# SnakeOnex/vit-is-all-you-need

Measured on AMD Instinct MI355X. Metric: images/sec ViT-B/16 224px bf16 fwd+bwd, higher is better.
Workload: dtype bf16; 1 GPU; ViT-B/16 224x224 bf16 forward+loss+backward, batch 256 per GPU (BASELINE configs[1]; configs[2] at 8 GPUs), random-init weights, 197 tokens, 79.44 M params; global_batch=256, parallelism=dp1

## Files before the change

### include/vitamd.h

```cpp
#ifndef VITAMD_H
#define VITAMD_H

#ifdef __cplusplus
extern "C" {
#endif

#define VITAMD_OK 0
#define VITAMD_ERR_SHAPE 1
#define VITAMD_ERR_ARG 2
#define VITAMD_ERR_LAUNCH 3
#define VITAMD_ERR_INIT 4

int vitamd_abi_version(void);

int vitamd_init(int device, void* stream);

#define VITAMD_EPI_BIAS_BF16 0
#define VITAMD_EPI_GELU 1
#define VITAMD_EPI_RESID_F32 2
#define VITAMD_EPI_DGELU 3
#define VITAMD_EPI_PATCH_F32 4
#define VITAMD_EPI_F32 5
#define VITAMD_EPI_GELU_DG 6
#define VITAMD_EPI_DMUL 7

int vitamd_gemm_nt_bf16(const void* A, const void* B, void* out, void* out2, const float* bias, const void* aux,
                        float* colsum, int M, int N, int K, int ldo, int epi, int n_patches, int seq, int extra,
                        int tile, void* stream);

#define VITAMD_NT_FORM_SMALL 1
#define VITAMD_NT_FORM_PP 2
#define VITAMD_NT_FORM_PP_PERSISTENT 3
#define VITAMD_NT_FORM_SEAM 4
#define VITAMD_NT_FORM_LOADER 5
#define VITAMD_NT_FORM_TAIL_SPLIT 0x80
int vitamd_gemm_nt_plan(int M, int N, int K, int ldo, int epi, int tile);

int vitamd_linear_dropout_resid_bf16(const void* A, const void* B, float* out, const float* bias, const float* resid,
                                     int M, int N, int K, float dropout_p, unsigned long long seed, int tile, void* stream);

int vitamd_gemm_tn_bf16(const void* L, const void* Rm, float* out, int R, int P, int Q, int ldl, int ldr, int ldo,
                        int splits, void* stream);

#define VITAMD_TN_FORM_SHARED 0
#define VITAMD_TN_FORM_EXCLUSIVE 1
int vitamd_gemm_tn_bf16_ws(const void* L, const void* Rm, float* out, int R, int P, int Q, int ldl, int ldr, int ldo,
                           int splits, float* ws, long ws_bytes, int accumulate, int form, void* stream);
long vitamd_gemm_tn_ws_bytes(int R, int P, int Q, int splits);

int vitamd_layernorm_fwd(const float* x_in, const void* addend_bf16, float* x_out, void* y_bf16, float* mean,
                         float* rstd, int M, int D, float eps, void* stream);
int vitamd_layernorm_bwd(const void* dy_bf16, const float* x, const float* mean, const float* rstd,
                         const float* g_res, float* g_out, void* g_bf16, float* colsum, int M, int D, void* stream);
int vitamd_layernorm_bwd_dropout(const void* dy_bf16, const float* x, const float* mean, const float* rstd,
                                 const float* g_res, float* g_out, void* g_bf16, float* colsum, int M, int D,
                                 float dropout_p, unsigned long long seed, void* stream);
int vitamd_layernorm_bwd_xhat(const void* dy_bf16, const void* y_bf16, const float* rstd, const float* g_res, float* g_out,
                              void* g_bf16, float* colsum, int M, int D, float dropout_p, unsigned long long seed, void* stream);
int vitamd_layernorm_fwd_keep(const float* x_in, const void* addend_bf16, float* x_out, void* y_bf16, float* mean, float* rstd,
                              int B, int seq, int keep, int D, float eps, void* stream);
int vitamd_layernorm_bwd_keep(const void* dy_bf16, const void* x_or_y, const float* mean, const float* rstd, const float* g_res,
                              float* g_out, void* g_bf16, float* colsum, int B, int seq, int keep, int D, int use_xhat,
                              float dropout_p, unsigned long long seed, void* stream);

int vitamd_layernorm_affine_fwd(const float* x, const float* gamma, const float* beta, void* y_bf16, float* mean,
                                float* rstd, int M, int D, float eps, void* stream);
int vitamd_layernorm_affine_bwd(const void* dy_bf16, const float* x, const float* mean, const float* rstd,
                                const float* gamma, const float* g_res, float* g_out, void* g_bf16, float* colsum,
                                float* dgamma, float* dbeta, int M, int D, void* stream);
int vitamd_layernorm_affine_fwd_f32(const float* x, const float* gamma, const float* beta, float* y, float* mean,
                                    float* rstd, int M, int D, float eps, void* stream);
int vitamd_layernorm_affine_bwd_f32(const float* dy, const float* x, const float* mean, const float* rstd,
                                    const float* gamma, float* g_out, float* dgamma, float* dbeta, int M, int D, void* stream);

int vitamd_attention_fwd(const void* qkv, void* o, float* lse2, int B, int N, int H, int head_dim, int causal,
                         float dropout_p, unsigned long long seed, void* stream);
int vitamd_attention_fwd_resid(const void* qkv, void* o, float* lse2, const float* resid_in, float* resid_out, int B, int N, int H,
                               int head_dim, int causal, float dropout_p, unsigned long long seed, void* stream);
int vitamd_attention_bwd(const void* qkv, const void* o, const float* lse2, const void* d_o, void* dqkv,
                         float* delta, float* dbias, int B, int N, int H, int head_dim, int causal, float dropout_p,
                         unsigned long long seed, void* stream);
int vitamd_attention_keep_forms(int N, int nq);
int vitamd_attention_fwd_keep(const void* qkv, void* o, float* lse2, int B, int N, int H, int head_dim, int nq, void* stream);
int vitamd_attention_bwd_keep(const void* qkv, const void* o, const float* lse2, const void* d_o, void* dqkv, float* delta,
                              float* dbias, int B, int N, int H, int head_dim, int nq, void* stream);

int vitamd_kv_append(const void* qkv, void* k_cache, void* v_cache, const int* len, int B, int T, int H, int head_dim, int Lmax,
                     void* stream);
long vitamd_decode_attention_ws_bytes(int B, int H, int Lmax);
int vitamd_decode_attention(const void* qkv, const void* k_cache, const void* v_cache, void* o, const int* len, int B, int H,
                            int head_dim, int Lmax, float* ws, long ws_bytes, void* stream);
long vitamd_gemm_skinny_ws_bytes(int M, int N, int K);
int vitamd_gemm_skinny_bf16(const void* A, const void* W, void* out, void* out2, const float* bias, const float* aux, int M, int N,
                            int K, int epi, float* ws, long ws_bytes, void* stream);

int vitamd_gemm_skinny_qkv_append(const void* A, const void* W, void* qkv, const float* bias, void* k_cache, void* v_cache, const int* len,
                                  int M, int H, int K, int head_dim, int Lmax, float* ws, long ws_bytes, void* stream);
int vitamd_decode_embed(const float* tok_table, const float* pos_table, const long long* token, const int* len, float* x, int B, int D,
                        int tok_rows, int pos_rows, void* stream);

int vitamd_sample_logits(const float* logits, long long* token, float* info, const float* u, const unsigned long long* step, int B, int V,
                         int ld, float temperature, int top_k, float top_p, unsigned long long seed, void* stream);

int vitamd_cross_entropy_fwd(const void* logits, int logits_bf16, const long long* target, float* loss_row, float* lse, float* stats,
                             int M, int V, int ld, long long ignore_index, void* stream);
int vitamd_cross_entropy_grid_rows(int V);
int vitamd_cross_entropy_bwd(const void* logits, int logits_bf16, const long long* target, const float* lse, const float* stats,
                             const float* grad_out, void* dlogits, int dlogits_bf16, int M, int V, int ld, int ldo,
                             long long ignore_index, void* stream);
int vitamd_embed_tokens_fwd(const float* tok_table, const float* pos_table, const long long* ids, float* x, int B, int S, int D,
                            int tok_rows, int pos_rows, void* stream);
int vitamd_embed_tokens_bwd(const float* g, const long long* ids, float* dtok, float* dpos, int B, int S, int D, int tok_rows, void* stream);

int vitamd_cast_f32_bf16(const float* in, void* out_bf16, long n, void* stream);
int vitamd_cast_f32_bf16_dropout(const float* in, void* out_bf16, long n, float dropout_p, unsigned long long seed, void* stream);
int vitamd_dropout_bf16(const void* in, void* out, long n, long group, float dropout_p, unsigned long long seed, void* stream);
int vitamd_dropout_f32(const float* in, float* out, long n, long group, float dropout_p, unsigned long long seed, void* stream);
int vitamd_cast_transpose_weight(const float* w, void* wb, void* wbt, int N, int K, void* stream);
int vitamd_cast_transpose_batched(const void* desc_dev, int n, int total_tiles, void* stream);
int vitamd_im2col_bf16(const float* img, void* out_bf16, int B, int C, int H, int W, int p, void* stream);
int vitamd_colsum_bf16(const void* x_bf16, float* out, int M, int N, int ld, void* stream);
int vitamd_embed_bwd(const float* g, float* dpos, float* dextra, void* dyp_bf16, float* dbias, float* dbias_rows, int B,
                     int seq, int extra, int D, void* stream);

int vitamd_vq_nearest(const float* x, const float* codebook, long long* idx, int M, int K, int d, void* stream);

int vitamd_conv3x3_fwd(const float* x, const float* w, const float* bias, float* y, int B, int Cin, int Cout, int H, int W,
                       void* stream);
int vitamd_conv3x3_bwd(const float* x, const float* w, const float* dy, float* dx, float* dw, float* db, int B, int Cin,
                       int Cout, int H, int W, void* stream);

int vitamd_adamw_step(float* p, const float* g, float* m, float* v, long n, float lr, float beta1, float beta2,
                      float eps, float weight_decay, int step, void* stream);
int vitamd_adamw_step_d(float* p, const float* g, float* m, float* v, long n, float lr, double beta1, double beta2,
                        float eps, float weight_decay, int step, void* stream);

typedef struct vitamd_mt_row {
  float* p;
  const float* g;
  float* m;
  float* v;
  long long n;
  int first_chunk;
  float lr, weight_decay;
  float beta1, one_minus_beta1, beta2, one_minus_beta2;
  float eps;
  float inv_bc1;
  float inv_sqrt_bc2;
} vitamd_mt_row;
long vitamd_mt_row_bytes(void);
int vitamd_mt_chunk_elems(void);
int vitamd_mt_grid_cap(void);
int vitamd_mt_sumsq(const vitamd_mt_row* rows_host, const void* rows_dev, int n_rows, int total_chunks, float* partials, float* norm_coef,
                    float max_norm, void* stream);
int vitamd_mt_adamw(const vitamd_mt_row* rows_host, const void* rows_dev, int n_rows, int total_chunks, const float* coef, void* stream);
int vitamd_mt_scale(const vitamd_mt_row* rows_host, const void* rows_dev, int n_rows, int total_chunks, const float* coef, void* stream);

#ifdef __cplusplus
}
#endif
#endif
```

### vit-is-all-you-need_amd/csrc/capi.hip

```cpp
#include "common.h"
#include "vitamd_internal.h"
#include "../../include/vitamd.h"

extern "C" int vitamd_abi_version(void) { return 9; }

extern "C" int vitamd_init(int device, void* stream) { return vitamd_init_impl(device, (hipStream_t)stream); }

extern "C" int vitamd_gemm_nt_bf16(const void* A, const void* B, void* out, void* out2, const float* bias, const void* aux,
                                   float* colsum, int M, int N, int K, int ldo, int epi, int n_patches, int seq, int extra,
                                   int tile, void* stream) {
  const int dg = (epi == 6 || epi == 7) ? 1 : 0;
  if (epi == 6) epi = EPI_GELU;
  if (epi == 7) epi = EPI_DGELU;
  GemmNtArgs p{A, B, out, out2, bias, aux, colsum, M, N, K, ldo, epi, n_patches, seq, extra, tile, 0u, 1.0f, 0u, 0u, 0, dg};
  if (!is_auto(tile) && tile != NT_TILE_128 && tile != NT_TILE_256 && tile != NT_TILE_320 && tile != NT_TILE_LOADER) return VITAMD_ERR_ARG;
  return vitamd_gemm_nt_impl(p, (hipStream_t)stream);
}

extern "C" int vitamd_gemm_nt_plan(int M, int N, int K, int ldo, int epi, int tile) {
  const int dg = (epi == 6 || epi == 7) ? 1 : 0;
  if (epi == 6) epi = EPI_GELU;
  if (epi == 7) epi = EPI_DGELU;
  static char dummy[16];
  GemmNtArgs p{dummy, dummy, dummy, dummy, nullptr, dummy, (float*)dummy, M, N, K, ldo, epi, 1, 1, 0, tile, 0u, 1.0f, 0u, 0u, 0, dg};
  if (!is_auto(tile) && tile != NT_TILE_128 && tile != NT_TILE_256 && tile != NT_TILE_320 && tile != NT_TILE_LOADER) return -VITAMD_ERR_ARG;
  return vitamd_gemm_nt_plan_impl(p);
}

extern "C" int vitamd_gemm_tn_bf16(const void* L, const void* Rm, float* out, int R, int P, int Q, int ldl, int ldr, int ldo,
                                   int splits, void* stream) {
  GemmTnArgs a{L, Rm, out, R, P, Q, ldl, ldr, ldo, splits, nullptr, 0, 1, 0};
  return vitamd_gemm_tn_impl(a, (hipStream_t)stream);
}

extern "C" int vitamd_gemm_tn_bf16_ws(const void* L, const void* Rm, float* out, int R, int P, int Q, int ldl, int ldr, int ldo,
                                      int splits, float* ws, long ws_bytes, int accumulate, int form, void* stream) {
  if (form != 0 && form != 1) return VITAMD_ERR_ARG;
  GemmTnArgs a{L, Rm, out, R, P, Q, ldl, ldr, ldo, splits, ws, (size_t)(ws_bytes < 0 ? 0 : ws_bytes), accumulate, form};
  return vitamd_gemm_tn_impl(a, (hipStream_t)stream);
}

static bool dropout_params(float p, unsigned& thresh, float& scale) {
  if (!(p >= 0.0f) || p >= 1.0f) return false;
  thresh = p > 0.0f ? (unsigned)((double)p * 4294967296.0) : 0u;
  if (p > 0.0f && thresh == 0u) thresh = 1u;
  scale = 1.0f / (1.0f - p);
  return true;
}

extern "C" int vitamd_linear_dropout_resid_bf16(const void* A, const void* B, float* out, const float* bias, const float* resid,
                                                int M, int N, int K, float dropout_p, unsigned long long seed, int tile, void* stream) {
  if (!is_auto(tile) && tile != NT_TILE_128 && tile != NT_TILE_256 && tile != NT_TILE_320) return VITAMD_ERR_ARG;
  GemmNtArgs p{A, B, out, nullptr, bias, resid, nullptr, M, N, K, N, EPI_RESID_F32, 0, 0, 0, tile, 0u, 1.0f,
               (unsigned)seed, (unsigned)(seed >> 32), 0, 0};
  if (!dropout_params(dropout_p, p.drop_thresh, p.drop_scale)) return VITAMD_ERR_ARG;
  return vitamd_gemm_nt_impl(p, (hipStream_t)stream);
}
```

### vit-is-all-you-need_amd/csrc/gemm_nt.hip

```cpp
#include <type_traits>
#include <mutex>
#include <atomic>
#include <cmath>
#include <cstring>
#include <climits>
#include "gemm_nt_ld.h"

namespace {

template <int BM, int BN, int WM, int WN, int EPI>
__global__ __launch_bounds__(WM * WN * 64) void gemm_nt_kernel(const GemmNtArgs p) {
  constexpr int NW = WM * WN;
  constexpr int WTM = BM / WM, WTN = BN / WN;
  constexpr int MT = WTM / 16, NT = WTN / 16;
  constexpr int PIECES = (BM + BN) / 8;
  constexpr int PPW = PIECES / NW;
  static_assert(PIECES % NW == 0, "pieces must divide over waves");
  constexpr int BUF_BYTES = (BM + BN) * 128;

  extern __shared__ __attribute__((aligned(16))) char smem[];

  const int tid = threadIdx.x;
  const int lane = tid & 63;
  const int wave = __builtin_amdgcn_readfirstlane(tid >> 6);
  const int wm = wave / WN, wn = wave % WN;

  const int tiles_n = (p.N + BN - 1) / BN;
  const int tiles_m = (p.M + BM - 1) / BM;
  const int tile = xcd_remap(blockIdx.x, tiles_m * tiles_n);
  const int m0 = (tile / tiles_n) * BM;
  const int n0 = (tile % tiles_n) * BN;

  const __bf16* __restrict__ A = (const __bf16*)p.A;
  const __bf16* __restrict__ B = (const __bf16*)p.B;
  const int K = p.K;

  const __bf16* src[PPW];
#pragma unroll
  for (int i = 0; i < PPW; ++i) {
    const int piece = wave * PPW + i;
    const int row = piece * 8 + (lane >> 3);
    const int logical = (lane & 7) ^ (row & 7);
    if (piece < BM / 8) {
      const int g = min(m0 + row, p.M - 1);
      src[i] = A + (size_t)g * K + logical * 8;
    } else {
      const int g = min(n0 + row - BM, p.N - 1);
      src[i] = B + (size_t)g * K + logical * 8;
    }
  }

  auto stage = [&](int kt, int buf) {
    char* base = smem + buf * BUF_BYTES + wave * PPW * 1024;
#pragma unroll
    for (int i = 0; i < PPW; ++i) glds16(src[i] + kt * BK, base + i * 1024);
  };

  f32x4 acc[MT][NT];
#pragma unroll
  for (int i = 0; i < MT; ++i)
#pragma unroll
    for (int j = 0; j < NT; ++j) acc[i][j] = (f32x4){0.f, 0.f, 0.f, 0.f};

  const int frag_off = (lane & 15) * 128 + ((((lane >> 4) ^ (lane & 7)) & 7) << 4);
  const int a_off = wm * WTM * 128 + frag_off;
  const int b_off = BM * 128 + wn * WTN * 128 + frag_off;

  const int nkt = K / BK;
  stage(0, 0);
  for (int kt = 0; kt < nkt; ++kt) {
    const int cur = kt & 1;
    asm volatile("s_waitcnt vmcnt(0)" ::: "memory");
    __syncthreads();
    if (kt + 1 < nkt) stage(kt + 1, cur ^ 1);
    const char* buf = smem + cur * BUF_BYTES;
#pragma unroll
    for (int ks = 0; ks < 2; ++ks) {
      bf16x8 af[MT], bfr[NT];
#pragma unroll
      for (int j = 0; j < NT; ++j) bfr[j] = *(const bf16x8*)(buf + ((b_off + j * 16 * 128) ^ (ks * 64)));
#pragma unroll
      for (int i = 0; i < MT; ++i) af[i] = *(const bf16x8*)(buf + ((a_off + i * 16 * 128) ^ (ks * 64)));
#pragma unroll
      for (int i = 0; i < MT; ++i)
#pragma unroll
        for (int j = 0; j < NT; ++j)
          acc[i][j] = __builtin_amdgcn_mfma_f32_16x16x32_bf16(bfr[j], af[i], acc[i][j], 0, 0, 0);
    }
  }
  if constexpr (BM == 256 && BN == 256 && WM == 2 && WN == 4 && EPI != EPI_F32) {
    if (p.N % 8 == 0 && p.ldo % 8 == 0) {
      gemm_epilogue_rows<EPI>(p, acc, m0, n0, wm, wn, lane, tid, wave, smem);
      return;
    }
  }
  gemm_epilogue<BN, WM, WN, WTM, WTN, MT, NT, EPI>(p, acc, m0, n0, wm, wn, lane, tid, smem);
}

template <int EPI, int MT, int LA, int LB, bool PERS = false>
__global__ __launch_bounds__(512) void gemm_nt_pp_kernel(const GemmNtArgs p) {
  using S = NtSchedule<MT, LA>;
  static_assert(LB == S::LB, "the B lead the shared schedule implements");
  constexpr int NP = S::NP;
  constexpr int BM = 32 * MT, BN = 256, WN = 4, NT = 4;
  constexpr int PART = 64 * 128;
  constexpr int BUFB = NP * PART + 256 * 128;

  extern __shared__ __attribute__((aligned(16))) char smem[];
  const int tid = threadIdx.x, lane = tid & 63;
  const int wave = __builtin_amdgcn_readfirstlane(tid >> 6);
  const int wm = wave / WN, wn = wave % WN;
  const int tiles_n = (p.N + BN - 1) / BN, tiles_m = (p.M + BM - 1) / BM;
  const int ntiles = tiles_m * tiles_n;
  const int K = p.K;
  const int nkt = K / 64;
  const srd_t srdA = make_srd(p.A, (size_t)p.M * K * 2);
  const srd_t srdB = make_srd(p.B, (size_t)p.N * K * 2);
  for (int ti = blockIdx.x; ti < ntiles; ti += PERS ? (int)gridDim.x : ntiles) {
  const NtTile t = nt_tile<BM>(ti, tiles_m, tiles_n);
  const int m0 = t.m0, n0 = t.n0;
  unsigned voffA[NP], voffB[4];
  pp_offsets<MT, false>(p, t, wave, lane, voffA, voffB);
  const unsigned lds0 = lds_addr(smem) + wave * 1024;
  constexpr unsigned OOB = 0x80000000u;
  auto request_a = [&](int kt, int j) {
    const bool live = kt >= 0 && kt < nkt;
    asm_glds16(srdA, lds0 + (kt & 1) * BUFB + j * PART, live ? voffA[j] : OOB, live ? (unsigned)kt * 128u : 0u);
  };
  auto request_b = [&](int kt, int q) {
    const bool live = kt >= 0 && kt < nkt;
    asm_glds16(srdB, lds0 + (kt & 1) * BUFB + NP * PART + q * 8192, live ? voffB[q] : OOB, live ? (unsigned)kt * 128u : 0u);
  };

  f32x4 acc[MT][NT];
#pragma unroll
  for (int i = 0; i < MT; ++i)
#pragma unroll
    for (int j = 0; j < NT; ++j) acc[i][j] = (f32x4){0.f, 0.f, 0.f, 0.f};

  const char *rdA[2], *rdB[2];
  frag_bases(smem + wm * 32 * 128, lane, rdA);
  frag_bases(smem + NP * PART + wn * 64 * 128, lane, rdB);

#pragma unroll
  for (int P = -S::lookback; P < 0; ++P) S::requests(S::tile_of(P), S::phase_of(P), request_a, request_b);
  VITAMD_WAIT_VM(S::wait(NP - 1));
  __builtin_amdgcn_s_barrier();
  asm volatile("" ::: "memory");
  if (wm == 1) __builtin_amdgcn_s_barrier();

  auto ktile = [&](int kt, auto bufc) {
    constexpr int BUF = decltype(bufc)::value;
    pp_ktile<MT, PART>(acc, rdA[0] + BUF * BUFB, rdA[1] + BUF * BUFB, rdB[0] + BUF * BUFB, rdB[1] + BUF * BUFB,
                       [&](int ph) { S::requests(kt, ph, request_a, request_b); }, [&](int ph) { VITAMD_WAIT_VM(S::wait(ph)); });
  };
  int kt = 0;
  for (; kt + 1 < nkt; kt += 2) {
    ktile(kt, std::integral_constant<int, 0>{});
    ktile(kt + 1, std::integral_constant<int, 1>{});
  }
  if (kt < nkt) ktile(kt, std::integral_constant<int, 0>{});
  if (wm == 0) __builtin_amdgcn_s_barrier();
  asm volatile("s_waitcnt vmcnt(0)" ::: "memory");
  if constexpr (EPI == EPI_F32) gemm_epilogue<BN, 2, WN, 16 * MT, 64, MT, NT, EPI>(p, acc, m0, n0, wm, wn, lane, tid, smem);
  else if (p.N % 8 == 0 && p.ldo % 8 == 0) gemm_epilogue_rows<EPI, MT>(p, acc, m0, n0, wm, wn, lane, tid, wave, smem);
  else gemm_epilogue<BN, 2, WN, 16 * MT, 64, MT, NT, EPI>(p, acc, m0, n0, wm, wn, lane, tid, smem);
  if constexpr (PERS) __syncthreads();
  }
}

static int device_cus() {
  static int cus[16] = {};
  int dev = 0;
  if (hipGetDevice(&dev) != hipSuccess || dev < 0 || dev >= 16) return 256;
  if (!cus[dev]) {
    int n = 0;
    cus[dev] = (hipDeviceGetAttribute(&n, hipDeviceAttributeMultiprocessorCount, dev) == hipSuccess && n > 0) ? n : 256;
  }
  return cus[dev];
}

template <int EPI, int MT, int LA, int LB, bool PERS = false>
int launch_pp(const GemmNtArgs& p, hipStream_t stream) {
  constexpr int ops_b = 2 * ((MT / 2) * 8192 + 32768), epi_b = 8 * MT * 2048;
  return launch_tiles(gemm_nt_pp_kernel<EPI, MT, LA, LB, PERS>, p, stream, 32 * MT, 512, ops_b > epi_b ? ops_b : epi_b, PERS ? device_cus() : INT_MAX);
}
#undef VITAMD_WAIT_VM

template <int BM, int BN, int WM, int WN, int EPI>
int launch(const GemmNtArgs& p, hipStream_t stream) {
  constexpr int lds = 2 * (BM + BN) * 128;
  auto kern = gemm_nt_kernel<BM, BN, WM, WN, EPI>;
  if (int e = set_lds(kern, lds)) return e;
  const int tiles = ((p.M + BM - 1) / BM) * ((p.N + BN - 1) / BN);
  hipLaunchKernelGGL(kern, dim3(tiles), dim3(WM * WN * 64), lds, stream, p);
  return hipGetLastError() == hipSuccess ? VITAMD_OK : VITAMD_ERR_LAUNCH;
}

static bool prefer_tall(const GemmNtArgs& p) {
  if (p.N % 8 != 0 || p.ldo % 8 != 0 || p.K % 64 != 0) return false;
  if (p.epi != EPI_BIAS_BF16 && p.epi != EPI_RESID_F32 && p.epi != EPI_GELU && p.epi != EPI_DGELU) return false;
  const long tn = (p.N + 255) / 256;
  const long r256 = (((p.M + 255) / 256) * tn + 255) / 256, r320 = (((p.M + 319) / 320) * tn + 255) / 256;
  return r320 * 320 <= r256 * 256;
}

static unsigned short bf16_rne_d(double v) {
  auto val = [](unsigned short b) { const unsigned w = (unsigned)b << 16; float g; memcpy(&g, &w, 4); return (double)g; };
  const float f = (float)v;
  unsigned u;
  memcpy(&u, &f, 4);
  unsigned short best = (unsigned short)((u + 0x7fffu + ((u >> 16) & 1u)) >> 16);
  double bd = fabs(val(best) - v);
  const unsigned short first = best;
  for (int dl = -1; dl <= 1; dl += 2) {
    const unsigned short n = (unsigned short)(first + dl);
    const double dd = fabs(val(n) - v);
    if (dd < bd || (dd == bd && !(n & 1) && (best & 1))) { best = n; bd = dd; }
  }
  return best;
}

static std::atomic<const unsigned*> g_gelu_tab[64];

static const unsigned* gelu_table() {
  int dev = -1;
  if (hipGetDevice(&dev) != hipSuccess || dev < 0 || dev >= 64) { (void)hipGetLastError(); return nullptr; }
  return g_gelu_tab[dev].load(std::memory_order_acquire);
}

}

const unsigned* vitamd_gelu_table() { return gelu_table(); }

int vitamd_init_impl(int device, hipStream_t stream) {
  static std::mutex mu;
  static unsigned host[4096];
  static bool built = false;
  int cur = -1;
  if (hipGetDevice(&cur) != hipSuccess) { (void)hipGetLastError(); return VITAMD_ERR_LAUNCH; }
  if (device < 0) device = cur;
  if (device >= 64) return VITAMD_ERR_ARG;
  std::lock_guard<std::mutex> lock(mu);
  if (g_gelu_tab[device].load(std::memory_order_acquire)) return VITAMD_OK;
  hipStreamCaptureStatus cap = hipStreamCaptureStatusNone;
  if (hipStreamIsCapturing(stream, &cap) != hipSuccess || cap != hipStreamCaptureStatusNone) { (void)hipGetLastError(); return VITAMD_ERR_ARG; }
  if (!built) {
    for (int sg = 0; sg < 2; ++sg)
      for (int i = 0; i < 2048; ++i) {
        const unsigned w = (unsigned)(0x3900 + i) << 16;
        float ax;
        memcpy(&ax, &w, 4);
        const double x = sg ? -(double)ax : (double)ax;
        const double cdf = 0.5 * erfc(-x * 0.70710678118654752440);
        const double pdf = 0.39894228040143267794 * exp(-0.5 * x * x);
        host[sg * 2048 + i] = (unsigned)bf16_rne_d(x * cdf) | ((unsigned)bf16_rne_d(cdf + x * pdf) << 16);
      }
    built = true;
  }
  if (device != cur && hipSetDevice(device) != hipSuccess) { (void)hipGetLastError(); return VITAMD_ERR_ARG; }
  void* d = nullptr;
  bool ok = hipMalloc(&d, sizeof(host)) == hipSuccess;
  ok = ok && hipMemcpy(d, host, sizeof(host), hipMemcpyHostToDevice) == hipSuccess && hipDeviceSynchronize() == hipSuccess;
  if (!ok) {
    (void)hipGetLastError();
    if (d) (void)hipFree(d);
  }
  if (device != cur) (void)hipSetDevice(cur);
  if (!ok) return VITAMD_ERR_LAUNCH;
  g_gelu_tab[device].store((const unsigned*)d, std::memory_order_release);
  return VITAMD_OK;
}

namespace {

enum NtForm { NT_FORM_SMALL = 1, NT_FORM_PP = 2, NT_FORM_PP_PERSISTENT = 3, NT_FORM_SEAM = 4, NT_FORM_LOADER = 5 };
struct NtPlan { int form, rows, err; };

static NtPlan plan_single(const GemmNtArgs& p) {
  int tile = p.tile;
  const int epi = p.epi;
  const bool seam_epi = epi == EPI_BIAS_BF16 || epi == EPI_GELU || epi == EPI_DGELU;
  const bool tall_epi = seam_epi || epi == EPI_RESID_F32;
  if (tile == NT_TILE_LOADER) return (seam_epi && ld_ok(p)) ? NtPlan{NT_FORM_LOADER, 256, VITAMD_OK} : NtPlan{0, 0, VITAMD_ERR_SHAPE};
  const bool no_seam = tile == NT_TILE_AUTO_NO_SEAM;
  if (no_seam) tile = NT_TILE_AUTO;
  const long big_tiles = (long)((p.M + 255) / 256) * ((p.N + 255) / 256);
  const bool pp_ok = (size_t)p.M * p.K * 2 < 0xf0000000ull && (size_t)p.N * p.K * 2 < 0xf0000000ull && p.K % 64 == 0;
  const bool big = p.N >= 256 && big_tiles >= 192 && pp_ok;
  const bool tall = tall_epi && prefer_tall(p);
  if (tile == NT_TILE_AUTO_NO_PERSISTENT) tile = NT_TILE_AUTO;
  else if (tile == NT_TILE_AUTO && big) {
    const int cus = device_cus();
    if (seam_epi && !no_seam && seam_ok(p) && p.K <= 1536) {
      if (epi == EPI_BIAS_BF16 && tall && (long)((p.M + 319) / 320) * ((p.N + 255) / 256) >= 3L * cus) return NtPlan{NT_FORM_SEAM, 320, VITAMD_OK};
      if (big_tiles >= 3L * cus) return NtPlan{ld_ok(p) ? NT_FORM_LOADER : NT_FORM_SEAM, 256, VITAMD_OK};
    }
    return NtPlan{NT_FORM_PP_PERSISTENT, tall ? 320 : 256, VITAMD_OK};
  }
  if (tile == NT_TILE_AUTO) tile = big ? (tall ? NT_TILE_320 : NT_TILE_256) : NT_TILE_128;
  if (tile == NT_TILE_320) return (tall_epi && pp_ok) ? NtPlan{NT_FORM_PP, 320, VITAMD_OK} : NtPlan{0, 0, VITAMD_ERR_SHAPE};
  if (tile == NT_TILE_256) return pp_ok ? NtPlan{NT_FORM_PP, 256, VITAMD_OK} : NtPlan{0, 0, VITAMD_ERR_SHAPE};
  if (tile != NT_TILE_128) return NtPlan{0, 0, VITAMD_ERR_ARG};
  return p.K % BK == 0 ? NtPlan{NT_FORM_SMALL, 128, VITAMD_OK} : NtPlan{0, 0, VITAMD_ERR_SHAPE};
}

template <int EPI>
int dispatch_tile(const GemmNtArgs& p, hipStream_t stream) {
  constexpr bool seam_epi = EPI == EPI_BIAS_BF16 || EPI == EPI_GELU || EPI == EPI_DGELU;
  constexpr bool tall_epi = seam_epi || EPI == EPI_RESID_F32;
  const NtPlan pl = plan_single(p);
  if (pl.err) return pl.err;
  switch (pl.form) {
    case NT_FORM_LOADER:
      if constexpr (seam_epi) return launch_ld<EPI, EPI == EPI_GELU>(p, stream, device_cus());
      break;
    case NT_FORM_SEAM:
      if constexpr (EPI == EPI_BIAS_BF16) { if (pl.rows == 320) return launch_seam<EPI, 10>(p, stream, device_cus()); }
      if constexpr (seam_epi) return launch_seam<EPI, 8, EPI == EPI_GELU>(p, stream, device_cus());
      break;
    case NT_FORM_PP_PERSISTENT:
      if constexpr (tall_epi) { if (pl.rows == 320) return launch_pp<EPI, 10, 4, 6, true>(p, stream); }
      return launch_pp<EPI, 8, 4, 6, true>(p, stream);
    case NT_FORM_PP:
      if constexpr (tall_epi) { if (pl.rows == 320) return launch_pp<EPI, 10, 4, 6>(p, stream); }
      return launch_pp<EPI, 8, 4, 6>(p, stream);
    case NT_FORM_SMALL:
      return launch<128, 128, 2, 2, EPI>(p, stream);
  }
  return VITAMD_ERR_SHAPE;
}

}

static int dispatch_epi(const GemmNtArgs& p, hipStream_t stream) {
  switch (p.epi) {
    case EPI_BIAS_BF16: return dispatch_tile<EPI_BIAS_BF16>(p, stream);
    case EPI_GELU: return dispatch_tile<EPI_GELU>(p, stream);
    case EPI_RESID_F32: return dispatch_tile<EPI_RESID_F32>(p, stream);
    case EPI_DGELU: return dispatch_tile<EPI_DGELU>(p, stream);
    case EPI_PATCH_F32: return dispatch_tile<EPI_PATCH_F32>(p, stream);
    case EPI_F32: return dispatch_tile<EPI_F32>(p, stream);
    default: return VITAMD_ERR_ARG;
  }
}

static int tail_split_rows(const GemmNtArgs& p, bool& tall) {
  const int CUS = device_cus();
  tall = is_auto(p.tile) && prefer_tall(p);
  const int bm = tall ? 320 : 256;
  const int tiles_m = (p.M + bm - 1) / bm, tiles_n = (p.N + 255) / 256;
  const long big_tiles = (long)tiles_m * tiles_n;
  const long rem = big_tiles % CUS;
  const bool split_on = p.epi == EPI_RESID_F32 && !tall;
  if (!(is_auto(p.tile) && split_on && p.epi != EPI_PATCH_F32 && p.N >= 256 && p.K % 64 == 0 && big_tiles > 2 * CUS && rem != 0 && rem * 10 < CUS * 6))
    return 0;
  const int rows_a = (int)((big_tiles - rem) / tiles_n) * bm;
  return rows_a > 0 && rows_a < p.M ? rows_a : 0;
}

static int check_args(const GemmNtArgs& p) {
  if (p.M <= 0 || p.N <= 0 || p.K <= 0 || p.K % 32 != 0 || p.N % 4 != 0 || p.ldo % 4 != 0) return VITAMD_ERR_SHAPE;
  if (!p.A || !p.B || !p.out) return VITAMD_ERR_ARG;
  if (p.epi == EPI_GELU && !p.out2) return VITAMD_ERR_ARG;
  if ((p.epi == EPI_RESID_F32 || p.epi == EPI_DGELU) && !p.aux) return VITAMD_ERR_ARG;
  if (p.epi == EPI_PATCH_F32 && (!p.aux || p.n_patches <= 0)) return VITAMD_ERR_ARG;
  if (p.epi < EPI_BIAS_BF16 || p.epi > EPI_F32) return VITAMD_ERR_ARG;
  return VITAMD_OK;
}

int vitamd_gemm_nt_impl(const GemmNtArgs& p0, hipStream_t stream) {
  if (int e = check_args(p0)) return e;
  GemmNtArgs p = p0;
  if (p.epi == EPI_GELU) {
    p.gelu_tab = gelu_table();
    if (!p.gelu_tab) return VITAMD_ERR_INIT;
  }
  bool tall = false;
  const int rows_a = tail_split_rows(p, tall);
  if (rows_a) {
    GemmNtArgs a = p, b = p;
    a.M = rows_a;
    a.tile = tall ? p.tile : NT_TILE_256;
    const size_t esz_out = (p.epi == EPI_RESID_F32 || p.epi == EPI_F32) ? 4 : 2;
    b.M = p.M - rows_a;
    b.A = (const char*)p.A + (size_t)rows_a * p.K * 2;
    b.out = (char*)p.out + (size_t)rows_a * p.ldo * esz_out;
    if (p.out2) b.out2 = (char*)p.out2 + (size_t)rows_a * p.ldo * 2;
    if (p.aux) b.aux = (const char*)p.aux + (size_t)rows_a * p.ldo * (p.epi == EPI_RESID_F32 ? 4 : 2);
    b.tile = NT_TILE_128;
    b.row0 = p.row0 + rows_a;
    if (int e = dispatch_epi(a, stream)) return e;
    return dispatch_epi(b, stream);
  }
  return dispatch_epi(p, stream);
}

int vitamd_gemm_nt_plan_impl(const GemmNtArgs& p0) {
  if (int e = check_args(p0)) return -e;
  bool tall = false;
  GemmNtArgs p = p0;
  const int rows_a = tail_split_rows(p, tall);
  if (rows_a) {
    p.M = rows_a;
    p.tile = tall ? p.tile : NT_TILE_256;
  }
  const NtPlan pl = plan_single(p);
  if (pl.err) return -pl.err;
  return pl.form | (pl.rows << 8) | (rows_a ? 0x80 : 0);
}
```

### vit-is-all-you-need_amd/csrc/gemm_nt_ld.h

```cpp
#pragma once
#include "gemm_nt_seam.h"

namespace {

template <int EPI, bool TAB = false, int SCHED = 1>
__global__ __launch_bounds__(768) void gemm_nt_ld_kernel(const GemmNtArgs p) {
  static_assert(EPI == EPI_BIAS_BF16 || EPI == EPI_GELU || EPI == EPI_DGELU, "epilogues of the loader form");
  static_assert(SCHED == 1, "request schedule");
  static_assert(!TAB || EPI == EPI_GELU, "table = GELU");
  constexpr int BM = 256, BN = 256, MT = 8, NT = 4;
  constexpr int AREG = 16384, ABUF = 32768, BBUF = 32768, BBASE = 2 * ABUF, OPS = BBASE + 2 * BBUF;
  constexpr int STG = 2048, TABOFF = OPS + 8 * STG;
  constexpr unsigned OOB = 0x80000000u;

  extern __shared__ __attribute__((aligned(16))) char smem[];
  const int tid = threadIdx.x, lane = tid & 63;
  const int wave = __builtin_amdgcn_readfirstlane(tid >> 6);
  const int tiles_n = (p.N + BN - 1) / BN, tiles_m = (p.M + BM - 1) / BM;
  const int ntiles = tiles_m * tiles_n;
  const int K = p.K;
  const int nkt = K / 64;
  auto coords = [&](int ti) { return nt_tile<BM>(ti, tiles_m, tiles_n); };

  if (wave >= 8) {
    const int l = wave - 8;
    const srd_t srdA = make_srd(p.A, (size_t)p.M * K * 2);
    const srd_t srdB = make_srd(p.B, (size_t)p.N * K * 2);
    const srd_t srdBias = make_srd(p.bias ? (const void*)p.bias : p.out, p.bias ? (size_t)p.N * 4 : 0);
    const unsigned ldsA = lds_addr(smem) + l * 4096;
    const unsigned ldsB = lds_addr(smem) + BBASE + l * 8192;
    unsigned voffA[2][4], voffB[8];
    auto offsets = [&](const NtTile& t) {
      const int r8 = lane >> 3;
      const unsigned chunk = (unsigned)(((lane & 7) ^ r8) * 16);
#pragma unroll
      for (int h = 0; h < 2; ++h)
#pragma unroll
        for (int i = 0; i < 4; ++i) {
          const int a = 4 * l + i;
          const int row = min(t.m0 + (a >> 3) * 128 + h * 64 + (a & 7) * 8 + r8, p.M - 1);
          voffA[h][i] = (unsigned)row * (unsigned)(K * 2) + chunk;
        }
#pragma unroll
      for (int i = 0; i < 8; ++i) {
        const int row = min(t.n0 + (8 * l + i) * 8 + r8, p.N - 1);
        voffB[i] = (unsigned)row * (unsigned)(K * 2) + chunk;
      }
    };
    bool live = true;
    unsigned so = 0u, par = 0u;
    auto request_b = [&](int i) {
      asm_glds16(srdB, ldsB + par * BBUF + i * 1024, live ? voffB[i] : OOB, so);
    };
    auto request_a = [&](int h, int i) {
      asm_glds16(srdA, ldsA + par * ABUF + h * AREG + i * 1024, live ? voffA[h][i] : OOB, so);
    };
    auto target = [&](int kt, bool lv) {
      live = lv;
      so = live ? (unsigned)kt * 128u : 0u;
      par = (unsigned)(kt & 1);
    };
    __builtin_amdgcn_s_setprio(3);
    int ti = blockIdx.x;
    NtTile cur = coords(ti);
    offsets(cur);
    int bias_n0 = cur.n0;
    target(0, true);
#pragma unroll
    for (int i = 0; i < 8; ++i) request_b(i);
#pragma unroll
    for (int i = 0; i < 4; ++i) request_a(0, i);
#pragma unroll
    for (int i = 0; i < 4; ++i) request_a(1, i);
    VITAMD_WAIT_VM(4);
    __builtin_amdgcn_s_barrier();
    for (;;) {
      const int ti_next = ti + (int)gridDim.x;
      const bool has_next = ti_next < ntiles;
      for (int kt = 0; kt < nkt; ++kt) {
        const bool last = kt + 1 == nkt;
        if (last && has_next) {
          cur = coords(ti_next);
          offsets(cur);
        }
        target(last ? 0 : kt + 1, !last || has_next);
        request_b(0); request_b(1); request_b(2);
        __builtin_amdgcn_s_barrier();
        request_b(3); request_b(4); request_b(5);
        VITAMD_WAIT_VM(6);
        __builtin_amdgcn_s_barrier();
        if constexpr (EPI != EPI_DGELU) {
          if (kt == 0) {
            asm_glds4(srdBias, lds_addr(smem) + OPS + l * STG, (unsigned)(bias_n0 + l * 64 + lane) * 4u, 0u);
            asm_glds4(srdBias, lds_addr(smem) + OPS + (4 + l) * STG, (unsigned)(bias_n0 + l * 64 + lane) * 4u, 0u);
          }
        }
        request_b(6); request_b(7); request_a(0, 0);
        __builtin_amdgcn_s_barrier();
        request_a(0, 1); request_a(0, 2); request_a(0, 3);
        __builtin_amdgcn_s_barrier();
        request_a(1, 0); request_a(1, 1);
        __builtin_amdgcn_s_barrier();
        request_a(1, 2); request_a(1, 3);
        __builtin_amdgcn_s_barrier();
        __builtin_amdgcn_s_barrier();
        VITAMD_WAIT_VM(4);
        __builtin_amdgcn_s_barrier();
      }
      __builtin_amdgcn_s_barrier();
      if (!has_next) break;
      ti = ti_next;
      bias_n0 = cur.n0;
    }
    asm volatile("s_waitcnt vmcnt(0)" ::: "memory");
    return;
  }

  const int wm = wave >> 2, wn = wave & 3;
  const srd_t rsO = make_srd(p.out, (size_t)p.M * p.ldo * 2);
  const srd_t rsO2 = make_srd(EPI == EPI_GELU ? p.out2 : p.out, (size_t)p.M * p.ldo * 2);
  const srd_t srdAux = make_srd(EPI == EPI_DGELU ? p.aux : p.out, (size_t)p.M * p.ldo * 2);
  if constexpr (TAB) gelu_table_to_lds(p.gelu_tab, smem + TABOFF, tid);
  __builtin_amdgcn_s_barrier();
  asm volatile("" ::: "memory");
  for (int ti = blockIdx.x; ti < ntiles; ti += (int)gridDim.x) {
    const NtTile cur = coords(ti);
    if (wm == 1) __builtin_amdgcn_s_barrier();
    f32x4 acc[MT][NT];
#pragma unroll
    for (int i = 0; i < MT; ++i)
#pragma unroll
      for (int j = 0; j < NT; ++j) acc[i][j] = (f32x4){0.f, 0.f, 0.f, 0.f};
    {
      int l2 = (int)__builtin_amdgcn_mbcnt_hi(~0u, __builtin_amdgcn_mbcnt_lo(~0u, 0u));
      asm volatile("" : "+v"(l2));
      const char *rdA[2], *rdB[2];
      frag_bases(smem + wm * 8192, l2, rdA);
      frag_bases(smem + BBASE + wn * 8192, l2, rdB);
      bf16x8 bq[NT], af[4];
      auto ktile = [&](auto bufc) {
        constexpr int BUF = decltype(bufc)::value;
#pragma unroll
        for (int ph = 0; ph < 4; ++ph) {
          const int ks = ph >> 1, h = ph & 1;
          if (h == 0) {
#pragma unroll
            for (int j = 0; j < NT; ++j) bq[j] = *(const bf16x8*)(rdB[ks] + BUF * BBUF + j * 2048);
          }
#pragma unroll
          for (int ii = 0; ii < 4; ++ii) af[ii] = *(const bf16x8*)(rdA[ks] + BUF * ABUF + h * AREG + ii * 2048);
          __builtin_amdgcn_sched_barrier(0);
          __builtin_amdgcn_s_barrier();
          asm volatile("s_waitcnt lgkmcnt(0)" ::: "memory");
          __builtin_amdgcn_sched_barrier(0);
          __builtin_amdgcn_s_setprio(1);
#pragma unroll
          for (int ii = 0; ii < 4; ++ii)
#pragma unroll
            for (int j = 0; j < NT; ++j)
              acc[4 * h + ii][j] = __builtin_amdgcn_mfma_f32_16x16x32_bf16(bq[j], af[ii], acc[4 * h + ii][j], 0, 0, 0);
          __builtin_amdgcn_s_setprio(0);
          __builtin_amdgcn_sched_barrier(0);
          __builtin_amdgcn_s_barrier();
          asm volatile("" ::: "memory");
        }
      };
      for (int kt = 0; kt < nkt; kt += 2) {
        ktile(std::integral_constant<int, 0>{});
        ktile(std::integral_constant<int, 1>{});
      }
    }
    if (wm == 0) __builtin_amdgcn_s_barrier();

    int ln = (int)__builtin_amdgcn_mbcnt_hi(~0u, __builtin_amdgcn_mbcnt_lo(~0u, 0u));
    asm volatile("" : "+v"(ln));
    const int mloc = ln & 15, g = ln >> 4, rsub = ln >> 3, pc = ln & 7;
    char* const stg = smem + OPS + wave * STG;
    const int m0 = cur.m0, n0 = cur.n0;
    const int ncol = n0 + wn * 64 + 8 * (pc ^ rsub);
    const bool ncol_ok = ncol < p.N;
    const int mrow0 = m0 + wm * 128 + rsub;
    const unsigned obase = ncol_ok ? (unsigned)mrow0 * (unsigned)(p.ldo * 2) + (unsigned)ncol * 2u : OOB;
    const unsigned rstep = (unsigned)(p.ldo * 2) * 8u;
    u32x4 aux[EPI == EPI_DGELU ? 2 * MT : 1];
    u32x2 pk[EPI == EPI_DGELU ? MT : 1][NT];
    f32x4 bias4[NT];
    if constexpr (EPI == EPI_DGELU) {
#pragma unroll
      for (int i = 0; i < MT; ++i)
#pragma unroll
        for (int j = 0; j < NT; ++j) pk[i][j] = (u32x2){pack_bf16x2(acc[i][j][0], acc[i][j][1]), pack_bf16x2(acc[i][j][2], acc[i][j][3])};
#pragma unroll
      for (int it = 0; it < 2 * MT; ++it) aux[it] = asm_bload16(srdAux, mrow0 + 8 * it < p.M ? obase : OOB, rstep * (unsigned)it);
      static_assert(MT == 8, "16 pre-load registers named in one asm statement");
      asm volatile("s_waitcnt vmcnt(0)" : "+v"(aux[0]), "+v"(aux[1]), "+v"(aux[2]), "+v"(aux[3]), "+v"(aux[4]), "+v"(aux[5]), "+v"(aux[6]), "+v"(aux[7]), "+v"(aux[8]), "+v"(aux[9]), "+v"(aux[10]), "+v"(aux[11]), "+v"(aux[12]), "+v"(aux[13]), "+v"(aux[14]), "+v"(aux[15]) :: "memory");
    } else {
#pragma unroll
      for (int j = 0; j < NT; ++j)
#pragma unroll
        for (int r = 0; r < 4; ++r) bias4[j][r] = round_bf16(((const float*)stg)[16 * j + 4 * g + r]);
    }
    float cs[8];
#pragma unroll
    for (int c = 0; c < 8; ++c) cs[c] = 0.f;
#pragma unroll
    for (int i = 0; i < MT; ++i) {
#pragma unroll
      for (int j = 0; j < NT; ++j) {
        u32x2 o;
        if constexpr (EPI == EPI_DGELU) o = pk[i][j];
        else {
          const f32x4 v = acc[i][j] + bias4[j];
          o = (u32x2){pack_bf16x2(v[0], v[1]), pack_bf16x2(v[2], v[3])};
        }
        *(u32x2*)(stg + mloc * 128 + (((2 * j + (g >> 1)) ^ (mloc & 7)) << 4) + (g & 1) * 8) = o;
      }
#pragma unroll
      for (int h = 0; h < 2; ++h) {
        const u32x4 v = *(const u32x4*)(stg + (rsub + 8 * h) * 128 + pc * 16);
        const unsigned voff = mrow0 + 16 * i + 8 * h < p.M ? obase : OOB;
        const unsigned soff = rstep * (unsigned)(2 * i + h);
        if constexpr (EPI == EPI_BIAS_BF16) {
          asm_bstore16_nt(v, rsO, voff, soff);
        } else if constexpr (EPI == EPI_GELU) {
          u32x4 a, d = v;
          if constexpr (TAB) gelu_lookup8(v, smem + TABOFF, p.gelu_dg != 0, a, d);
          else
#pragma unroll
            for (int c = 0; c < 4; ++c) {
              float dlo, dhi;
              a[c] = pack_bf16x2(gelu_fwd_grad(bf16lo(v[c]), dlo), gelu_fwd_grad(bf16hi(v[c]), dhi));
              if (p.gelu_dg) d[c] = pack_bf16x2(dlo, dhi);
            }
          asm_bstore16_nt(d, rsO, voff, soff);
          asm_bstore16_nt(a, rsO2, voff, soff);
        } else {
          const u32x4 pz = aux[2 * i + h];
          u32x4 o;
#pragma unroll
          for (int c = 0; c < 4; ++c) {
            const float lo = round_bf16(bf16lo(v[c]) * bf16lo(pz[c]));
            const float hi = round_bf16(bf16hi(v[c]) * bf16hi(pz[c]));
            if (voff != OOB) { cs[2 * c] += lo; cs[2 * c + 1] += hi; }
            o[c] = pack_bf16x2(lo, hi);
          }
          asm_bstore16_nt(o, rsO, voff, soff);
        }
      }
    }
    if constexpr (EPI == EPI_DGELU) {
#pragma unroll
      for (int bf = 1; bf < 8; bf <<= 1)
#pragma unroll
        for (int c = 0; c < 8; ++c) cs[c] += __shfl_xor(cs[c], 9 * bf, 64);
      float s = cs[0];
#pragma unroll
      for (int c = 1; c < 8; ++c) s = rsub == c ? cs[c] : s;
      atomicAdd(p.colsum + n0 + wn * 64 + 8 * (pc ^ rsub) + rsub, s);
    }
    asm volatile("s_waitcnt lgkmcnt(0)" ::: "memory");
  }
}

template <int EPI, bool TAB = false, int SCHED = 1>
int launch_ld(const GemmNtArgs& p, hipStream_t stream, int cus) {
  if (TAB && !p.gelu_tab) return VITAMD_ERR_ARG;
  return launch_tiles(gemm_nt_ld_kernel<EPI, TAB, SCHED>, p, stream, 256, 768, 160 * 1024, cus);
}

static bool ld_ok(const GemmNtArgs& p) { return seam_ok(p) && p.K % 128 == 0; }

}
```

### vit-is-all-you-need_amd/csrc/gemm_nt_seam.h

```cpp
#pragma once
#include "gemm_nt_pp.h"

namespace {

template <int EPI, int MT, bool TAB = false>
__global__ __launch_bounds__(512) void gemm_nt_seam_kernel(const GemmNtArgs p) {
  static_assert(EPI == EPI_BIAS_BF16 || EPI == EPI_GELU || EPI == EPI_DGELU, "epilogues without (or with up-front) auxiliary loads");
  static_assert(!TAB || (EPI == EPI_GELU && MT == 8), "the GELU table needs the 16 KiB that only the 256-row ring leaves");
  constexpr int LA = 4;
  using S = NtSchedule<MT, LA>;
  constexpr int NP = S::NP;
  constexpr int BM = 32 * MT, BN = 256, WN = 4, NT = 4;
  constexpr int PART = 8192, ASLOT = NP * PART, BSLOT = 32768, BBASE = 2 * ASLOT, OPS = BBASE + 2 * BSLOT;
  constexpr int STG = TAB ? 2048 : (160 * 1024 - OPS) / 8;
  constexpr int TABOFF = OPS + 8 * STG;
  constexpr int SL = STG / 2048;
  static_assert(SL >= 1 && MT % SL == 0, "staging");
  constexpr int E = EPI == EPI_GELU ? 4 * MT : EPI == EPI_DGELU ? 2 * MT + 1 : 2 * MT;
  static_assert(S::wait(NP - 1) + E <= 63 && S::wait(0, E) <= 63, "vmcnt is a 6-bit counter");

  extern __shared__ __attribute__((aligned(16))) char smem[];
  const int tid = threadIdx.x, lane = tid & 63;
  const int wave = __builtin_amdgcn_readfirstlane(tid >> 6);
  const int wm = wave / WN, wn = wave % WN;
  const int tiles_n = (p.N + BN - 1) / BN, tiles_m = (p.M + BM - 1) / BM;
  const int ntiles = tiles_m * tiles_n;
  const int K = p.K;
  const int nkt = K / 64;
  const srd_t srdA = make_srd(p.A, (size_t)p.M * K * 2);
  const srd_t srdB = make_srd(p.B, (size_t)p.N * K * 2);
  const srd_t rsO = make_srd(p.out, (size_t)p.M * p.ldo * 2);
  const srd_t rsO2 = make_srd(EPI == EPI_GELU ? p.out2 : p.out, (size_t)p.M * p.ldo * 2);
  const srd_t srdAux = make_srd(EPI == EPI_DGELU ? p.aux : p.out, (size_t)p.M * p.ldo * 2);
  const srd_t srdBias = make_srd(p.bias ? (const void*)p.bias : p.out, p.bias ? (size_t)p.N * 4 : 0);
  constexpr unsigned OOB = 0x80000000u;
  const unsigned lds0 = lds_addr(smem) + wave * 1024;

  unsigned voffA[NP], voffB[4];
  auto offsets = [&](const NtTile& t) {
    int l2 = (int)__builtin_amdgcn_mbcnt_hi(~0u, __builtin_amdgcn_mbcnt_lo(~0u, 0u));
    asm volatile("" : "+v"(l2));
    pp_offsets<MT, true>(p, t, wave, l2, voffA, voffB);
  };
  bool fill = true;
  auto request_a = [&](int kt, int j) {
    const bool live = fill && kt >= 0 && kt < nkt;
    asm_glds16(srdA, lds0 + ((kt + 8) & 1) * ASLOT + j * PART, live ? voffA[j] : OOB, live ? (unsigned)kt * 128u : 0u);
  };
  auto request_b = [&](int kt, int q) {
    const bool live = fill && kt >= 0 && kt < nkt;
    asm_glds16(srdB, lds0 + BBASE + ((kt + 8) & 1) * BSLOT + q * 8192, live ? voffB[q] : OOB, live ? (unsigned)kt * 128u : 0u);
  };
  auto prologue = [&]() {
#pragma unroll
    for (int P = -S::lookback; P < 0; ++P) S::requests(S::tile_of(P), S::phase_of(P), request_a, request_b);
  };

  const char *rdA[2], *rdB[2];
  frag_bases(smem + wm * 32 * 128, lane, rdA);
  frag_bases(smem + BBASE + wn * 64 * 128, lane, rdB);

  if constexpr (TAB) gelu_table_to_lds(p.gelu_tab, smem + TABOFF, tid);
  int ti = blockIdx.x;
  NtTile cur = nt_tile<BM>(ti, tiles_m, tiles_n);
  offsets(cur);
  prologue();
  VITAMD_WAIT_VM(S::wait(NP - 1));
  __builtin_amdgcn_s_barrier();
  asm volatile("" ::: "memory");
  if (wm == 1) __builtin_amdgcn_s_barrier();
  bool seam = false;

  for (;;) {
    f32x4 acc[MT][NT];
#pragma unroll
    for (int i = 0; i < MT; ++i)
#pragma unroll
      for (int j = 0; j < NT; ++j) acc[i][j] = (f32x4){0.f, 0.f, 0.f, 0.f};

    auto ktile = [&](int kt) {
      const bool lenient = seam && kt == 0;
      const int sa = (kt & 1) * ASLOT, sb = (kt & 1) * BSLOT;
      pp_ktile<MT, PART>(acc, rdA[0] + sa, rdA[1] + sa, rdB[0] + sb, rdB[1] + sb,
                         [&](int ph) { S::requests(kt, ph, request_a, request_b); },
                         [&](int ph) {
                           if (S::wait(ph, E) != S::wait(ph) && lenient) VITAMD_WAIT_VM(S::wait(ph, E));
                           else VITAMD_WAIT_VM(S::wait(ph));
                         });
    };
    for (int kt = 0; kt < nkt; ++kt) ktile(kt);
    if (wm == 0) __builtin_amdgcn_s_barrier();
    asm volatile("s_waitcnt vmcnt(0)" ::: "memory");

    int ln = (int)__builtin_amdgcn_mbcnt_hi(~0u, __builtin_amdgcn_mbcnt_lo(~0u, 0u));
    asm volatile("" : "+v"(ln));
    const int mloc = ln & 15, g = ln >> 4, rsub = ln >> 3, pc = ln & 7;
    char* const stg = smem + OPS + wave * STG;
    const int m0 = cur.m0, n0 = cur.n0;
    const int ncol = n0 + wn * 64 + 8 * (pc ^ rsub);
    const bool ncol_ok = ncol < p.N;
    const int mrow0 = m0 + wm * (16 * MT) + rsub;
    const unsigned obase = ncol_ok ? (unsigned)mrow0 * (unsigned)(p.ldo * 2) + (unsigned)ncol * 2u : OOB;
    const unsigned rstep = (unsigned)(p.ldo * 2) * 8u;
    u32x4 aux[EPI == EPI_DGELU ? 2 * MT : 1];
    u32x2 pk[EPI == EPI_DGELU ? MT : 1][NT];
    if constexpr (EPI == EPI_DGELU) {
#pragma unroll
      for (int i = 0; i < MT; ++i)
#pragma unroll
        for (int j = 0; j < NT; ++j) pk[i][j] = (u32x2){pack_bf16x2(acc[i][j][0], acc[i][j][1]), pack_bf16x2(acc[i][j][2], acc[i][j][3])};
#pragma unroll
      for (int it = 0; it < 2 * MT; ++it) {
        aux[it] = asm_bload16(srdAux, mrow0 + 8 * it < p.M ? obase : OOB, rstep * (unsigned)it);
      }
    } else {
      asm_glds4(srdBias, lds_addr(stg), (unsigned)(n0 + wn * 64 + ln) * 4u, 0u);
    }
    const int ti_next = ti + (int)gridDim.x;
    const bool has_next = ti_next < ntiles;
    if (has_next) {
      cur = nt_tile<BM>(ti_next, tiles_m, tiles_n);
      offsets(cur);
    }
    fill = has_next;
    prologue();
    fill = true;
    constexpr int NREQ = S::prologue_requests();
    if constexpr (EPI == EPI_DGELU) {
      static_assert(MT == 8, "16 pre-load registers named in one asm statement");
      asm volatile("s_waitcnt vmcnt(%16)" : "+v"(aux[0]), "+v"(aux[1]), "+v"(aux[2]), "+v"(aux[3]), "+v"(aux[4]), "+v"(aux[5]), "+v"(aux[6]), "+v"(aux[7]), "+v"(aux[8]), "+v"(aux[9]), "+v"(aux[10]), "+v"(aux[11]), "+v"(aux[12]), "+v"(aux[13]), "+v"(aux[14]), "+v"(aux[15]) : "n"(NREQ) : "memory");
    } else {
      asm volatile("s_waitcnt vmcnt(%0)" :: "n"(NREQ) : "memory");
    }
    f32x4 bias4[NT];
#pragma unroll
    for (int j = 0; j < NT; ++j) {
      bias4[j] = (f32x4){0.f, 0.f, 0.f, 0.f};
      if constexpr (EPI != EPI_DGELU) {
#pragma unroll
        for (int r = 0; r < 4; ++r) bias4[j][r] = round_bf16(((const float*)stg)[16 * j + 4 * g + r]);
      }
    }
    float cs[8];
#pragma unroll
    for (int c = 0; c < 8; ++c) cs[c] = 0.f;
#pragma unroll
    for (int rd = 0; rd < MT / SL; ++rd) {
#pragma unroll
      for (int s = 0; s < SL; ++s) {
        const int i = rd * SL + s;
#pragma unroll
        for (int j = 0; j < NT; ++j) {
          u32x2 o;
          if constexpr (EPI == EPI_DGELU) o = pk[i][j];
          else {
            const f32x4 v = acc[i][j] + bias4[j];
            o = (u32x2){pack_bf16x2(v[0], v[1]), pack_bf16x2(v[2], v[3])};
          }
          *(u32x2*)(stg + s * 2048 + mloc * 128 + (((2 * j + (g >> 1)) ^ (mloc & 7)) << 4) + (g & 1) * 8) = o;
        }
      }
#pragma unroll
      for (int s = 0; s < SL; ++s) {
        const int i = rd * SL + s;
#pragma unroll
        for (int h = 0; h < 2; ++h) {
          const u32x4 v = *(const u32x4*)(stg + s * 2048 + (rsub + 8 * h) * 128 + pc * 16);
          const unsigned voff = mrow0 + 16 * i + 8 * h < p.M ? obase : OOB;
          const unsigned soff = rstep * (unsigned)(2 * i + h);
          if constexpr (EPI == EPI_BIAS_BF16) {
            asm_bstore16_nt(v, rsO, voff, soff);
          } else if constexpr (EPI == EPI_GELU) {
            u32x4 a, d = v;
            if constexpr (TAB) gelu_lookup8(v, smem + TABOFF, p.gelu_dg != 0, a, d);
            else
#pragma unroll
            for (int c = 0; c < 4; ++c) {
              float dlo, dhi;
              a[c] = pack_bf16x2(gelu_fwd_grad(bf16lo(v[c]), dlo), gelu_fwd_grad(bf16hi(v[c]), dhi));
              if (p.gelu_dg) d[c] = pack_bf16x2(dlo, dhi);
            }
            asm_bstore16_nt(d, rsO, voff, soff);
            asm_bstore16_nt(a, rsO2, voff, soff);
          } else {
            const u32x4 pz = aux[2 * i + h];
            u32x4 o;
#pragma unroll
            for (int c = 0; c < 4; ++c) {
              const float lo = round_bf16(bf16lo(v[c]) * bf16lo(pz[c]));
              const float hi = round_bf16(bf16hi(v[c]) * bf16hi(pz[c]));
              if (voff != OOB) { cs[2 * c] += lo; cs[2 * c + 1] += hi; }
              o[c] = pack_bf16x2(lo, hi);
            }
            asm_bstore16_nt(o, rsO, voff, soff);
          }
        }
      }
    }
    if constexpr (EPI == EPI_DGELU) {
#pragma unroll
      for (int bf = 1; bf < 8; bf <<= 1)
#pragma unroll
        for (int c = 0; c < 8; ++c) cs[c] += __shfl_xor(cs[c], 9 * bf, 64);
      float s = cs[0];
#pragma unroll
      for (int c = 1; c < 8; ++c) s = rsub == c ? cs[c] : s;
      atomicAdd(p.colsum + n0 + wn * 64 + 8 * (pc ^ rsub) + rsub, s);
    }
    if (!has_next) break;
    ti = ti_next;
    VITAMD_WAIT_VM(S::wait(NP - 1) + E);
    asm volatile("s_waitcnt lgkmcnt(0)" ::: "memory");
    __builtin_amdgcn_s_barrier();
    asm volatile("" ::: "memory");
    if (wm == 1) __builtin_amdgcn_s_barrier();
    seam = true;
  }
}

template <int EPI, int MT, bool TAB = false>
int launch_seam(const GemmNtArgs& p, hipStream_t stream, int cus) {
  if (TAB && !p.gelu_tab) return VITAMD_ERR_ARG;
  return launch_tiles(gemm_nt_seam_kernel<EPI, MT, TAB>, p, stream, 32 * MT, 512, 160 * 1024, cus);
}

static bool seam_ok(const GemmNtArgs& p) {
  if (p.K % 64 != 0 || p.K < 128 || p.N % 8 != 0 || p.ldo % 8 != 0) return false;
  if ((size_t)p.M * p.K * 2 >= 0xf0000000ull || (size_t)p.N * p.K * 2 >= 0xf0000000ull || (size_t)p.M * p.ldo * 2 >= 0x80000000ull) return false;
  if (p.epi == EPI_DGELU) return p.gelu_dg && p.colsum != nullptr && p.N % 256 == 0 && p.aux != nullptr;
  if (p.epi == EPI_GELU) return p.out2 != nullptr;
  return p.epi == EPI_BIAS_BF16;
}

}
```

### vit-is-all-you-need_amd/csrc/gemm_tn.hip

```cpp
#include "common.h"
#include "vitamd_internal.h"

namespace {

constexpr int BR = 64;
constexpr int BP = 256, BQ = 256;
constexpr int WP = 2, WQ = 4, NW = 8;
constexpr int MT = BP / WP / 32;
constexpr int NT = BQ / WQ / 32;
constexpr int TILE_BYTES = BR * 512;
constexpr int BUF_BYTES = 2 * TILE_BYTES;
constexpr int PPW = (2 * BR / 2) / NW;

typedef LDS_AS bf16x4* lds_bf16x4_ptr;

__device__ __forceinline__ bf16x8 tr_frag(const char* p) {
  bf16x4 lo = __builtin_amdgcn_ds_read_tr16_b64_v4bf16((lds_bf16x4_ptr)(p));
  bf16x4 hi = __builtin_amdgcn_ds_read_tr16_b64_v4bf16((lds_bf16x4_ptr)(p + 4 * 512));
  return __builtin_shufflevector(lo, hi, 0, 1, 2, 3, 4, 5, 6, 7);
}

constexpr int QSLOT = 16 * 512 * 2;

template <bool WS, int NQ, int D>
__global__ __launch_bounds__(NW * 64) void gemm_tn_pp_kernel(const GemmTnArgs a, int tiles_p, int tiles_q, int splits) {
  static_assert(D >= 2 && D <= NQ - 2, "prefetch distance: WAR rule");
  extern __shared__ __attribute__((aligned(16))) char smem[];
  const int tid = threadIdx.x, lane = tid & 63;
  const int wave = __builtin_amdgcn_readfirstlane(tid >> 6);
  const int wp = wave / WQ, wq = wave % WQ;

  const int ntile = tiles_p * tiles_q;
  const int id = xcd_remap(blockIdx.x, ntile * splits);
  const int split = id / ntile, tile = id % ntile;
  const int p0 = (tile / tiles_q) * BP, q0 = (tile % tiles_q) * BQ;
  const int nsteps = (a.R + BR - 1) / BR;
  const int s_lo = (int)((long)nsteps * split / splits), s_hi = (int)((long)nsteps * (split + 1) / splits);
  if (s_lo >= s_hi) return;
  const int g_lo = 4 * s_lo, g_hi = 4 * s_hi;

  const bool isL = wave < NW / 2;
  const int ld = isL ? a.ldl : a.ldr;
  const int c0 = isL ? p0 : q0;
  const int ncols = isL ? a.P : a.Q;
  const srd_t srd = isL ? make_srd(a.L, (size_t)a.R * a.ldl * 2) : make_srd(a.Rm, (size_t)a.R * a.ldr * 2);
  unsigned voff[2];
#pragma unroll
  for (int i = 0; i < 2; ++i) {
    const int row = ((wave & 3) * 2 + i) * 2 + (lane >> 5);
    const int logical = (lane & 31) ^ ((row & 3) << 2);
    const int col = c0 + logical * 8;
    voff[i] = (col < ncols) ? (unsigned)(((size_t)row * ld + col) * 2) : 0x80000000u;
  }
  const unsigned qbytes = (unsigned)16 * ld * 2;
  const unsigned dst0 = lds_addr(smem) + (isL ? 0 : 8192) + (wave & 3) * 2048;

  f32x16 acc[MT][NT];
#pragma unroll
  for (int i = 0; i < MT; ++i)
#pragma unroll
    for (int j = 0; j < NT; ++j)
#pragma unroll
      for (int r = 0; r < 16; ++r) acc[i][j][r] = 0.f;

  const int h = lane >> 5, colhalf = (lane >> 4) & 1, qq = (lane >> 2) & 3, pp = lane & 3;
  const int rowpart = (8 * h + qq) * 512 + (pp & 1) * 8;
  int offA[MT], offB[NT];
#pragma unroll
  for (int i = 0; i < MT; ++i) {
    const int chunk = (wp * (BP / WP) + i * 32) / 8 + 2 * colhalf + (pp >> 1);
    offA[i] = rowpart + ((chunk ^ (qq << 2)) << 4);
  }
#pragma unroll
  for (int j = 0; j < NT; ++j) {
    const int chunk = (wq * (BQ / WQ) + j * 32) / 8 + 2 * colhalf + (pp >> 1);
    offB[j] = 8192 + rowpart + ((chunk ^ (qq << 2)) << 4);
  }

  int slot_w = 0;
  unsigned soff = (unsigned)g_lo * qbytes;
#pragma unroll
  for (int d = 0; d < D; ++d) {
    const unsigned dst = dst0 + slot_w * QSLOT;
    asm_glds16(srd, dst, voff[0], soff);
    asm_glds16(srd, dst + 1024, voff[1], soff);
    soff += qbytes;
    slot_w = slot_w + 1 == NQ ? 0 : slot_w + 1;
  }
  static_assert(D <= 8, "add a vmcnt literal");
#define VITAMD_WAIT_VM(n) asm volatile("s_waitcnt vmcnt(%0)" ::"n"(n) : "memory")
  VITAMD_WAIT_VM(2 * (D - 1));
  __builtin_amdgcn_s_barrier();
  asm volatile("" ::: "memory");
  if (wp == 1) __builtin_amdgcn_s_barrier();
  int slot_r = 0;
  for (int g = g_lo; g < g_hi; ++g) {
    const char* q = smem + slot_r * QSLOT;
    bf16x8 af[MT], bfr[NT];
#pragma unroll
    for (int j = 0; j < NT; ++j) bfr[j] = tr_frag(q + offB[j]);
#pragma unroll
    for (int i = 0; i < MT; ++i) af[i] = tr_frag(q + offA[i]);
    {
      const unsigned dst = dst0 + slot_w * QSLOT;
      asm_glds16(srd, dst, voff[0], soff);
      asm_glds16(srd, dst + 1024, voff[1], soff);
      soff += qbytes;
      slot_w = slot_w + 1 == NQ ? 0 : slot_w + 1;
    }
    VITAMD_WAIT_VM(2 * (D - 1));
    __builtin_amdgcn_sched_barrier(0);
    __builtin_amdgcn_s_barrier();
    asm volatile("s_waitcnt lgkmcnt(0)" ::: "memory");
    __builtin_amdgcn_sched_barrier(0);
    __builtin_amdgcn_s_setprio(1);
#pragma unroll
    for (int i = 0; i < MT; ++i)
#pragma unroll
      for (int j = 0; j < NT; ++j) acc[i][j] = __builtin_amdgcn_mfma_f32_32x32x16_bf16(af[i], bfr[j], acc[i][j], 0, 0, 0);
    __builtin_amdgcn_s_setprio(0);
    __builtin_amdgcn_sched_barrier(0);
    __builtin_amdgcn_s_barrier();
    asm volatile("" ::: "memory");
    slot_r = slot_r + 1 == NQ ? 0 : slot_r + 1;
  }
  if (wp == 0) __builtin_amdgcn_s_barrier();
  asm volatile("s_waitcnt vmcnt(0)" ::: "memory");
#undef VITAMD_WAIT_VM

  if constexpr (WS) {
    float* wt = a.ws + ((size_t)split * ntile + tile) * (BP * BQ);
#pragma unroll
    for (int j = 0; j < NT; ++j) {
      const int ql = wq * (BQ / WQ) + j * 32 + (lane & 31);
#pragma unroll
      for (int i = 0; i < MT; ++i) {
        const int pl = wp * (BP / WP) + i * 32 + 4 * (lane >> 5);
#pragma unroll
        for (int r = 0; r < 16; ++r) wt[(pl + (r & 3) + 8 * (r >> 2)) * BQ + ql] = acc[i][j][r];
      }
    }
  } else {
#pragma unroll
    for (int j = 0; j < NT; ++j) {
      const int q = q0 + wq * (BQ / WQ) + j * 32 + (lane & 31);
#pragma unroll
      for (int i = 0; i < MT; ++i) {
        const int pbase = p0 + wp * (BP / WP) + i * 32 + 4 * (lane >> 5);
#pragma unroll
        for (int r = 0; r < 16; ++r) {
          const int p = pbase + (r & 3) + 8 * (r >> 2);
          if (p < a.P && q < a.Q) atomicAdd(a.out + (size_t)p * a.ldo + q, acc[i][j][r]);
        }
      }
    }
  }
}

template <int NQ, int D>
__global__ __launch_bounds__(768) void gemm_tn_ld_kernel(const GemmTnArgs a, int tiles_p, int tiles_q, int splits) {
  static_assert(D >= 2 && D <= NQ - 2, "prefetch distance: WAR rule");
  extern __shared__ __attribute__((aligned(16))) char smem[];
  const int tid = threadIdx.x, lane = tid & 63;
  const int wave = __builtin_amdgcn_readfirstlane(tid >> 6);
  const bool loader = wave >= NW;
  const int ntile = tiles_p * tiles_q;
  const int id = xcd_remap(blockIdx.x, ntile * splits);
  const int split = id / ntile, tile = id % ntile;
  const int p0 = (tile / tiles_q) * BP, q0 = (tile % tiles_q) * BQ;
  const int nsteps = (a.R + BR - 1) / BR;
  const int s_lo = (int)((long)nsteps * split / splits), s_hi = (int)((long)nsteps * (split + 1) / splits);
  if (s_lo >= s_hi) return;
  const int g_lo = 4 * s_lo, g_hi = 4 * s_hi;
#define VITAMD_WAIT_VM(n) asm volatile("s_waitcnt vmcnt(%0)" ::"n"(n) : "memory")
  if (loader) {
    const int l = wave - NW;
    const srd_t srdL = make_srd(a.L, (size_t)a.R * a.ldl * 2), srdR = make_srd(a.Rm, (size_t)a.R * a.ldr * 2);
    unsigned voffL[2], voffR[2];
#pragma unroll
    for (int i = 0; i < 2; ++i) {
      const int row = (l * 2 + i) * 2 + (lane >> 5);
      const int logical = (lane & 31) ^ ((row & 3) << 2);
      voffL[i] = (p0 + logical * 8 < a.P) ? (unsigned)(((size_t)row * a.ldl + p0 + logical * 8) * 2) : 0x80000000u;
      voffR[i] = (q0 + logical * 8 < a.Q) ? (unsigned)(((size_t)row * a.ldr + q0 + logical * 8) * 2) : 0x80000000u;
    }
    const unsigned qbL = (unsigned)16 * a.ldl * 2, qbR = (unsigned)16 * a.ldr * 2;
    const unsigned dstL = lds_addr(smem) + l * 2048, dstR = dstL + 8192;
    unsigned soL = (unsigned)g_lo * qbL, soR = (unsigned)g_lo * qbR;
    int slot_w = 0;
    auto issue_l = [&]() {
      const unsigned o = slot_w * QSLOT;
      asm_glds16(srdL, dstL + o, voffL[0], soL);
      asm_glds16(srdL, dstL + o + 1024, voffL[1], soL);
    };
    auto issue_r = [&]() {
      const unsigned o = slot_w * QSLOT;
      asm_glds16(srdR, dstR + o, voffR[0], soR);
      asm_glds16(srdR, dstR + o + 1024, voffR[1], soR);
      soL += qbL; soR += qbR;
      slot_w = slot_w + 1 == NQ ? 0 : slot_w + 1;
    };
    auto issue = [&]() { issue_l(); issue_r(); };
    __builtin_amdgcn_s_setprio(3);
#pragma unroll
    for (int d = 0; d < D; ++d) issue();
    VITAMD_WAIT_VM(4 * (D - 1));
    __builtin_amdgcn_s_barrier();
    for (int g = g_lo; g < g_hi; ++g) {
      issue_l();
      __builtin_amdgcn_s_barrier();
      issue_r();
      VITAMD_WAIT_VM(4 * (D - 1));
      __builtin_amdgcn_s_barrier();
    }
    __builtin_amdgcn_s_barrier();
    asm volatile("s_waitcnt vmcnt(0)" ::: "memory");
    return;
  }
  const int wp = wave / WQ, wq = wave % WQ;
  f32x16 acc[MT][NT];
#pragma unroll
  for (int i = 0; i < MT; ++i)
#pragma unroll
    for (int j = 0; j < NT; ++j)
#pragma unroll
      for (int r = 0; r < 16; ++r) acc[i][j][r] = 0.f;
  const int h = lane >> 5, colhalf = (lane >> 4) & 1, qq = (lane >> 2) & 3, pp = lane & 3;
  const int rowpart = (8 * h + qq) * 512 + (pp & 1) * 8;
  int offA[MT], offB[NT];
#pragma unroll
  for (int i = 0; i < MT; ++i) {
    const int chunk = (wp * (BP / WP) + i * 32) / 8 + 2 * colhalf + (pp >> 1);
    offA[i] = rowpart + ((chunk ^ (qq << 2)) << 4);
  }
#pragma unroll
  for (int j = 0; j < NT; ++j) {
    const int chunk = (wq * (BQ / WQ) + j * 32) / 8 + 2 * colhalf + (pp >> 1);
    offB[j] = 8192 + rowpart + ((chunk ^ (qq << 2)) << 4);
  }
  __builtin_amdgcn_s_barrier();
  asm volatile("" ::: "memory");
  if (wp == 1) __builtin_amdgcn_s_barrier();
  int slot_r = 0;
  for (int g = g_lo; g < g_hi; ++g) {
    const char* q = smem + slot_r * QSLOT;
    bf16x8 af[MT], bfr[NT];
#pragma unroll
    for (int j = 0; j < NT; ++j) bfr[j] = tr_frag(q + offB[j]);
#pragma unroll
    for (int i = 0; i < MT; ++i) af[i] = tr_frag(q + offA[i]);
    __builtin_amdgcn_sched_barrier(0);
    __builtin_amdgcn_s_barrier();
    asm volatile("s_waitcnt lgkmcnt(0)" ::: "memory");
    __builtin_amdgcn_sched_barrier(0);
    __builtin_amdgcn_s_setprio(1);
#pragma unroll
    for (int i = 0; i < MT; ++i)
#pragma unroll
      for (int j = 0; j < NT; ++j) acc[i][j] = __builtin_amdgcn_mfma_f32_32x32x16_bf16(af[i], bfr[j], acc[i][j], 0, 0, 0);
    __builtin_amdgcn_s_setprio(0);
    __builtin_amdgcn_sched_barrier(0);
    __builtin_amdgcn_s_barrier();
    asm volatile("" ::: "memory");
    slot_r = slot_r + 1 == NQ ? 0 : slot_r + 1;
  }
  if (wp == 0) __builtin_amdgcn_s_barrier();
#undef VITAMD_WAIT_VM
  float* wt = a.ws + ((size_t)split * ntile + tile) * (BP * BQ);
#pragma unroll
  for (int j = 0; j < NT; ++j) {
    const int ql = wq * (BQ / WQ) + j * 32 + (lane & 31);
#pragma unroll
    for (int i = 0; i < MT; ++i) {
      const int pl = wp * (BP / WP) + i * 32 + 4 * (lane >> 5);
#pragma unroll
      for (int r = 0; r < 16; ++r) wt[(pl + (r & 3) + 8 * (r >> 2)) * BQ + ql] = acc[i][j][r];
    }
  }
}

constexpr int RPT = 1;
__global__ __launch_bounds__(256) void splitk_reduce_kernel(const float* __restrict__ ws, float* __restrict__ out, int P, int Q, int ldo,
                                                            int tiles_q, int ntile, int splits, int accumulate) {
  const int tile = blockIdx.y;
  const int p0 = (tile / tiles_q) * BP, q0 = (tile % tiles_q) * BQ;
  f32x4 sum[RPT];
  const float* src[RPT];
  bool ok[RPT];
#pragma unroll
  for (int k = 0; k < RPT; ++k) {
    const int idx = (blockIdx.x * RPT + k) * 256 + threadIdx.x;
    const int pl = idx >> 6, ql = (idx & 63) * 4;
    ok[k] = p0 + pl < P && q0 + ql < Q;
    src[k] = ws + (size_t)tile * (BP * BQ) + pl * BQ + ql;
    sum[k] = ok[k] ? *(const f32x4*)src[k] : (f32x4){0.f, 0.f, 0.f, 0.f};
  }
  for (int s2 = 1; s2 < splits; ++s2) {
#pragma unroll
    for (int k = 0; k < RPT; ++k)
      if (ok[k]) sum[k] += *(const f32x4*)(src[k] + (size_t)s2 * ntile * (BP * BQ));
  }
#pragma unroll
  for (int k = 0; k < RPT; ++k) {
    if (!ok[k]) continue;
    const int idx = (blockIdx.x * RPT + k) * 256 + threadIdx.x;
    const int p = p0 + (idx >> 6), q = q0 + (idx & 63) * 4;
    float* dst = out + (size_t)p * ldo + q;
    if (q + 3 < Q && (ldo & 3) == 0) {
      if (accumulate) sum[k] += *(const f32x4*)dst;
      *(f32x4*)dst = sum[k];
    } else {
      for (int c = 0; c < 4 && q + c < Q; ++c) dst[c] = accumulate ? dst[c] + sum[k][c] : sum[k][c];
    }
  }
}

}

static int auto_splits(int R, int P, int Q, int requested) {
  const int ntile = ((P + BP - 1) / BP) * ((Q + BQ - 1) / BQ);
  const int nsteps = (R + BR - 1) / BR;
  int splits = requested;
  if (splits <= 0) splits = ntile >= 256 ? 1 : 256 / ntile;
  if (splits > nsteps) splits = nsteps;
  return splits;
}

extern "C" long vitamd_gemm_tn_ws_bytes(int R, int P, int Q, int splits) {
  if (R <= 0 || P <= 0 || Q <= 0) return 0;
  const long ntile = (long)((P + BP - 1) / BP) * ((Q + BQ - 1) / BQ);
  return (long)auto_splits(R, P, Q, splits) * ntile * BP * BQ * (long)sizeof(float);
}

int vitamd_gemm_tn_impl(const GemmTnArgs& a, hipStream_t stream) {
  if (a.R <= 0 || a.P <= 0 || a.Q <= 0 || a.ldl % 8 || a.ldr % 8 || a.ldl < a.P || a.ldr < a.Q || a.ldo < a.Q) return VITAMD_ERR_SHAPE;
  if ((size_t)(a.R + BR) * a.ldl * 2 >= 0x80000000ull || (size_t)(a.R + BR) * a.ldr * 2 >= 0x80000000ull) return VITAMD_ERR_SHAPE;
  if (!a.L || !a.Rm || !a.out) return VITAMD_ERR_ARG;
  const int tiles_p = (a.P + BP - 1) / BP, tiles_q = (a.Q + BQ - 1) / BQ;
  const int ntile = tiles_p * tiles_q;
  const int splits = auto_splits(a.R, a.P, a.Q, a.splits);
  constexpr int lds = 8 * QSLOT;
  const bool use_ws = a.ws != nullptr && a.ws_bytes >= (size_t)splits * ntile * BP * BQ * sizeof(float);
  if (!use_ws && !a.accumulate) return VITAMD_ERR_ARG;
  const dim3 grid(ntile * splits), block(NW * 64);
  if (use_ws) {
    if (a.form == 1) {
      if (int e = set_lds(gemm_tn_ld_kernel<8, 4>, lds)) return e;
      hipLaunchKernelGGL((gemm_tn_ld_kernel<8, 4>), grid, dim3(768), lds, stream, a, tiles_p, tiles_q, splits);
    } else {
      if (int e = set_lds(gemm_tn_pp_kernel<true, 8, 4>, lds)) return e;
      hipLaunchKernelGGL((gemm_tn_pp_kernel<true, 8, 4>), grid, block, lds, stream, a, tiles_p, tiles_q, splits);
    }
    hipLaunchKernelGGL(splitk_reduce_kernel, dim3(BP * BQ / 4 / 256 / RPT, ntile), dim3(256), 0, stream, a.ws, a.out, a.P, a.Q, a.ldo, tiles_q, ntile, splits,
                       a.accumulate);
  } else {
    if (int e = set_lds(gemm_tn_pp_kernel<false, 8, 4>, lds)) return e;
    hipLaunchKernelGGL((gemm_tn_pp_kernel<false, 8, 4>), grid, block, lds, stream, a, tiles_p, tiles_q, splits);
  }
  return hipGetLastError() == hipSuccess ? VITAMD_OK : VITAMD_ERR_LAUNCH;
}
```

### vit-is-all-you-need_amd/csrc/vitamd_internal.h

```cpp
#pragma once
#include <hip/hip_runtime.h>

enum GemmEpilogue {
  EPI_BIAS_BF16 = 0,
  EPI_GELU = 1,
  EPI_RESID_F32 = 2,
  EPI_DGELU = 3,
  EPI_PATCH_F32 = 4,
  EPI_F32 = 5,
};

enum NtTileCode {
  NT_TILE_AUTO = 0,
  NT_TILE_128 = 128,
  NT_TILE_256 = 256,
  NT_TILE_320 = 320,
  NT_TILE_AUTO_NO_PERSISTENT = 512,
  NT_TILE_AUTO_NO_SEAM = 1024,
  NT_TILE_LOADER = 2048,
};
inline bool is_auto(int tile) { return tile == NT_TILE_AUTO || tile == NT_TILE_AUTO_NO_PERSISTENT || tile == NT_TILE_AUTO_NO_SEAM; }

struct GemmNtArgs {
  const void* A;
  const void* B;
  void* out;
  void* out2;
  const float* bias;
  const void* aux;
  float* colsum;
  int M, N, K, ldo;
  int epi;
  int n_patches, seq, extra;
  int tile;
  unsigned drop_thresh;
  float drop_scale;
  unsigned drop_seed_lo, drop_seed_hi;
  int row0;
  int gelu_dg;
  const unsigned* gelu_tab;
};

struct GemmTnArgs {
  const void* L;
  const void* Rm;
  float* out;
  int R, P, Q, ldl, ldr, ldo;
  int splits;
  float* ws;
  size_t ws_bytes;
  int accumulate;
  int form;
};

int vitamd_gemm_nt_impl(const GemmNtArgs& p, hipStream_t stream);
int vitamd_gemm_nt_plan_impl(const GemmNtArgs& p);
int vitamd_init_impl(int device, hipStream_t stream);
const unsigned* vitamd_gelu_table();
int vitamd_gemm_tn_impl(const GemmTnArgs& p, hipStream_t stream);
```

### vit-is-all-you-need_amd/vitamd/functions.py

```python
from __future__ import annotations

import weakref

import torch

from . import ops

BF16, F32 = torch.bfloat16, torch.float32

_amp_fwd = torch.amp.custom_fwd(device_type="cuda", cast_inputs=torch.float32)
_amp_bwd = torch.amp.custom_bwd(device_type="cuda")


class WeightCache:

    def __init__(self):
        self._c = {}
        self._groups = {}
        self.epoch = 0

    def clear(self):
        self.epoch += 1

    def _fresh(self, ent, w, want_t):
        return (ent is not None and ent["ref"]() is w and ent["ver"] == w._version and ent["ptr"] == w.data_ptr()
                and ent["epoch"] == self.epoch and (ent["wbt"] is not None or not want_t))

    @staticmethod
    def _as2d(w):
        w2 = w.detach()
        return w2 if w2.dim() == 2 else w2.reshape(w2.shape[0], -1)

    def _entry(self, w, want_t):
        ent = self._c.get(id(w))
        w2 = self._as2d(w)
        if ent is None or ent["ref"]() is not w or ent["ptr"] != w.data_ptr() or tuple(ent["wb"].shape) != tuple(w2.shape):
            if len(self._c) > 4096:
                self._c = {k: v for k, v in self._c.items() if v["ref"]() is not None}
                self._groups.clear()
            ent = self._c[id(w)] = {"ref": weakref.ref(w), "ver": -1, "ptr": w.data_ptr(), "epoch": -1,
                                    "wb": torch.empty(w2.shape, dtype=BF16, device=w.device), "wbt": None}
        if want_t and ent["wbt"] is None:
            ent["wbt"] = torch.empty((w2.shape[1], w2.shape[0]), dtype=BF16, device=w.device)
            ent["ver"] = -1
        return ent

    def get(self, w: torch.Tensor, want_t: bool):
        if not w.is_cuda:
            raise ops._lib.VitamdError("weight: expected a ROCm device tensor (the HIP kernels are the only implementation)")
        ent = self._c.get(id(w))
        if self._fresh(ent, w, want_t):
            return ent["wb"], ent["wbt"]
        ent = self._entry(w, want_t)
        w2 = self._as2d(w).contiguous()
        N, K = w2.shape
        ops._lib.check(ops._L().vitamd_cast_transpose_weight(w2.data_ptr(), ent["wb"].data_ptr(),
                                                             ent["wbt"].data_ptr() if ent["wbt"] is not None else None, N, K,
                                                             ops._stream()), "cast_transpose_weight")
        ent["ver"], ent["epoch"] = w._version, self.epoch
        return ent["wb"], ent["wbt"]

    def prepare(self, weights, want_t: bool):
        for w in weights:
            ops._need(w.detach(), F32, "weight")
        if all(self._fresh(self._c.get(id(w)), w, want_t) for w in weights):
            return
        import numpy as np
        ents = [self._entry(w, want_t) for w in weights]
        key = (tuple(id(w) for w in weights), want_t)
        grp = self._groups.get(key)
        sig = tuple((e["ptr"], e["wb"].data_ptr(), e["wbt"].data_ptr() if e["wbt"] is not None else 0) for e in ents)
        if grp is None or grp["sig"] != sig or any(not w.is_contiguous() for w in weights):
            if any(not w.is_contiguous() for w in weights):
                for w in weights:
                    self.get(w, want_t)
                return
            dt = np.dtype([("w", "<u8"), ("wb", "<u8"), ("wbt", "<u8"), ("N", "<i4"), ("K", "<i4"), ("first", "<i4"), ("tk", "<i4")])
            tab = np.zeros(len(weights), dtype=dt)
            first = 0
            for i, (w, e) in enumerate(zip(weights, ents)):
                N, K = e["wb"].shape
                tab[i] = (e["ptr"], sig[i][1], sig[i][2], N, K, first, (K + 63) // 64)
                first += ((N + 63) // 64) * ((K + 63) // 64)
            dev_tab = torch.from_numpy(tab.view(np.uint8).copy()).to(weights[0].device)
            grp = self._groups[key] = {"sig": sig, "table": dev_tab, "tiles": first}
        ops._lib.check(ops._L().vitamd_cast_transpose_batched(grp["table"].data_ptr(), len(weights), grp["tiles"], ops._stream()),
                       "cast_transpose_batched")
        for w, e in zip(weights, ents):
            e["ver"], e["epoch"] = w._version, self.epoch


WEIGHTS = WeightCache()


TN_TARGET_WGS = None


TN_FORM_POLICY = "auto"


def _tn_form(which):
    if TN_FORM_POLICY == "shared":
        return ops.TN_FORM_SHARED
    if TN_FORM_POLICY == "exclusive" or not SIDE.enabled:
        return ops.TN_FORM_EXCLUSIVE
    return ops.TN_FORM_EXCLUSIVE if which == "fc2" else ops.TN_FORM_SHARED


def _tn_splits(dW, R=None):
    target = tn_target_wgs()
    if not target or not SIDE.enabled:
        return 0
    ntile = ((dW.shape[0] + 255) // 256) * ((dW.shape[1] + 255) // 256)
    splits = max(1, round(target / ntile))
    if R is not None:
        splits = min(splits, max(1, (R + 63) // 64))
    return splits


def tn_target_wgs():
    if TN_TARGET_WGS is not None:
        return TN_TARGET_WGS
    return 252 if ops.NT_PERSISTENT else 128


DEFER_RESID = True

KEEP_ROWS = True


def keep_rows(keep, N, causal, p_attn, p_mlp):
    if keep is None or not KEEP_ROWS or keep >= N or causal or p_attn > 0 or p_mlp > 0:
        return None
    return int(keep)


def streams_overlap(device, side=None):
    device = torch.device(device)
    side = side if side is not None else SIDE.stream(device)
    R, P = 16384, 512
    l = torch.ones(R, P, device=device, dtype=torch.bfloat16)
    o1, o2 = torch.empty(P, P, device=device), torch.empty(P, P, device=device)
    cur = torch.cuda.current_stream(device)

    def run(both):
        cur.synchronize(); side.synchronize()
        a, b = torch.cuda.Event(enable_timing=True), torch.cuda.Event(enable_timing=True)
        a.record(cur)
        if both:
            side.wait_stream(cur)
            with torch.cuda.stream(side):
                for _ in range(3):
                    ops.gemm_tn(l, l, o2, accumulate=False, splits=1)
        for _ in range(3):
            ops.gemm_tn(l, l, o1, accumulate=False, splits=1)
        if both:
            cur.wait_stream(side)
        b.record(cur)
        b.synchronize()
        return a.elapsed_time(b)

    run(True)
    one = min(run(False) for _ in range(2))
    two = min(run(True) for _ in range(2))
    return two / max(one, 1e-6)


def ensure_side_overlap(device, attempts=6):
    device = _indexed(device)
    ratio = streams_overlap(device)
    kept = []
    while ratio > 1.5 and attempts > 0:
        kept.append(SIDE._streams[device])
        SIDE._streams[device] = torch.cuda.Stream(device=device)
        ratio = streams_overlap(device)
        attempts -= 1
    return ratio


def _f32c(t):
    return t.detach().to(F32).contiguous()


def new_seed():
    return int(torch.randint(0, 2 ** 62, (1,)).item())


def _keep_native(N, keep):
    return ops.attention_keep_forms(N, keep) == (ops.KEEP_FWD | ops.KEEP_BWD)


def layer_forward(x0, wqkv, bqkv, w1, b1, w2, b2, B, N, H, causal, need_grad, p_attn=0.0, p_mlp=0.0, pending=None, defer=False, keep=None):
    drop = (p_attn, new_seed() if p_attn > 0 else 0, p_mlp, new_seed() if p_mlp > 0 else 0)
    wqkv_b, _ = WEIGHTS.get(wqkv, need_grad)
    w1_b, _ = WEIGHTS.get(w1, need_grad)
    w2_b, _ = WEIGHTS.get(w2, need_grad)
    x0, a, mean1, rstd1 = ops.layernorm_fwd(x0, addend=pending)
    qkv = ops.gemm_nt(a, wqkv_b, ops.EPI_BIAS_BF16, bias=bqkv)
    if keep is not None:
        if causal or p_attn > 0 or p_mlp > 0 or defer or not 0 < keep < N:
            raise ops._lib.VitamdError("layer_forward: keep needs a non-causal layer without dropout, defer=False and 0 < keep < N")
        if _keep_native(N, keep):
            o, lse = ops.attention_fwd_keep(qkv, B, N, H, keep)
            o_k = o
        else:
            o, lse = ops.attention_fwd(qkv, B, N, H)
            o_k = o.view(B, N, -1)[:, :keep].reshape(B * keep, -1).contiguous()
        x1, bln, mean2, rstd2 = ops.layernorm_fwd_keep(x0, o_k, B, N, keep)
        pre, h = ops.gemm_nt(bln, w1_b, ops.EPI_GELU_DG, bias=b1)
        x2 = ops.gemm_nt(h, w2_b, ops.EPI_RESID_F32, bias=b2, aux=x1)
        saved = (x0, mean1, rstd1, a, qkv, o, lse, x1, mean2, rstd2, bln, pre, h) if need_grad else None
        return x2, saved, drop
    o, lse = ops.attention_fwd(qkv, B, N, H, causal, dropout=drop[:2])
    x1, bln, mean2, rstd2 = ops.layernorm_fwd(x0, addend=o)
    pre, h = ops.gemm_nt(bln, w1_b, ops.EPI_GELU_DG, bias=b1)
    y = None
    if p_mlp > 0:
        x2 = ops.linear_dropout_resid(h, w2_b, b2, x1, drop[2:])
    elif defer:
        x2, y = x1, ops.gemm_nt(h, w2_b, ops.EPI_BIAS_BF16, bias=b2)
    else:
        x2 = ops.gemm_nt(h, w2_b, ops.EPI_RESID_F32, bias=b2, aux=x1)
    saved = (x0, mean1, rstd1, a, qkv, o, lse, x1, mean2, rstd2, bln, pre, h) if need_grad else None
    return (x2, y) if defer else x2, saved, drop


def _indexed(device):
    device = torch.device(device)
    if device.type == "cuda" and device.index is None:
        device = torch.device("cuda", torch.cuda.current_device())
    return device


class _Side:

    def __init__(self):
        self._streams = {}
        self.enabled = True

    def stream(self, device):
        device = _indexed(device)
        s = self._streams.get(device)
        if s is None:
            s = self._streams[device] = torch.cuda.Stream(device=device)
        return s


SIDE = _Side()


def claim_streams(device):
    device = _indexed(device)
    with torch.cuda.stream(SIDE.stream(device)):
        torch.zeros(16, device=device).add_(1)
    torch.cuda.current_stream(device).synchronize()


class GradSink:
    _sinks = []

    @classmethod
    def register(cls, sink):
        cls._sinks = [r for r in cls._sinks if r() is not None and r() is not sink]
        cls._sinks.append(weakref.ref(sink))

    @classmethod
    def find(cls, params):
        if params is None:
            return None
        for r in cls._sinks:
            s = r()
            if s is not None and s.owns(params):
                return s
        return None


def layer_sizes(D):
    return (3 * D * D, 3 * D, 4 * D * D, 4 * D, 4 * D * D, D), ((3 * D, D), (3 * D,), (4 * D, D), (4 * D,), (D, 4 * D), (D,))


def grad_arena(D, n_layers, device, params=None):
    sizes, shapes = layer_sizes(D)
    sink = GradSink.find(params)
    if sink is not None:
        got = sink.arena_for(params, n_layers)
        if got is not None:
            return got, sink
    per_w, per_b = sum(sizes[0::2]), sum(sizes[1::2])
    flat_w = torch.empty(per_w * n_layers, dtype=F32, device=device)
    flat_b = torch.zeros(per_b * n_layers, dtype=F32, device=device)
    out = []
    for i in range(n_layers):
        ow, ob, views = i * per_w, i * per_b, []
        for j, (n, sh) in enumerate(zip(sizes, shapes)):
            if j % 2 == 0:
                views.append(flat_w[ow: ow + n].view(sh))
                ow += n
            else:
                views.append(flat_b[ob: ob + n].view(sh))
                ob += n
        out.append(tuple(views))
    return out, None


KEEP_WGRAD_SIDE = True


def layer_backward(g2, saved, wqkv, w1, w2, B, N, H, causal, grads, dy2=None, have_db2=False, emit_bf16=False,
                   emit_colsum=None, drop=(0.0, 0, 0.0, 0), emit_dropout=(0.0, 0), keep=None):
    x0, mean1, rstd1, a, qkv, o, lse, x1, mean2, rstd2, bln, pre, h = saved
    dWqkv, dbqkv, dW1, db1, dW2, db2 = grads
    main = torch.cuda.current_stream()
    side = SIDE.stream(g2.device) if SIDE.enabled else main

    def on_side(fn, *tensors):
        if side is main:
            fn()
            return
        ev = torch.cuda.Event()
        ev.record(main)
        side.wait_event(ev)
        with torch.cuda.stream(side):
            fn()
        _SIDE_KEEP.extend(tensors)

    R_mlp = g2.shape[0] if keep is not None else None
    on_side_mlp = on_side if keep is None or KEEP_WGRAD_SIDE else (lambda fn, *tensors: fn())
    _, wqkv_t = WEIGHTS.get(wqkv, True)
    _, w1_t = WEIGHTS.get(w1, True)
    _, w2_t = WEIGHTS.get(w2, True)
    if dy2 is None:
        dy2 = ops.cast_bf16_dropout(g2, drop[2:]) if drop[2] > 0 else ops.cast_bf16(g2)
    def wgrad_fc2():
        ops.gemm_tn(dy2, h, dW2, accumulate=False, splits=_tn_splits(dW2, R_mlp), form=_tn_form("fc2"))
        if not have_db2:
            ops.colsum(dy2, db2)
    on_side_mlp(wgrad_fc2, dy2, h, dW2, db2)
    dpre = ops.gemm_nt(dy2, w2_t, ops.EPI_DMUL, aux=pre, colsum=db1)
    on_side_mlp(lambda: ops.gemm_tn(dpre, bln, dW1, accumulate=False, splits=_tn_splits(dW1, R_mlp), form=_tn_form("fc1")), dpre, bln, dW1)
    dbln = ops.gemm_nt(dpre, w1_t, ops.EPI_BIAS_BF16)
    g1, d_o = ops.layernorm_bwd(dbln, x1, mean2, rstd2, g_res=g2, want_bf16=True, xhat=bln)
    if keep is None:
        dqkv = ops.attention_bwd(qkv, o, lse, d_o, B, N, H, causal, dbias=dbqkv, dropout=drop[:2])
    elif _keep_native(N, keep):
        dqkv = ops.attention_bwd_keep(qkv, o, lse, d_o, B, N, H, keep, dbias=dbqkv)
    else:
        d_o_full = torch.zeros((B, N, d_o.shape[1]), dtype=BF16, device=d_o.device)
        d_o_full[:, :keep] = d_o.view(B, keep, -1)
        dqkv = ops.attention_bwd(qkv, o, lse, d_o_full.view(B * N, -1), B, N, H, causal, dbias=dbqkv)
    on_side(lambda: ops.gemm_tn(dqkv, a, dWqkv, accumulate=False, splits=_tn_splits(dWqkv), form=_tn_form("qkv")), dqkv, a, dWqkv)
    da = ops.gemm_nt(dqkv, wqkv_t, ops.EPI_BIAS_BF16)
    g0, g0b = ops.layernorm_bwd(da, x0, mean1, rstd1, g_res=g1, want_bf16=emit_bf16, colsum=emit_colsum, dropout=emit_dropout,
                                xhat=a, keep=None if keep is None else (N, keep))
    return g0, g0b


_SIDE_KEEP = []
_SIDE_DONE = []


def side_checkpoint(device):
    if not SIDE.enabled:
        _SIDE_KEEP.clear()
        return
    ev = torch.cuda.Event()
    ev.record(SIDE.stream(device))
    _SIDE_DONE.append((ev, list(_SIDE_KEEP)))
    _SIDE_KEEP.clear()
    while len(_SIDE_DONE) > 1:
        old_ev, _ = _SIDE_DONE.pop(0)
        torch.cuda.current_stream().wait_event(old_ev)


def join_side(device):
    if SIDE.enabled:
        ev = torch.cuda.Event()
        ev.record(SIDE.stream(device))
        torch.cuda.current_stream().wait_event(ev)
    _SIDE_KEEP.clear()
    _SIDE_DONE.clear()


class TransformerLayerFn(torch.autograd.Function):
    @staticmethod
    @_amp_fwd
    def forward(ctx, x, wqkv, bqkv, w1, b1, w2, b2, n_heads, causal, p_attn=0.0, p_mlp=0.0):
        B, N, D = x.shape
        need_grad = any(ctx.needs_input_grad)
        x2, saved, drop = layer_forward(_f32c(x).view(B * N, D), wqkv, _f32c(bqkv), w1, _f32c(b1), w2, _f32c(b2), B, N, n_heads,
                                        causal, need_grad, p_attn, p_mlp)
        if need_grad:
            ctx.save_for_backward(*saved)
            ctx.weights = (wqkv, w1, w2)
        ctx.drop = drop
        ctx.meta = (B, N, D, n_heads, causal, x.dtype)
        return x2.view(B, N, D).to(x.dtype)

    @staticmethod
    @_amp_bwd
    def backward(ctx, g):
        B, N, D, H, causal, xdtype = ctx.meta
        wqkv, w1, w2 = ctx.weights
        (grads,), _ = grad_arena(D, 1, g.device)
        g0, _ = layer_backward(_f32c(g).view(B * N, D), ctx.saved_tensors, wqkv, w1, w2, B, N, H, causal, grads, drop=ctx.drop)
        join_side(g.device)
        return (g0.view(B, N, D).to(xdtype), *grads, None, None, None, None)


class TransformerStackFn(torch.autograd.Function):

    @staticmethod
    @_amp_fwd
    def forward(ctx, x, n_heads, causal, p_attn, p_mlp, keep, *params):
        B, N, D = x.shape
        L = len(params) // 6
        if keep is not None and keep <= 0:
            raise ValueError(f"keep must be a positive number of tokens, got {keep}")
        k_last = keep_rows(keep, N, causal, p_attn, p_mlp)
        need_grad = any(ctx.needs_input_grad)
        cur = _f32c(x).view(B * N, D)
        saved_all, drops = [], []
        WEIGHTS.prepare([params[6 * i + j] for i in range(L) for j in (0, 2, 4)], need_grad)
        pending = None
        for i in range(L):
            wqkv, bqkv, w1, b1, w2, b2 = params[6 * i: 6 * i + 6]
            defer = DEFER_RESID and i + 1 < L and p_mlp == 0
            out, saved, drop = layer_forward(cur, wqkv, _f32c(bqkv), w1, _f32c(b1), w2, _f32c(b2), B, N, n_heads, causal, need_grad,
                                             p_attn, p_mlp, pending=pending, defer=defer, keep=k_last if i + 1 == L else None)
            cur, pending = out if defer else (out, None)
            drops.append(drop)
            if need_grad:
                saved_all.extend(saved)
        if need_grad:
            ctx.save_for_backward(*saved_all)
            ctx.params = params
        ctx.drops = drops
        n_out = N if k_last is None else k_last
        slice_to = keep if k_last is None and keep is not None and keep < N else None
        ctx.meta = (B, N, D, n_heads, causal, L, x.dtype, k_last, slice_to)
        out = cur.view(B, n_out, D)
        if slice_to is not None:
            out = out[:, :slice_to].contiguous()
        return out.to(x.dtype)

    @staticmethod
    @_amp_bwd
    def backward(ctx, g):
        B, N, D, H, causal, L, xdtype, k_last, slice_to = ctx.meta
        saved_all = ctx.saved_tensors
        params = ctx.params
        n_saved = len(saved_all) // L
        if slice_to is not None:
            full = torch.zeros((B, N, D), dtype=F32, device=g.device)
            full[:, :slice_to] = g
            g = full
        cur = _f32c(g).view(B * (N if k_last is None else k_last), D)
        arena, sink = grad_arena(D, L, cur.device, params)
        dy2 = None
        try:
            for i in reversed(range(L)):
                wqkv, _, w1, _, w2, _ = params[6 * i: 6 * i + 6]
                nxt_db2 = arena[i - 1][5] if i > 0 else None
                cur, dy2 = layer_backward(cur, saved_all[n_saved * i: n_saved * (i + 1)], wqkv, w1, w2, B, N, H, causal, arena[i],
                                          dy2=dy2, have_db2=dy2 is not None, emit_bf16=i > 0, emit_colsum=nxt_db2,
                                          drop=ctx.drops[i], emit_dropout=ctx.drops[i - 1][2:] if i > 0 else (0.0, 0),
                                          keep=k_last if i + 1 == L else None)
                if sink is not None:
                    sink.layer_ready(params, i)
                side_checkpoint(cur.device)
        finally:
            join_side(cur.device)
        grads = [t for layer in arena for t in layer]
        return (cur.view(B, N, D).to(xdtype), None, None, None, None, None, *grads)


class AttentionFn(torch.autograd.Function):
    @staticmethod
    @_amp_fwd
    def forward(ctx, x, wqkv, bqkv, n_heads, causal, p_attn=0.0):
        B, N, D = x.shape
        need_grad = any(ctx.needs_input_grad)
        wb, _ = WEIGHTS.get(wqkv, need_grad)
        xb = ops.cast_bf16(_f32c(x).view(B * N, D))
        qkv = ops.gemm_nt(xb, wb, ops.EPI_BIAS_BF16, bias=_f32c(bqkv))
        ctx.drop = (p_attn, new_seed() if p_attn > 0 else 0)
        o, lse = ops.attention_fwd(qkv, B, N, n_heads, causal, dropout=ctx.drop)
        if need_grad:
            ctx.save_for_backward(xb, qkv, o, lse)
            ctx.wqkv = wqkv
        ctx.meta = (B, N, D, n_heads, causal, x.dtype)
        return o.view(B, N, D).to(x.dtype)

    @staticmethod
    @_amp_bwd
    def backward(ctx, g):
        B, N, D, H, causal, xdtype = ctx.meta
        xb, qkv, o, lse = ctx.saved_tensors
        _, wt = WEIGHTS.get(ctx.wqkv, True)
        d_o = ops.cast_bf16(_f32c(g).view(B * N, D))
        db = torch.zeros((3 * D,), dtype=F32, device=g.device)
        dqkv = ops.attention_bwd(qkv, o, lse, d_o, B, N, H, causal, dbias=db, dropout=ctx.drop)
        dW = torch.empty((3 * D, D), dtype=F32, device=g.device)
        ops.gemm_tn(dqkv, xb, dW, accumulate=False)
        dx = ops.gemm_nt(dqkv, wt, ops.EPI_BIAS_BF16)
        return dx.view(B, N, D).to(xdtype), dW, db, None, None, None


class PatchEmbedFn(torch.autograd.Function):
    @staticmethod
    @_amp_fwd
    def forward(ctx, images, conv_w, conv_b, pos_w, extra_w, patch, n_patches):
        B = images.shape[0]
        D = conv_w.shape[0]
        extra = extra_w.shape[0]
        seq = n_patches + extra
        need_grad = any(ctx.needs_input_grad)
        patches = ops.im2col(_f32c(images), patch)
        if patches.shape[0] != B * n_patches:
            raise ops._lib.VitamdError(f"patch grid gives {patches.shape[0] // B} patches, config says {n_patches}")
        wb, _ = WEIGHTS.get(conv_w, ctx.needs_input_grad[0])
        x = torch.empty((B * seq, D), dtype=F32, device=images.device)
        ops.gemm_nt(patches, wb, ops.EPI_PATCH_F32, bias=_f32c(conv_b), aux=_f32c(pos_w)[:n_patches].contiguous(), out=x,
                    n_patches=n_patches, seq=seq, extra=extra)
        x = x.view(B, seq, D)
        if extra > 0:
            x[:, :extra] = extra_w.detach().to(F32)
        if need_grad:
            ctx.save_for_backward(patches)
            ctx.conv_w = conv_w
        ctx.meta = (B, D, extra, seq, n_patches, tuple(conv_w.shape), pos_w.shape[0], tuple(images.shape), patch)
        return x

    @staticmethod
    @_amp_bwd
    def backward(ctx, g):
        B, D, extra, seq, n_patches, wshape, pos_rows, ishape, patch = ctx.meta
        (patches,) = ctx.saved_tensors
        dpos, dextra, dyp, dbias = ops.embed_bwd(_f32c(g).view(B * seq, D), B, seq, extra, D)
        dW = torch.empty((D, patches.shape[1]), dtype=F32, device=g.device)
        ops.gemm_tn(dyp, patches, dW, accumulate=False)
        dimg = None
        if ctx.needs_input_grad[0]:
            _, wt = WEIGHTS.get(ctx.conv_w, True)
            dpatch = ops.gemm_nt(dyp, wt, ops.EPI_BIAS_BF16)
            _, C, Hh, Ww = ishape
            gh, gw = Hh // patch, Ww // patch
            dimg = dpatch.view(B, gh, gw, C, patch, patch).permute(0, 3, 1, 4, 2, 5).reshape(B, C, gh * patch, gw * patch).to(F32)
            if (gh * patch, gw * patch) != (Hh, Ww):
                full = torch.zeros(ishape, dtype=F32, device=g.device)
                full[:, :, : gh * patch, : gw * patch] = dimg
                dimg = full
        if pos_rows != n_patches:
            full = torch.zeros((pos_rows, D), dtype=F32, device=g.device)
            full[:n_patches] = dpos
            dpos = full
        return dimg, dW.view(wshape), dbias, dpos, dextra, None, None


def _pad64(n):
    return (n + 63) // 64 * 64


_PADDED = {}


def _padded_weight(w, b, Np, Kp):
    base = w._base if w._base is not None else w
    ent = _PADDED.get(id(base))
    bver = -1 if b is None else b._version
    if (ent is None or ent["ref"]() is not base or ent["ver"] != w._version or ent["ptr"] != w.data_ptr() or ent["epoch"] != WEIGHTS.epoch
            or ent["bver"] != bver or ent["shape"] != (Np, Kp)):
        if len(_PADDED) > 1024:
            for k in [k for k, v in _PADDED.items() if v["ref"]() is None]:
                del _PADDED[k]
        Nout, K = w.shape
        wp = torch.zeros((Np, Kp), dtype=F32, device=w.device)
        wp[:Nout, :K] = w.detach()
        bp = torch.zeros((Np,), dtype=F32, device=w.device)
        if b is not None:
            bp[:Nout] = b.detach()
        wb, wbt = ops.cast_weight(wp, True, True)
        ent = _PADDED[id(base)] = {"ref": weakref.ref(base), "ver": w._version, "ptr": w.data_ptr(), "epoch": WEIGHTS.epoch, "bver": bver,
                                "shape": (Np, Kp), "wb": wb, "wbt": wbt, "bp": bp}
    return ent["wb"], ent["wbt"], ent["bp"]


class LinearFn(torch.autograd.Function):

    @staticmethod
    @_amp_fwd
    def forward(ctx, x, w, b):
        M, K = x.shape
        Nout = w.shape[0]
        Np, Kp = _pad64(Nout), _pad64(K)
        dev = x.device
        wb, wbt, bp = _padded_weight(w, b, Np, Kp)
        xf = _f32c(x)
        if Kp != K:
            xpad = torch.zeros((M, Kp), dtype=F32, device=dev)
            xpad[:, :K] = xf
            xf = xpad
        xb = ops.cast_bf16(xf)
        y = ops.gemm_nt(xb, wb, ops.EPI_BIAS_BF16, bias=bp)
        ctx.save_for_backward(xb, wbt)
        ctx.meta = (M, K, Kp, Nout, Np, x.dtype, b is not None)
        return y[:, :Nout].to(F32)

    @staticmethod
    @_amp_bwd
    def backward(ctx, g):
        M, K, Kp, Nout, Np, xdtype, has_b = ctx.meta
        xb, wbt = ctx.saved_tensors
        gp = torch.zeros((M, Np), dtype=F32, device=g.device)
        gp[:, :Nout] = g
        gb = ops.cast_bf16(gp)
        dx = ops.gemm_nt(gb, wbt, ops.EPI_BIAS_BF16) if ctx.needs_input_grad[0] else None
        dWp = torch.empty((Np, Kp), dtype=F32, device=g.device)
        ops.gemm_tn(gb, xb, dWp, accumulate=False)
        db = ops.colsum(gb)[:Nout].clone() if has_b else None
        return (dx[:, :K].to(xdtype) if dx is not None else None), dWp[:Nout, :K].clone(), db


def linear(x, weight, bias):
    lead = x.shape[:-1]
    y = LinearFn.apply(x.reshape(-1, x.shape[-1]), weight.reshape(weight.shape[0], -1), bias)
    return y.view(*lead, weight.shape[0])
```

### vit-is-all-you-need_amd/vitamd/lib.py

```python
from __future__ import annotations

import ctypes
import os
import subprocess

_HERE = os.path.dirname(os.path.abspath(__file__))
LIB_PATH = os.path.join(_HERE, "libvitamd.so")
CSRC = os.path.join(os.path.dirname(_HERE), "csrc")
ABI_VERSION = 9

_c = ctypes
_P, _I, _F, _L, _U64, _D, _LL = _c.c_void_p, _c.c_int, _c.c_float, _c.c_long, _c.c_ulonglong, _c.c_double, _c.c_longlong

SIGNATURES = {
    "vitamd_abi_version": [],
    "vitamd_init": [_I, _P],
    "vitamd_gemm_nt_plan": [_I, _I, _I, _I, _I, _I],
    "vitamd_gemm_nt_bf16": [_P, _P, _P, _P, _P, _P, _P, _I, _I, _I, _I, _I, _I, _I, _I, _I, _P],
    "vitamd_gemm_tn_bf16": [_P, _P, _P, _I, _I, _I, _I, _I, _I, _I, _P],
    "vitamd_gemm_tn_bf16_ws": [_P, _P, _P, _I, _I, _I, _I, _I, _I, _I, _P, _L, _I, _I, _P],
    "vitamd_gemm_tn_ws_bytes": [_I, _I, _I, _I],
    "vitamd_layernorm_fwd": [_P, _P, _P, _P, _P, _P, _I, _I, _F, _P],
    "vitamd_layernorm_bwd": [_P, _P, _P, _P, _P, _P, _P, _P, _I, _I, _P],
    "vitamd_layernorm_affine_fwd": [_P, _P, _P, _P, _P, _P, _I, _I, _F, _P],
    "vitamd_layernorm_affine_bwd": [_P, _P, _P, _P, _P, _P, _P, _P, _P, _P, _P, _I, _I, _P],
    "vitamd_layernorm_affine_fwd_f32": [_P, _P, _P, _P, _P, _P, _I, _I, _F, _P],
    "vitamd_layernorm_affine_bwd_f32": [_P, _P, _P, _P, _P, _P, _P, _P, _I, _I, _P],
    "vitamd_attention_fwd": [_P, _P, _P, _I, _I, _I, _I, _I, _F, _U64, _P],
    "vitamd_attention_fwd_resid": [_P, _P, _P, _P, _P, _I, _I, _I, _I, _I, _F, _U64, _P],
    "vitamd_attention_bwd": [_P, _P, _P, _P, _P, _P, _P, _I, _I, _I, _I, _I, _F, _U64, _P],
    "vitamd_layernorm_bwd_dropout": [_P, _P, _P, _P, _P, _P, _P, _P, _I, _I, _F, _U64, _P],
    "vitamd_layernorm_bwd_xhat": [_P, _P, _P, _P, _P, _P, _P, _I, _I, _F, _U64, _P],
    "vitamd_linear_dropout_resid_bf16": [_P, _P, _P, _P, _P, _I, _I, _I, _F, _U64, _I, _P],
    "vitamd_cast_f32_bf16_dropout": [_P, _P, _L, _F, _U64, _P],
    "vitamd_cast_f32_bf16": [_P, _P, _L, _P],
    "vitamd_dropout_bf16": [_P, _P, _L, _L, _F, _U64, _P],
    "vitamd_dropout_f32": [_P, _P, _L, _L, _F, _U64, _P],
    "vitamd_cast_transpose_weight": [_P, _P, _P, _I, _I, _P],
    "vitamd_cast_transpose_batched": [_P, _I, _I, _P],
    "vitamd_im2col_bf16": [_P, _P, _I, _I, _I, _I, _I, _P],
    "vitamd_colsum_bf16": [_P, _P, _I, _I, _I, _P],
    "vitamd_embed_bwd": [_P, _P, _P, _P, _P, _P, _I, _I, _I, _I, _P],
    "vitamd_vq_nearest": [_P, _P, _P, _I, _I, _I, _P],
    "vitamd_conv3x3_fwd": [_P, _P, _P, _P, _I, _I, _I, _I, _I, _P],
    "vitamd_conv3x3_bwd": [_P, _P, _P, _P, _P, _P, _I, _I, _I, _I, _I, _P],
    "vitamd_adamw_step": [_P, _P, _P, _P, _L, _F, _F, _F, _F, _F, _I, _P],
    "vitamd_adamw_step_d": [_P, _P, _P, _P, _L, _F, _D, _D, _F, _F, _I, _P],
    "vitamd_mt_row_bytes": [],
    "vitamd_mt_chunk_elems": [],
    "vitamd_mt_grid_cap": [],
    "vitamd_mt_sumsq": [_P, _P, _I, _I, _P, _P, _F, _P],
    "vitamd_mt_adamw": [_P, _P, _I, _I, _P, _P],
    "vitamd_mt_scale": [_P, _P, _I, _I, _P, _P],
    "vitamd_kv_append": [_P, _P, _P, _P, _I, _I, _I, _I, _I, _P],
    "vitamd_decode_attention_ws_bytes": [_I, _I, _I],
    "vitamd_decode_attention": [_P, _P, _P, _P, _P, _I, _I, _I, _I, _P, _L, _P],
    "vitamd_gemm_skinny_ws_bytes": [_I, _I, _I],
    "vitamd_gemm_skinny_bf16": [_P, _P, _P, _P, _P, _P, _I, _I, _I, _I, _P, _L, _P],
    "vitamd_gemm_skinny_qkv_append": [_P, _P, _P, _P, _P, _P, _P, _I, _I, _I, _I, _I, _P, _L, _P],
    "vitamd_decode_embed": [_P, _P, _P, _P, _P, _I, _I, _I, _I, _P],
    "vitamd_sample_logits": [_P, _P, _P, _P, _P, _I, _I, _I, _F, _I, _F, _U64, _P],
    "vitamd_layernorm_fwd_keep": [_P, _P, _P, _P, _P, _P, _I, _I, _I, _I, _F, _P],
    "vitamd_layernorm_bwd_keep": [_P, _P, _P, _P, _P, _P, _P, _P, _I, _I, _I, _I, _I, _F, _U64, _P],
    "vitamd_attention_keep_forms": [_I, _I],
    "vitamd_attention_fwd_keep": [_P, _P, _P, _I, _I, _I, _I, _I, _P],
    "vitamd_attention_bwd_keep": [_P, _P, _P, _P, _P, _P, _P, _I, _I, _I, _I, _I, _P],
    "vitamd_cross_entropy_grid_rows": [_I],
    "vitamd_cross_entropy_fwd": [_P, _I, _P, _P, _P, _P, _I, _I, _I, _LL, _P],
    "vitamd_cross_entropy_bwd": [_P, _I, _P, _P, _P, _P, _P, _I, _I, _I, _I, _I, _LL, _P],
    "vitamd_embed_tokens_fwd": [_P, _P, _P, _P, _I, _I, _I, _I, _I, _P],
    "vitamd_embed_tokens_bwd": [_P, _P, _P, _P, _I, _I, _I, _I, _P],
}

ERRORS = {1: "unsupported shape", 2: "bad argument", 3: "HIP launch failure", 4: "vitamd_init has not run for this device"}

_lib = None


class VitamdError(RuntimeError):
    pass


def build(verbose: bool = False) -> str:
    r = subprocess.run(["make", "-C", CSRC, "-j8"], capture_output=True, text=True)
    if verbose or r.returncode != 0:
        print(r.stdout[-4000:], r.stderr[-4000:])
    if r.returncode != 0:
        raise VitamdError("building libvitamd.so failed")
    return LIB_PATH


def hip_runtimes(maps_path="/proc/self/maps"):
    found = set()
    with open(maps_path) as fh:
        for line in fh:
            parts = line.split(None, 5)
            if len(parts) == 6 and "libamdhip64" in os.path.basename(parts[5].strip()):
                found.add(os.path.realpath(parts[5].strip()))
    return sorted(found)


def check_single_hip_runtime(maps_path="/proc/self/maps"):
    found = hip_runtimes(maps_path)
    if len(found) > 1 and os.environ.get("VITAMD_ALLOW_TWO_HIP_RUNTIMES") != "1":
        raise VitamdError("two HIP runtimes are mapped into this process: " + " and ".join(found) + " - libvitamd.so must resolve libamdhip64 to "
                          "the runtime that owns the caller's streams and pointers (import torch / load the framework BEFORE dlopen-ing libvitamd.so)")
    return found


def load():
    global _lib
    if _lib is not None:
        return _lib
    if not os.path.exists(LIB_PATH):
        raise VitamdError(f"{LIB_PATH} is missing: run `python -c 'import __graft_entry__ as g; g.build()'` "
                          "(the HIP kernels are the only implementation of this path; there is no fallback)")
    import torch
    lib = ctypes.CDLL(LIB_PATH)
    check_single_hip_runtime()
    for name, argtypes in SIGNATURES.items():
        fn = getattr(lib, name)
        fn.argtypes = argtypes
        fn.restype = ctypes.c_long if name.endswith("_bytes") else ctypes.c_int
    if lib.vitamd_abi_version() != ABI_VERSION:
        raise VitamdError("libvitamd.so ABI version mismatch; rebuild")
    _lib = lib
    return lib


def check(code: int, what: str):
    if code != 0:
        raise VitamdError(f"{what}: {ERRORS.get(code, code)}")
```

### vit-is-all-you-need_amd/vitamd/ops.py

```python
from __future__ import annotations

import torch

from . import lib as _lib

EPI_BIAS_BF16, EPI_GELU, EPI_RESID_F32, EPI_DGELU, EPI_PATCH_F32, EPI_F32, EPI_GELU_DG, EPI_DMUL = range(8)
import os as _os
NT_PERSISTENT = _os.environ.get("VITAMD_NT_PERSISTENT", "1") != "0"
_seam_env = _os.environ.get("VITAMD_NT_SEAM", "auto")
NT_SEAM = {"1": True, "0": False}.get(_seam_env)
SEAM_PROBE = {}
NT_FORM_SEAM, NT_FORM_LOADER = 4, 5
_RAW_AUTO = -1
LN_EPS = 1e-5
BF16, F32 = torch.bfloat16, torch.float32


def _L():
    return _lib.load()


_INITIALISED = set()


def init(device=None):
    device = torch.device("cuda", torch.cuda.current_device()) if device is None else torch.device(device)
    idx = device.index if device.index is not None else torch.cuda.current_device()
    if idx in _INITIALISED:
        return
    if torch.cuda.is_current_stream_capturing():
        raise _lib.VitamdError("vitamd.ops.init: first use of a device inside a stream capture; run one eager step (or ops.init(device)) before capturing")
    _lib.check(_L().vitamd_init(idx, torch.cuda.current_stream(device).cuda_stream), f"vitamd_init[device {idx}]")
    _INITIALISED.add(idx)


def _stream():
    return torch.cuda.current_stream().cuda_stream


def _p(t):
    return None if t is None else t.data_ptr()


def _need(t, dtype, name, ndim=None):
    if not isinstance(t, torch.Tensor) or not t.is_cuda:
        raise _lib.VitamdError(f"{name}: expected a ROCm device tensor (the HIP kernels are the only implementation)")
    if t.dtype != dtype:
        raise _lib.VitamdError(f"{name}: expected {dtype}, got {t.dtype}")
    if not t.is_contiguous():
        raise _lib.VitamdError(f"{name}: must be contiguous")
    if ndim is not None and t.dim() != ndim:
        raise _lib.VitamdError(f"{name}: expected {ndim}-d, got {t.dim()}-d")
    return t


def gemm_nt(a, b, epi, *, bias=None, aux=None, out=None, out2=None, colsum=None, n_patches=0, seq=0, extra=0,
            out_rows=None, tile=0):
    _need(a, BF16, "a", 2); _need(b, BF16, "b", 2)
    M, K = a.shape
    N, K2 = b.shape
    if K != K2:
        raise _lib.VitamdError(f"gemm_nt: K mismatch {K} vs {K2}")
    out_dtype = F32 if epi in (EPI_RESID_F32, EPI_PATCH_F32, EPI_F32) else BF16
    if out is None:
        out = torch.empty((out_rows if out_rows is not None else M, N), dtype=out_dtype, device=a.device)
    _need(out, out_dtype, "out")
    if epi in (EPI_GELU, EPI_GELU_DG) and out2 is None:
        out2 = torch.empty((M, N), dtype=BF16, device=a.device)
    if bias is not None:
        _need(bias, F32, "bias", 1)
    if epi in (EPI_GELU, EPI_GELU_DG):
        init(a.device)
    if tile == 0:
        tile = auto_tile(a.device, M, N, K, epi)
    elif tile == _RAW_AUTO:
        tile = 0
    code = _L().vitamd_gemm_nt_bf16(_p(a), _p(b), _p(out), _p(out2), _p(bias), _p(aux), _p(colsum), M, N, K, N, epi,
                                    n_patches, seq, extra, tile, _stream())
    _lib.check(code, f"gemm_nt[M={M},N={N},K={K},epi={epi}]")
    return (out, out2) if epi in (EPI_GELU, EPI_GELU_DG) else out


def seam_enabled(device):
    if NT_SEAM is not None:
        return NT_SEAM
    idx = device.index if device.index is not None else torch.cuda.current_device()
    rec = SEAM_PROBE.get(idx)
    return None if rec is None else rec["enabled"]


def auto_tile(device, M, N, K, epi):
    if not NT_PERSISTENT:
        return 512
    on = seam_enabled(device)
    if on is None:
        if _L().vitamd_gemm_nt_plan(M, N, K, N, epi, 0) & 0x7f not in (NT_FORM_SEAM, NT_FORM_LOADER) or torch.cuda.is_current_stream_capturing():
            return 0
        on = seam_probe(device)
    return 0 if on else 1024


def seam_probe(device, rows=49152, reps=3):
    device = torch.device(device)
    if device.index is None:
        device = torch.device("cuda", torch.cuda.current_device())
    x = torch.randn(rows, 768, device=device).to(BF16)
    w = torch.randn(2304, 768, device=device).mul_(0.03).to(BF16)
    out = torch.empty((rows, 2304), dtype=BF16, device=device)
    times = {}
    for name, tile in (("seam_us", _RAW_AUTO), ("plain_us", 1024)):
        launch = lambda: gemm_nt(x, w, EPI_BIAS_BF16, out=out, tile=tile)
        launch()
        s, e = torch.cuda.Event(enable_timing=True), torch.cuda.Event(enable_timing=True)
        s.record()
        for _ in range(reps):
            launch()
        e.record()
        e.synchronize()
        times[name] = s.elapsed_time(e) / reps * 1e3
    on = times["seam_us"] <= 1.25 * times["plain_us"]
    SEAM_PROBE[device.index] = {"seam_us": round(times["seam_us"], 1), "plain_us": round(times["plain_us"], 1), "enabled": on}
    if not on:
        import warnings
        warnings.warn(f"vitamd: the seam form of the NT GEMM is slower than the plain persistent form on {device} "
                      f"({times['seam_us']:.0f} vs {times['plain_us']:.0f} us): switched off for this device")
    return on


_WORKSPACES = {}


def _workspace(device, nbytes):
    key = (device, torch.cuda.current_stream().cuda_stream)
    ws = _WORKSPACES.get(key)
    if ws is None or ws.numel() * 4 < nbytes:
        ws = _WORKSPACES[key] = torch.empty((nbytes + 3) // 4, dtype=F32, device=device)
    return ws


TN_FORM_SHARED, TN_FORM_EXCLUSIVE = 0, 1


def gemm_tn(l, r, out, splits=0, accumulate=True, atomic=False, form=TN_FORM_SHARED):
    _need(l, BF16, "l", 2); _need(r, BF16, "r", 2); _need(out, F32, "out", 2)
    R, P = l.shape
    R2, Q = r.shape
    if R != R2 or tuple(out.shape) != (P, Q):
        raise _lib.VitamdError("gemm_tn: shape mismatch")
    if atomic:
        if not accumulate:
            raise _lib.VitamdError("gemm_tn: the atomic form can only accumulate")
        code = _L().vitamd_gemm_tn_bf16(_p(l), _p(r), _p(out), R, P, Q, P, Q, Q, splits, _stream())
    else:
        nbytes = _L().vitamd_gemm_tn_ws_bytes(R, P, Q, splits)
        ws = _workspace(l.device, nbytes)
        code = _L().vitamd_gemm_tn_bf16_ws(_p(l), _p(r), _p(out), R, P, Q, P, Q, Q, splits, _p(ws), ws.numel() * 4, int(accumulate),
                                           int(form), _stream())
    _lib.check(code, f"gemm_tn[R={R},P={P},Q={Q}]")
    return out


def layernorm_fwd(x, addend=None):
    _need(x, F32, "x", 2)
    M, D = x.shape
    y = torch.empty((M, D), dtype=BF16, device=x.device)
    mean = torch.empty((M,), dtype=F32, device=x.device)
    rstd = torch.empty((M,), dtype=F32, device=x.device)
    x_out = None
    if addend is not None:
        _need(addend, BF16, "addend", 2)
        x_out = torch.empty_like(x)
    code = _L().vitamd_layernorm_fwd(_p(x), _p(addend), _p(x_out), _p(y), _p(mean), _p(rstd), M, D, LN_EPS, _stream())
    _lib.check(code, f"layernorm_fwd[M={M},D={D}]")
    return (x_out if addend is not None else x), y, mean, rstd


def layernorm_fwd_keep(x, addend, B, seq, keep):
    _need(x, F32, "x", 2); _need(addend, BF16, "addend", 2)
    D = x.shape[1]
    if x.shape[0] != B * seq or tuple(addend.shape) != (B * keep, D) or not 0 < keep <= seq:
        raise _lib.VitamdError(f"layernorm_fwd_keep: x must be [B*seq, D], addend [B*keep, D], 0 < keep <= seq (B={B}, seq={seq}, keep={keep})")
    Mk = B * keep
    x_out = torch.empty((Mk, D), dtype=F32, device=x.device)
    y = torch.empty((Mk, D), dtype=BF16, device=x.device)
    mean = torch.empty((Mk,), dtype=F32, device=x.device)
    rstd = torch.empty((Mk,), dtype=F32, device=x.device)
    _lib.check(_L().vitamd_layernorm_fwd_keep(_p(x), _p(addend), _p(x_out), _p(y), _p(mean), _p(rstd), B, seq, keep, D, LN_EPS, _stream()),
               f"layernorm_fwd_keep[B={B},seq={seq},keep={keep},D={D}]")
    return x_out, y, mean, rstd


def layernorm_bwd(dy, x, mean, rstd, g_res=None, want_bf16=False, colsum=None, dropout=(0.0, 0), xhat=None, keep=None):
    _need(dy, BF16, "dy", 2); _need(x, F32, "x", 2)
    M, D = x.shape
    g = torch.empty_like(x)
    gb = torch.empty((M, D), dtype=BF16, device=x.device) if want_bf16 else None
    if g_res is not None:
        _need(g_res, F32, "g_res", 2)
    if keep is not None:
        seq, k = keep
        if g_res is None or M % seq or not 0 < k <= seq or tuple(g_res.shape) != (M // seq * k, D):
            raise _lib.VitamdError(f"layernorm_bwd: keep=({seq}, {k}) needs M % seq == 0 and g_res fp32 [M/seq*k, D]")
        use_xhat = xhat is not None and D in (256, 512, 768, 1024)
        if use_xhat:
            _need(xhat, BF16, "xhat", 2)
        code = _L().vitamd_layernorm_bwd_keep(_p(dy), _p(xhat if use_xhat else x), _p(mean), _p(rstd), _p(g_res), _p(g), _p(gb), _p(colsum),
                                              M // seq, seq, k, D, int(use_xhat), float(dropout[0]), int(dropout[1]), _stream())
        _lib.check(code, f"layernorm_bwd_keep[M={M},D={D},seq={seq},keep={k}]")
        return g, gb
    if xhat is not None and D in (256, 512, 768, 1024):
        _need(xhat, BF16, "xhat", 2)
        code = _L().vitamd_layernorm_bwd_xhat(_p(dy), _p(xhat), _p(rstd), _p(g_res), _p(g), _p(gb), _p(colsum), M, D,
                                              float(dropout[0]), int(dropout[1]), _stream())
        _lib.check(code, f"layernorm_bwd_xhat[M={M},D={D}]")
        return g, gb
    code = _L().vitamd_layernorm_bwd_dropout(_p(dy), _p(x), _p(mean), _p(rstd), _p(g_res), _p(g), _p(gb), _p(colsum), M, D,
                                             float(dropout[0]), int(dropout[1]), _stream())
    _lib.check(code, f"layernorm_bwd[M={M},D={D}]")
    return g, gb


def layernorm_affine_fwd(x, gamma, beta, eps=LN_EPS):
    _need(x, F32, "x", 2); _need(gamma, F32, "gamma", 1); _need(beta, F32, "beta", 1)
    M, D = x.shape
    y = torch.empty((M, D), dtype=BF16, device=x.device)
    mean = torch.empty((M,), dtype=F32, device=x.device)
    rstd = torch.empty((M,), dtype=F32, device=x.device)
    _lib.check(_L().vitamd_layernorm_affine_fwd(_p(x), _p(gamma), _p(beta), _p(y), _p(mean), _p(rstd), M, D, float(eps), _stream()),
               "layernorm_affine_fwd")
    return y, mean, rstd


def layernorm_affine_bwd(dy, x, mean, rstd, gamma, dgamma, dbeta, g_res=None, want_bf16=False, colsum=None):
    _need(dy, BF16, "dy", 2); _need(x, F32, "x", 2); _need(gamma, F32, "gamma", 1)
    _need(dgamma, F32, "dgamma", 1); _need(dbeta, F32, "dbeta", 1)
    M, D = x.shape
    g = torch.empty_like(x)
    gb = torch.empty((M, D), dtype=BF16, device=x.device) if want_bf16 else None
    _lib.check(_L().vitamd_layernorm_affine_bwd(_p(dy), _p(x), _p(mean), _p(rstd), _p(gamma), _p(g_res), _p(g), _p(gb), _p(colsum),
                                                _p(dgamma), _p(dbeta), M, D, _stream()), "layernorm_affine_bwd")
    return g, gb


def layernorm_affine_fwd_f32(x, gamma, beta, eps=LN_EPS):
    _need(x, F32, "x", 2); _need(gamma, F32, "gamma", 1); _need(beta, F32, "beta", 1)
    M, D = x.shape
    y = torch.empty_like(x)
    mean = torch.empty((M,), dtype=F32, device=x.device)
    rstd = torch.empty((M,), dtype=F32, device=x.device)
    _lib.check(_L().vitamd_layernorm_affine_fwd_f32(_p(x), _p(gamma), _p(beta), _p(y), _p(mean), _p(rstd), M, D, float(eps), _stream()),
               "layernorm_affine_fwd_f32")
    return y, mean, rstd


def layernorm_affine_bwd_f32(dy, x, mean, rstd, gamma, dgamma, dbeta):
    _need(dy, F32, "dy", 2); _need(x, F32, "x", 2); _need(gamma, F32, "gamma", 1)
    _need(dgamma, F32, "dgamma", 1); _need(dbeta, F32, "dbeta", 1)
    M, D = x.shape
    g = torch.empty_like(x)
    _lib.check(_L().vitamd_layernorm_affine_bwd_f32(_p(dy), _p(x), _p(mean), _p(rstd), _p(gamma), _p(g), _p(dgamma), _p(dbeta), M, D,
                                                    _stream()), "layernorm_affine_bwd_f32")
    return g


ATTN_RESID_MAX_N = 256


def attention_fwd(qkv, B, N, H, causal=False, dropout=(0.0, 0), resid=None):
    _need(qkv, BF16, "qkv", 2)
    D = H * 64
    if tuple(qkv.shape) != (B * N, 3 * D):
        raise _lib.VitamdError("attention_fwd: qkv must be [B*N, 3*H*64] (head_dim 64 only)")
    o = torch.empty((B * N, D), dtype=BF16, device=qkv.device)
    lse = torch.empty((B, H, N), dtype=F32, device=qkv.device)
    if resid is not None:
        _need(resid, F32, "resid", 2)
        if tuple(resid.shape) != (B * N, D):
            raise _lib.VitamdError("attention_fwd: resid must be [B*N, H*64]")
        x1 = torch.empty_like(resid)
        code = _L().vitamd_attention_fwd_resid(_p(qkv), _p(o), _p(lse), _p(resid), _p(x1), B, N, H, 64, int(causal), float(dropout[0]),
                                               int(dropout[1]), _stream())
        _lib.check(code, f"attention_fwd_resid[B={B},N={N},H={H}]")
        return o, lse, x1
    code = _L().vitamd_attention_fwd(_p(qkv), _p(o), _p(lse), B, N, H, 64, int(causal), float(dropout[0]), int(dropout[1]), _stream())
    _lib.check(code, f"attention_fwd[B={B},N={N},H={H}]")
    return o, lse


def attention_bwd(qkv, o, lse, d_o, B, N, H, causal=False, dbias=None, dropout=(0.0, 0)):
    _need(qkv, BF16, "qkv", 2); _need(o, BF16, "o", 2); _need(d_o, BF16, "d_o", 2); _need(lse, F32, "lse")
    if dbias is not None:
        _need(dbias, F32, "dbias", 1)
    dqkv = torch.empty_like(qkv)
    delta = torch.empty_like(lse)
    code = _L().vitamd_attention_bwd(_p(qkv), _p(o), _p(lse), _p(d_o), _p(dqkv), _p(delta), _p(dbias), B, N, H, 64, int(causal),
                                     float(dropout[0]), int(dropout[1]), _stream())
    _lib.check(code, f"attention_bwd[B={B},N={N},H={H}]")
    return dqkv


KEEP_FWD, KEEP_BWD = 1, 2


def attention_keep_forms(N, nq):
    return int(_L().vitamd_attention_keep_forms(int(N), int(nq)))


def attention_fwd_keep(qkv, B, N, H, nq):
    _need(qkv, BF16, "qkv", 2)
    D = H * 64
    if tuple(qkv.shape) != (B * N, 3 * D) or not 0 < nq <= N:
        raise _lib.VitamdError("attention_fwd_keep: qkv must be [B*N, 3*H*64] (head_dim 64 only) and 0 < nq <= N")
    o = torch.empty((B * nq, D), dtype=BF16, device=qkv.device)
    lse = torch.empty((B, H, N), dtype=F32, device=qkv.device)
    _lib.check(_L().vitamd_attention_fwd_keep(_p(qkv), _p(o), _p(lse), B, N, H, 64, nq, _stream()), f"attention_fwd_keep[B={B},N={N},H={H},nq={nq}]")
    return o, lse


def attention_bwd_keep(qkv, o, lse, d_o, B, N, H, nq, dbias=None):
    _need(qkv, BF16, "qkv", 2); _need(o, BF16, "o", 2); _need(d_o, BF16, "d_o", 2); _need(lse, F32, "lse")
    D = H * 64
    if tuple(qkv.shape) != (B * N, 3 * D) or tuple(o.shape) != (B * nq, D) or tuple(d_o.shape) != (B * nq, D) or lse.numel() != B * H * N:
        raise _lib.VitamdError("attention_bwd_keep: qkv [B*N, 3*H*64], o and d_o compact [B*nq, H*64], lse [B, H, N]")
    if dbias is not None:
        _need(dbias, F32, "dbias", 1)
    dqkv = torch.empty_like(qkv)
    delta = torch.empty_like(lse)
    _lib.check(_L().vitamd_attention_bwd_keep(_p(qkv), _p(o), _p(lse), _p(d_o), _p(dqkv), _p(delta), _p(dbias), B, N, H, 64, nq, _stream()),
               f"attention_bwd_keep[B={B},N={N},H={H},nq={nq}]")
    return dqkv


def linear_dropout_resid(a, b, bias, resid, dropout):
    _need(a, BF16, "a", 2); _need(b, BF16, "b", 2); _need(resid, F32, "resid", 2); _need(bias, F32, "bias", 1)
    M, K = a.shape
    N = b.shape[0]
    out = torch.empty((M, N), dtype=F32, device=a.device)
    code = _L().vitamd_linear_dropout_resid_bf16(_p(a), _p(b), _p(out), _p(bias), _p(resid), M, N, K, float(dropout[0]), int(dropout[1]),
                                                 0 if NT_PERSISTENT else 512, _stream())
    _lib.check(code, f"linear_dropout_resid[M={M},N={N},K={K}]")
    return out


def cast_bf16_dropout(x, dropout):
    _need(x, F32, "x")
    out = torch.empty(x.shape, dtype=BF16, device=x.device)
    _lib.check(_L().vitamd_cast_f32_bf16_dropout(_p(x), _p(out), x.numel(), float(dropout[0]), int(dropout[1]), _stream()), "cast_dropout")
    return out


def dropout(x, p, seed, group=1, inplace=False):
    if x.dtype not in (BF16, F32):
        raise _lib.VitamdError(f"dropout: expected bf16 or fp32, got {x.dtype}")
    _need(x, x.dtype, "x")
    out = x if inplace else torch.empty_like(x)
    fn = _L().vitamd_dropout_bf16 if x.dtype == BF16 else _L().vitamd_dropout_f32
    _lib.check(fn(_p(x), _p(out), x.numel(), int(group), float(p), int(seed), _stream()), "dropout")
    return out


def cast_bf16(x):
    _need(x, F32, "x")
    out = torch.empty(x.shape, dtype=BF16, device=x.device)
    _lib.check(_L().vitamd_cast_f32_bf16(_p(x), _p(out), x.numel(), _stream()), "cast_f32_bf16")
    return out


def cast_weight(w, want_plain=True, want_transposed=False):
    _need(w, F32, "w", 2)
    N, K = w.shape
    wb = torch.empty((N, K), dtype=BF16, device=w.device) if want_plain else None
    wbt = torch.empty((K, N), dtype=BF16, device=w.device) if want_transposed else None
    _lib.check(_L().vitamd_cast_transpose_weight(_p(w), _p(wb), _p(wbt), N, K, _stream()), "cast_transpose_weight")
    return wb, wbt


def im2col(img, p):
    _need(img, F32, "img", 4)
    B, C, H, W = img.shape
    out = torch.empty((B * (H // p) * (W // p), C * p * p), dtype=BF16, device=img.device)
    _lib.check(_L().vitamd_im2col_bf16(_p(img), _p(out), B, C, H, W, p, _stream()), "im2col")
    return out


def colsum(x, out=None):
    _need(x, BF16, "x", 2)
    M, N = x.shape
    if out is None:
        out = torch.zeros((N,), dtype=F32, device=x.device)
    _lib.check(_L().vitamd_colsum_bf16(_p(x), _p(out), M, N, N, _stream()), "colsum")
    return out


def embed_bwd(g, B, seq, extra, D):
    _need(g, F32, "g", 2)
    n_p = seq - extra
    dev = g.device
    dpos = torch.zeros((n_p, D), dtype=F32, device=dev)
    dextra = torch.zeros((extra, D), dtype=F32, device=dev)
    dyp = torch.empty((B * n_p, D), dtype=BF16, device=dev)
    dbias = torch.zeros((D,), dtype=F32, device=dev)
    rows = torch.zeros((max(n_p, 1), D), dtype=F32, device=dev)
    _lib.check(_L().vitamd_embed_bwd(_p(g), _p(dpos), _p(dextra) if extra > 0 else None, _p(dyp), _p(dbias), _p(rows), B, seq, extra, D,
                                     _stream()), "embed_bwd")
    return dpos, dextra, dyp, dbias


def vq_nearest(x, codebook):
    _need(x, F32, "x", 2); _need(codebook, F32, "codebook", 2)
    M, d = x.shape
    K, d2 = codebook.shape
    if d != d2:
        raise _lib.VitamdError("vq_nearest: dim mismatch")
    idx = torch.empty((M,), dtype=torch.int64, device=x.device)
    _lib.check(_L().vitamd_vq_nearest(_p(x), _p(codebook), _p(idx), M, K, d, _stream()), "vq_nearest")
    return idx


def conv3x3_fwd(x, w, bias):
    _need(x, F32, "x", 4); _need(w, F32, "w", 4)
    B, C, H, W = x.shape
    Co = w.shape[0]
    if tuple(w.shape) != (Co, C, 3, 3):
        raise _lib.VitamdError("conv3x3: weight must be [Cout, Cin, 3, 3]")
    y = torch.empty((B, Co, H, W), dtype=F32, device=x.device)
    _lib.check(_L().vitamd_conv3x3_fwd(_p(x), _p(w), _p(bias), _p(y), B, C, Co, H, W, _stream()), f"conv3x3_fwd[Cin={C},Cout={Co}]")
    return y


def conv3x3_bwd(x, w, dy, need_dx=True, need_dw=True, has_bias=True):
    _need(x, F32, "x", 4); _need(w, F32, "w", 4); _need(dy, F32, "dy", 4)
    B, C, H, W = x.shape
    Co = w.shape[0]
    if tuple(dy.shape) != (B, Co, H, W):
        raise _lib.VitamdError("conv3x3_bwd: dy shape mismatch")
    dx = torch.empty_like(x) if need_dx else None
    dw = torch.zeros_like(w) if need_dw else None
    db = torch.zeros((Co,), dtype=F32, device=x.device) if (need_dw and has_bias) else None
    _lib.check(_L().vitamd_conv3x3_bwd(_p(x), _p(w), _p(dy), _p(dx), _p(dw), _p(db), B, C, Co, H, W, _stream()), "conv3x3_bwd")
    return dx, dw, db


SKINNY_MAX_M = 64
SKINNY_EPIS = (EPI_BIAS_BF16, EPI_GELU, EPI_RESID_F32, EPI_F32)
DECODE_MAX_LEN = 16384


def _need_len(length):
    _need(length, torch.int32, "len")
    if length.numel() != 1:
        raise _lib.VitamdError("len: expected a one-element device int32")
    return length


def _need_cache(k_cache, v_cache, B, H):
    _need(k_cache, BF16, "k_cache", 4); _need(v_cache, BF16, "v_cache", 4)
    if k_cache.shape != v_cache.shape or k_cache.shape[0] != B or k_cache.shape[1] != H or k_cache.shape[3] != 64:
        raise _lib.VitamdError(f"cache: expected k and v bf16 [B={B}, H={H}, Lmax, 64], got {tuple(k_cache.shape)} / {tuple(v_cache.shape)}")
    Lmax = k_cache.shape[2]
    if not 1 <= Lmax <= DECODE_MAX_LEN:
        raise _lib.VitamdError(f"cache: Lmax must be in [1, {DECODE_MAX_LEN}], got {Lmax}")
    return Lmax


def kv_append(qkv, k_cache, v_cache, length, B, T, H, host_len=None):
    _need(qkv, BF16, "qkv", 2); _need_len(length)
    Lmax = _need_cache(k_cache, v_cache, B, H)
    if tuple(qkv.shape) != (B * T, 3 * H * 64):
        raise _lib.VitamdError(f"kv_append: qkv must be [B*T, 3*H*64] = [{B * T}, {3 * H * 64}], got {tuple(qkv.shape)}")
    if T > Lmax or (host_len is not None and host_len + T > Lmax):
        raise _lib.VitamdError(f"kv_append: len {host_len} + T {T} exceeds the cache length {Lmax}")
    _lib.check(_L().vitamd_kv_append(_p(qkv), _p(k_cache), _p(v_cache), _p(length), B, T, H, 64, Lmax, _stream()),
               f"kv_append[B={B},T={T},H={H},Lmax={Lmax}]")


def decode_attention(qkv, k_cache, v_cache, length, B, H, host_len=None):
    _need(qkv, BF16, "qkv", 2); _need_len(length)
    Lmax = _need_cache(k_cache, v_cache, B, H)
    if tuple(qkv.shape) != (B, 3 * H * 64):
        raise _lib.VitamdError(f"decode_attention: qkv must be [B, 3*H*64] = [{B}, {3 * H * 64}], got {tuple(qkv.shape)}")
    if host_len is not None and host_len + 1 > Lmax:
        raise _lib.VitamdError(f"decode_attention: len {host_len} + 1 exceeds the cache length {Lmax}")
    nbytes = _L().vitamd_decode_attention_ws_bytes(B, H, Lmax)
    if nbytes < 0:
        raise _lib.VitamdError(f"decode_attention[B={B},H={H},Lmax={Lmax}]: {_lib.ERRORS.get(-nbytes, nbytes)}")
    ws = _workspace(qkv.device, nbytes) if nbytes > 0 else None
    o = torch.empty((B, H * 64), dtype=BF16, device=qkv.device)
    _lib.check(_L().vitamd_decode_attention(_p(qkv), _p(k_cache), _p(v_cache), _p(o), _p(length), B, H, 64, Lmax, _p(ws),
                                            0 if ws is None else ws.numel() * 4, _stream()), f"decode_attention[B={B},H={H},Lmax={Lmax}]")
    return o


def gemm_skinny(a, w, epi, *, bias=None, aux=None, out=None):
    _need(a, BF16, "a", 2); _need(w, BF16, "w", 2)
    M, K = a.shape
    N, K2 = w.shape
    if K != K2:
        raise _lib.VitamdError(f"gemm_skinny: K mismatch {K} vs {K2}")
    if epi not in SKINNY_EPIS:
        raise _lib.VitamdError(f"gemm_skinny: unsupported epilogue {epi}")
    if not 1 <= M <= SKINNY_MAX_M or N % 4 != 0 or K % 64 != 0:
        raise _lib.VitamdError(f"gemm_skinny[M={M},N={N},K={K}]: needs 1 <= M <= {SKINNY_MAX_M}, N % 4 == 0, K % 64 == 0")
    out_dtype = F32 if epi in (EPI_RESID_F32, EPI_F32) else BF16
    if out is None:
        out = torch.empty((M, N), dtype=out_dtype, device=a.device)
    _need(out, out_dtype, "out", 2)
    out2 = torch.empty((M, N), dtype=BF16, device=a.device) if epi == EPI_GELU else None
    if bias is not None:
        _need(bias, F32, "bias", 1)
        if bias.numel() != N:
            raise _lib.VitamdError(f"gemm_skinny: bias must have {N} elements")
    if epi == EPI_RESID_F32:
        _need(aux, F32, "aux", 2)
        if tuple(aux.shape) != (M, N):
            raise _lib.VitamdError(f"gemm_skinny: aux must be [{M}, {N}]")
    if tuple(out.shape) != (M, N):
        raise _lib.VitamdError(f"gemm_skinny: out must be [{M}, {N}]")
    if epi == EPI_GELU:
        init(a.device)
    nbytes = _L().vitamd_gemm_skinny_ws_bytes(M, N, K)
    ws = _workspace(a.device, nbytes) if nbytes > 0 else None
    code = _L().vitamd_gemm_skinny_bf16(_p(a), _p(w), _p(out), _p(out2), _p(bias), _p(aux) if epi == EPI_RESID_F32 else None, M, N, K, epi,
                                        _p(ws), 0 if ws is None else ws.numel() * 4, _stream())
    _lib.check(code, f"gemm_skinny[M={M},N={N},K={K},epi={epi}]")
    return (out, out2) if epi == EPI_GELU else out


def gemm_skinny_qkv_append(a, w, bias, k_cache, v_cache, length, H, host_len=None):
    _need(a, BF16, "a", 2); _need(w, BF16, "w", 2); _need_len(length)
    M, K = a.shape
    N, K2 = w.shape
    Lmax = _need_cache(k_cache, v_cache, M, H)
    if K != K2:
        raise _lib.VitamdError(f"gemm_skinny_qkv_append: K mismatch {K} vs {K2}")
    if N != 3 * H * 64:
        raise _lib.VitamdError(f"gemm_skinny_qkv_append: w must be [3*H*64, K] = [{3 * H * 64}, {K}], got {tuple(w.shape)}")
    if not 1 <= M <= SKINNY_MAX_M or K % 64 != 0:
        raise _lib.VitamdError(f"gemm_skinny_qkv_append[M={M},N={N},K={K}]: needs 1 <= M <= {SKINNY_MAX_M}, K % 64 == 0")
    if bias is not None:
        _need(bias, F32, "bias", 1)
        if bias.numel() != N:
            raise _lib.VitamdError(f"gemm_skinny_qkv_append: bias must have {N} elements")
    if host_len is not None and host_len + 1 > Lmax:
        raise _lib.VitamdError(f"gemm_skinny_qkv_append: len {host_len} + 1 exceeds the cache length {Lmax}")
    qkv = torch.empty((M, N), dtype=BF16, device=a.device)
    nbytes = _L().vitamd_gemm_skinny_ws_bytes(M, N, K)
    ws = _workspace(a.device, nbytes) if nbytes > 0 else None
    code = _L().vitamd_gemm_skinny_qkv_append(_p(a), _p(w), _p(qkv), _p(bias), _p(k_cache), _p(v_cache), _p(length), M, H, K, 64, Lmax,
                                              _p(ws), 0 if ws is None else ws.numel() * 4, _stream())
    _lib.check(code, f"gemm_skinny_qkv_append[M={M},H={H},K={K},Lmax={Lmax}]")
    return qkv


def decode_embed(tok_table, pos_table, tokens, length, out=None):
    _need(tok_table, F32, "tok_table", 2); _need(pos_table, F32, "pos_table", 2); _need(tokens, torch.int64, "tokens", 1); _need_len(length)
    B, D = tokens.shape[0], tok_table.shape[1]
    if pos_table.shape[1] != D or D % 4 != 0 or D < 4:
        raise _lib.VitamdError(f"decode_embed: tables must share D with D % 4 == 0, got {tuple(tok_table.shape)} / {tuple(pos_table.shape)}")
    if B < 1:
        raise _lib.VitamdError("decode_embed: expected at least one token")
    if out is None:
        out = torch.empty((B, D), dtype=F32, device=tokens.device)
    _need(out, F32, "out", 2)
    if tuple(out.shape) != (B, D):
        raise _lib.VitamdError(f"decode_embed: out must be [{B}, {D}], got {tuple(out.shape)}")
    _lib.check(_L().vitamd_decode_embed(_p(tok_table), _p(pos_table), _p(tokens), _p(length), _p(out), B, D, tok_table.shape[0],
                                        pos_table.shape[0], _stream()), f"decode_embed[B={B},D={D}]")
    return out


SAMPLE_MAX_V = 65536


def check_sampling(temperature, top_k, top_p, V=None):
    if not (isinstance(temperature, (int, float)) and 0 < temperature < float("inf")):
        raise ValueError(f"sampling: temperature must be a finite number > 0, got {temperature!r}")
    if not (isinstance(top_k, int) and not isinstance(top_k, bool) and top_k >= 0):
        raise ValueError(f"sampling: top_k must be an integer >= 0 (0 = off), got {top_k!r}")
    if not (isinstance(top_p, (int, float)) and 0 < top_p <= 1):
        raise ValueError(f"sampling: top_p must be in (0, 1] (1 = off), got {top_p!r}")
    if V is not None and not 2 <= V <= SAMPLE_MAX_V:
        raise ValueError(f"sampling: the vocabulary must hold 2 .. {SAMPLE_MAX_V} entries, got {V}")


def sample_logits(logits, temperature=1.0, top_k=0, top_p=1.0, *, u=None, seed=0, step=None, return_info=False):
    V = logits.shape[-1] if isinstance(logits, torch.Tensor) and logits.dim() == 2 else None
    check_sampling(temperature, top_k, top_p, V)
    if not isinstance(seed, int) or not 0 <= seed < 1 << 64:
        raise ValueError(f"sampling: seed must be an integer in [0, 2^64), got {seed!r}")
    if not isinstance(logits, torch.Tensor) or not logits.is_cuda:
        raise _lib.VitamdError("logits: expected a ROCm device tensor (the HIP kernels are the only implementation)")
    if logits.dtype != F32 or logits.dim() != 2 or logits.stride(1) != 1 or logits.stride(0) < logits.shape[1]:
        raise _lib.VitamdError(f"logits: expected fp32 [B, V] with unit inner stride, got {logits.dtype} {tuple(logits.shape)} strides {logits.stride()}")
    B, V = logits.shape
    if B < 1:
        raise _lib.VitamdError("logits: expected at least one row")
    if u is not None:
        _need(u, F32, "u", 1)
        if u.numel() != B:
            raise _lib.VitamdError(f"u: expected {B} elements, got {u.numel()}")
    if step is not None:
        _need(step, torch.uint64, "step")
        if step.numel() != 1:
            raise _lib.VitamdError("step: expected a one-element device uint64")
    token = torch.empty((B,), dtype=torch.int64, device=logits.device)
    info = torch.empty((B, 4), dtype=F32, device=logits.device) if return_info else None
    _lib.check(_L().vitamd_sample_logits(_p(logits), _p(token), _p(info), _p(u), _p(step), B, V, logits.stride(0), float(temperature), int(top_k),
                                         float(top_p), seed, _stream()), f"sample_logits[B={B},V={V},T={temperature},top_k={top_k},top_p={top_p}]")
    return (token, info) if return_info else token


CE_MAX_V = 65536


def cross_entropy_grid_rows(V):
    n = int(_L().vitamd_cross_entropy_grid_rows(int(V)))
    if n < 0:
        raise ValueError(f"cross_entropy: the vocabulary must hold 2 .. {CE_MAX_V} entries, got {V}")
    return n


def _need_logits(logits, name="logits"):
    V = logits.shape[-1] if isinstance(logits, torch.Tensor) and logits.dim() == 2 else None
    if V is not None and not 2 <= V <= CE_MAX_V:
        raise ValueError(f"cross_entropy: the vocabulary must hold 2 .. {CE_MAX_V} entries, got {V}")
    if not isinstance(logits, torch.Tensor) or not logits.is_cuda:
        raise _lib.VitamdError(f"{name}: expected a ROCm device tensor (the HIP kernels are the only implementation)")
    if logits.dtype not in (F32, BF16) or logits.dim() != 2 or logits.stride(1) != 1 or logits.stride(0) < logits.shape[1]:
        raise _lib.VitamdError(f"{name}: expected fp32 or bf16 [M, V] with unit inner stride, got {logits.dtype} {tuple(logits.shape)} "
                               f"strides {logits.stride()}")
    if logits.shape[0] < 1:
        raise _lib.VitamdError(f"{name}: expected at least one row")
    return logits.shape[0], logits.shape[1], logits.stride(0), int(logits.dtype == BF16)


def cross_entropy_fwd(logits, target, ignore_index=-100):
    M, V, ld, is_bf16 = _need_logits(logits)
    _need(target, torch.int64, "target", 1)
    if target.numel() != M:
        raise _lib.VitamdError(f"target: expected {M} elements, got {target.numel()}")
    loss_row = torch.empty((M,), dtype=F32, device=logits.device)
    lse = torch.empty((M,), dtype=F32, device=logits.device)
    stats = torch.empty((2,), dtype=F32, device=logits.device)
    _lib.check(_L().vitamd_cross_entropy_fwd(_p(logits), is_bf16, _p(target), _p(loss_row), _p(lse), _p(stats), M, V, ld, int(ignore_index),
                                             _stream()), f"cross_entropy_fwd[M={M},V={V},ld={ld}]")
    return loss_row, lse, stats


def cross_entropy_bwd(logits, target, lse, stats, grad_out=None, ignore_index=-100, out=None, out_dtype=None):
    M, V, ld, is_bf16 = _need_logits(logits)
    _need(target, torch.int64, "target", 1); _need(lse, F32, "lse", 1); _need(stats, F32, "stats", 1)
    if target.numel() != M or lse.numel() != M or stats.numel() != 2:
        raise _lib.VitamdError(f"cross_entropy_bwd: expected target [{M}], lse [{M}] and stats [2]")
    if grad_out is not None:
        _need(grad_out, F32, "grad_out")
        if grad_out.numel() != 1:
            raise _lib.VitamdError("grad_out: expected a one-element device fp32")
    if out is None:
        out = torch.empty((M, V), dtype=out_dtype or logits.dtype, device=logits.device)
    Mo, Vo, ldo, out_bf16 = _need_logits(out, "out")
    if (Mo, Vo) != (M, V):
        raise _lib.VitamdError(f"out: expected [{M}, {V}], got {tuple(out.shape)}")
    if out.data_ptr() == logits.data_ptr() and (out_bf16 != is_bf16 or ldo != ld):
        raise _lib.VitamdError("cross_entropy_bwd: in place needs the logits' own dtype and stride")
    _lib.check(_L().vitamd_cross_entropy_bwd(_p(logits), is_bf16, _p(target), _p(lse), _p(stats), _p(grad_out), _p(out), out_bf16, M, V, ld,
                                             ldo, int(ignore_index), _stream()), f"cross_entropy_bwd[M={M},V={V},ld={ld},ldo={ldo}]")
    return out


def _need_embed(ids, tok_table, pos_table, what):
    _need(tok_table, F32, "tok_table", 2); _need(pos_table, F32, "pos_table", 2); _need(ids, torch.int64, "ids", 2)
    B, S = ids.shape
    D = tok_table.shape[1]
    if pos_table.shape[1] != D or D % 4 != 0 or D < 4:
        raise _lib.VitamdError(f"{what}: tables must share D with D % 4 == 0, got {tuple(tok_table.shape)} / {tuple(pos_table.shape)}")
    if B < 1 or not 1 <= S <= pos_table.shape[0]:
        raise _lib.VitamdError(f"{what}: ids [B, S] need B >= 1 and 1 <= S <= {pos_table.shape[0]} positions, got {tuple(ids.shape)}")
    return B, S, D


def embed_tokens_fwd(ids, tok_table, pos_table, out=None):
    B, S, D = _need_embed(ids, tok_table, pos_table, "embed_tokens_fwd")
    if out is None:
        out = torch.empty((B * S, D), dtype=F32, device=ids.device)
    _need(out, F32, "out", 2)
    if tuple(out.shape) != (B * S, D):
        raise _lib.VitamdError(f"embed_tokens_fwd: out must be [{B * S}, {D}], got {tuple(out.shape)}")
    _lib.check(_L().vitamd_embed_tokens_fwd(_p(tok_table), _p(pos_table), _p(ids), _p(out), B, S, D, tok_table.shape[0], pos_table.shape[0],
                                            _stream()), f"embed_tokens_fwd[B={B},S={S},D={D}]")
    return out


def embed_tokens_bwd(g, ids, dtok, dpos):
    B, S, D = _need_embed(ids, dtok, dpos, "embed_tokens_bwd")
    _need(g, F32, "g", 2)
    if tuple(g.shape) != (B * S, D):
        raise _lib.VitamdError(f"embed_tokens_bwd: g must be [{B * S}, {D}], got {tuple(g.shape)}")
    _lib.check(_L().vitamd_embed_tokens_bwd(_p(g), _p(ids), _p(dtok), _p(dpos), B, S, D, dtok.shape[0], _stream()),
               f"embed_tokens_bwd[B={B},S={S},D={D}]")
    return dtok, dpos
```

Before: 9092 images/sec.

## Compute bias gradients inside weight-gradient GEMMs instead of epilogue/attention colsums

Bias gradients for fc2, fc1 and qkv are now accumulated from the A-fragments inside the split-K TN weight-gradient kernel using bf16 dot2 with ones. Partial sums are written to the workspace and reduced in the existing split-K reduce pass. This removes the separate colsum kernel for db2, the colsum epilogue in the dGELU NT GEMM (a new no-colsum variant), and the dbias path in attention backward. The cost is extra dot instructions and rotated fragment indexing in the TN inner loop, plus extra reduce blocks, and the precision of bias sums may change.

Result: faster. 9195 images/sec (median of 6 runs) (+1.1%).

```diff
diff --git a/include/vitamd.h b/include/vitamd.h
--- a/include/vitamd.h
+++ b/include/vitamd.h
@@ -47,6 +47,9 @@
 int vitamd_gemm_tn_bf16_ws(const void* L, const void* Rm, float* out, int R, int P, int Q, int ldl, int ldr, int ldo,
                            int splits, float* ws, long ws_bytes, int accumulate, int form, void* stream);
 long vitamd_gemm_tn_ws_bytes(int R, int P, int Q, int splits);
+
+int vitamd_gemm_tn_bf16_ws_colsum(const void* L, const void* Rm, float* out, float* colsum, int R, int P, int Q, int ldl, int ldr,
+                                  int ldo, int splits, float* ws, long ws_bytes, int accumulate, int form, void* stream);
 
 int vitamd_layernorm_fwd(const float* x_in, const void* addend_bf16, float* x_out, void* y_bf16, float* mean,
                          float* rstd, int M, int D, float eps, void* stream);
diff --git a/vit-is-all-you-need_amd/csrc/capi.hip b/vit-is-all-you-need_amd/csrc/capi.hip
--- a/vit-is-all-you-need_amd/csrc/capi.hip
+++ b/vit-is-all-you-need_amd/csrc/capi.hip
@@ -13,7 +13,7 @@
   if (epi == 6) epi = EPI_GELU;
   if (epi == 7) epi = EPI_DGELU;
   GemmNtArgs p{A, B, out, out2, bias, aux, colsum, M, N, K, ldo, epi, n_patches, seq, extra, tile, 0u, 1.0f, 0u, 0u, 0, dg};
-  if (!is_auto(tile) && tile != NT_TILE_128 && tile != NT_TILE_256 && tile != NT_TILE_320 && tile != NT_TILE_LOADER) return VITAMD_ERR_ARG;
+  if (!is_auto(tile) && tile != NT_TILE_128 && tile != NT_TILE_256 && tile != NT_TILE_320 && tile != NT_TILE_LOADER && tile != NT_TILE_SEAM) return VITAMD_ERR_ARG;
   return vitamd_gemm_nt_impl(p, (hipStream_t)stream);
 }
 
@@ -23,7 +23,7 @@
   if (epi == 7) epi = EPI_DGELU;
   static char dummy[16];
   GemmNtArgs p{dummy, dummy, dummy, dummy, nullptr, dummy, (float*)dummy, M, N, K, ldo, epi, 1, 1, 0, tile, 0u, 1.0f, 0u, 0u, 0, dg};
-  if (!is_auto(tile) && tile != NT_TILE_128 && tile != NT_TILE_256 && tile != NT_TILE_320 && tile != NT_TILE_LOADER) return -VITAMD_ERR_ARG;
+  if (!is_auto(tile) && tile != NT_TILE_128 && tile != NT_TILE_256 && tile != NT_TILE_320 && tile != NT_TILE_LOADER && tile != NT_TILE_SEAM) return -VITAMD_ERR_ARG;
   return vitamd_gemm_nt_plan_impl(p);
 }
 
@@ -37,6 +37,14 @@
                                       int splits, float* ws, long ws_bytes, int accumulate, int form, void* stream) {
   if (form != 0 && form != 1) return VITAMD_ERR_ARG;
   GemmTnArgs a{L, Rm, out, R, P, Q, ldl, ldr, ldo, splits, ws, (size_t)(ws_bytes < 0 ? 0 : ws_bytes), accumulate, form};
+  return vitamd_gemm_tn_impl(a, (hipStream_t)stream);
+}
+
+extern "C" int vitamd_gemm_tn_bf16_ws_colsum(const void* L, const void* Rm, float* out, float* colsum, int R, int P, int Q, int ldl, int ldr,
+                                             int ldo, int splits, float* ws, long ws_bytes, int accumulate, int form, void* stream) {
+  if (form != 0 && form != 1) return VITAMD_ERR_ARG;
+  GemmTnArgs a{L, Rm, out, R, P, Q, ldl, ldr, ldo, splits, ws, (size_t)(ws_bytes < 0 ? 0 : ws_bytes), accumulate, form, colsum};
+  if (colsum && !ws) return VITAMD_ERR_ARG;
   return vitamd_gemm_tn_impl(a, (hipStream_t)stream);
 }
 
diff --git a/vit-is-all-you-need_amd/csrc/gemm_nt.hip b/vit-is-all-you-need_amd/csrc/gemm_nt.hip
--- a/vit-is-all-you-need_amd/csrc/gemm_nt.hip
+++ b/vit-is-all-you-need_amd/csrc/gemm_nt.hip
@@ -283,6 +283,7 @@
   const bool seam_epi = epi == EPI_BIAS_BF16 || epi == EPI_GELU || epi == EPI_DGELU;
   const bool tall_epi = seam_epi || epi == EPI_RESID_F32;
   if (tile == NT_TILE_LOADER) return (seam_epi && ld_ok(p)) ? NtPlan{NT_FORM_LOADER, 256, VITAMD_OK} : NtPlan{0, 0, VITAMD_ERR_SHAPE};
+  if (tile == NT_TILE_SEAM) return (seam_epi && seam_ok(p)) ? NtPlan{NT_FORM_SEAM, 256, VITAMD_OK} : NtPlan{0, 0, VITAMD_ERR_SHAPE};
   const bool no_seam = tile == NT_TILE_AUTO_NO_SEAM;
   if (no_seam) tile = NT_TILE_AUTO;
   const long big_tiles = (long)((p.M + 255) / 256) * ((p.N + 255) / 256);
@@ -313,9 +314,11 @@
   if (pl.err) return pl.err;
   switch (pl.form) {
     case NT_FORM_LOADER:
+      if constexpr (EPI == EPI_DGELU) { if (!p.colsum) return launch_ld<EPI_DGELU_NOCS>(p, stream, device_cus()); }
       if constexpr (seam_epi) return launch_ld<EPI, EPI == EPI_GELU>(p, stream, device_cus());
       break;
     case NT_FORM_SEAM:
+      if constexpr (EPI == EPI_DGELU) { if (!p.colsum) return launch_seam<EPI_DGELU_NOCS, 8>(p, stream, device_cus()); }
       if constexpr (EPI == EPI_BIAS_BF16) { if (pl.rows == 320) return launch_seam<EPI, 10>(p, stream, device_cus()); }
       if constexpr (seam_epi) return launch_seam<EPI, 8, EPI == EPI_GELU>(p, stream, device_cus());
       break;
diff --git a/vit-is-all-you-need_amd/csrc/gemm_nt_ld.h b/vit-is-all-you-need_amd/csrc/gemm_nt_ld.h
--- a/vit-is-all-you-need_amd/csrc/gemm_nt_ld.h
+++ b/vit-is-all-you-need_amd/csrc/gemm_nt_ld.h
@@ -5,9 +5,11 @@
 
 template <int EPI, bool TAB = false, int SCHED = 1>
 __global__ __launch_bounds__(768) void gemm_nt_ld_kernel(const GemmNtArgs p) {
-  static_assert(EPI == EPI_BIAS_BF16 || EPI == EPI_GELU || EPI == EPI_DGELU, "epilogues of the loader form");
+  static_assert(EPI == EPI_BIAS_BF16 || EPI == EPI_GELU || EPI == EPI_DGELU || EPI == EPI_DGELU_NOCS, "epilogues of the loader form");
   static_assert(SCHED == 1, "request schedule");
   static_assert(!TAB || EPI == EPI_GELU, "table = GELU");
+  constexpr bool DG = EPI == EPI_DGELU || EPI == EPI_DGELU_NOCS;
+  constexpr bool CS = EPI == EPI_DGELU;
   constexpr int BM = 256, BN = 256, MT = 8, NT = 4;
   constexpr int AREG = 16384, ABUF = 32768, BBUF = 32768, BBASE = 2 * ABUF, OPS = BBASE + 2 * BBUF;
   constexpr int STG = 2048, TABOFF = OPS + 8 * STG;
@@ -89,7 +91,7 @@
         request_b(3); request_b(4); request_b(5);
         VITAMD_WAIT_VM(6);
         __builtin_amdgcn_s_barrier();
-        if constexpr (EPI != EPI_DGELU) {
+        if constexpr (!DG) {
           if (kt == 0) {
             asm_glds4(srdBias, lds_addr(smem) + OPS + l * STG, (unsigned)(bias_n0 + l * 64 + lane) * 4u, 0u);
             asm_glds4(srdBias, lds_addr(smem) + OPS + (4 + l) * STG, (unsigned)(bias_n0 + l * 64 + lane) * 4u, 0u);
@@ -119,7 +121,7 @@
   const int wm = wave >> 2, wn = wave & 3;
   const srd_t rsO = make_srd(p.out, (size_t)p.M * p.ldo * 2);
   const srd_t rsO2 = make_srd(EPI == EPI_GELU ? p.out2 : p.out, (size_t)p.M * p.ldo * 2);
-  const srd_t srdAux = make_srd(EPI == EPI_DGELU ? p.aux : p.out, (size_t)p.M * p.ldo * 2);
+  const srd_t srdAux = make_srd(DG ? p.aux : p.out, (size_t)p.M * p.ldo * 2);
   if constexpr (TAB) gelu_table_to_lds(p.gelu_tab, smem + TABOFF, tid);
   __builtin_amdgcn_s_barrier();
   asm volatile("" ::: "memory");
@@ -182,10 +184,10 @@
     const int mrow0 = m0 + wm * 128 + rsub;
     const unsigned obase = ncol_ok ? (unsigned)mrow0 * (unsigned)(p.ldo * 2) + (unsigned)ncol * 2u : OOB;
     const unsigned rstep = (unsigned)(p.ldo * 2) * 8u;
-    u32x4 aux[EPI == EPI_DGELU ? 2 * MT : 1];
-    u32x2 pk[EPI == EPI_DGELU ? MT : 1][NT];
+    u32x4 aux[DG ? 2 * MT : 1];
+    u32x2 pk[DG ? MT : 1][NT];
     f32x4 bias4[NT];
-    if constexpr (EPI == EPI_DGELU) {
+    if constexpr (DG) {
 #pragma unroll
       for (int i = 0; i < MT; ++i)
 #pragma unroll
@@ -208,7 +210,7 @@
 #pragma unroll
       for (int j = 0; j < NT; ++j) {
         u32x2 o;
-        if constexpr (EPI == EPI_DGELU) o = pk[i][j];
+        if constexpr (DG) o = pk[i][j];
         else {
           const f32x4 v = acc[i][j] + bias4[j];
           o = (u32x2){pack_bf16x2(v[0], v[1]), pack_bf16x2(v[2], v[3])};
@@ -241,14 +243,14 @@
           for (int c = 0; c < 4; ++c) {
             const float lo = round_bf16(bf16lo(v[c]) * bf16lo(pz[c]));
             const float hi = round_bf16(bf16hi(v[c]) * bf16hi(pz[c]));
-            if (voff != OOB) { cs[2 * c] += lo; cs[2 * c + 1] += hi; }
+            if constexpr (CS) { if (voff != OOB) { cs[2 * c] += lo; cs[2 * c + 1] += hi; } }
             o[c] = pack_bf16x2(lo, hi);
           }
           asm_bstore16_nt(o, rsO, voff, soff);
         }
       }
     }
-    if constexpr (EPI == EPI_DGELU) {
+    if constexpr (CS) {
 #pragma unroll
       for (int bf = 1; bf < 8; bf <<= 1)
 #pragma unroll
diff --git a/vit-is-all-you-need_amd/csrc/gemm_nt_seam.h b/vit-is-all-you-need_amd/csrc/gemm_nt_seam.h
--- a/vit-is-all-you-need_amd/csrc/gemm_nt_seam.h
+++ b/vit-is-all-you-need_amd/csrc/gemm_nt_seam.h
@@ -5,8 +5,10 @@
 
 template <int EPI, int MT, bool TAB = false>
 __global__ __launch_bounds__(512) void gemm_nt_seam_kernel(const GemmNtArgs p) {
-  static_assert(EPI == EPI_BIAS_BF16 || EPI == EPI_GELU || EPI == EPI_DGELU, "epilogues without (or with up-front) auxiliary loads");
+  static_assert(EPI == EPI_BIAS_BF16 || EPI == EPI_GELU || EPI == EPI_DGELU || EPI == EPI_DGELU_NOCS, "epilogues without (or with up-front) auxiliary loads");
   static_assert(!TAB || (EPI == EPI_GELU && MT == 8), "the GELU table needs the 16 KiB that only the 256-row ring leaves");
+  constexpr bool DG = EPI == EPI_DGELU || EPI == EPI_DGELU_NOCS;
+  constexpr bool CS = EPI == EPI_DGELU;
   constexpr int LA = 4;
   using S = NtSchedule<MT, LA>;
   constexpr int NP = S::NP;
@@ -16,7 +18,7 @@
   constexpr int TABOFF = OPS + 8 * STG;
   constexpr int SL = STG / 2048;
   static_assert(SL >= 1 && MT % SL == 0, "staging");
-  constexpr int E = EPI == EPI_GELU ? 4 * MT : EPI == EPI_DGELU ? 2 * MT + 1 : 2 * MT;
+  constexpr int E = EPI == EPI_GELU ? 4 * MT : CS ? 2 * MT + 1 : 2 * MT;
   static_assert(S::wait(NP - 1) + E <= 63 && S::wait(0, E) <= 63, "vmcnt is a 6-bit counter");
 
   extern __shared__ __attribute__((aligned(16))) char smem[];
@@ -31,7 +33,7 @@
   const srd_t srdB = make_srd(p.B, (size_t)p.N * K * 2);
   const srd_t rsO = make_srd(p.out, (size_t)p.M * p.ldo * 2);
   const srd_t rsO2 = make_srd(EPI == EPI_GELU ? p.out2 : p.out, (size_t)p.M * p.ldo * 2);
-  const srd_t srdAux = make_srd(EPI == EPI_DGELU ? p.aux : p.out, (size_t)p.M * p.ldo * 2);
+  const srd_t srdAux = make_srd(DG ? p.aux : p.out, (size_t)p.M * p.ldo * 2);
   const srd_t srdBias = make_srd(p.bias ? (const void*)p.bias : p.out, p.bias ? (size_t)p.N * 4 : 0);
   constexpr unsigned OOB = 0x80000000u;
   const unsigned lds0 = lds_addr(smem) + wave * 1024;
@@ -102,9 +104,9 @@
     const int mrow0 = m0 + wm * (16 * MT) + rsub;
     const unsigned obase = ncol_ok ? (unsigned)mrow0 * (unsigned)(p.ldo * 2) + (unsigned)ncol * 2u : OOB;
     const unsigned rstep = (unsigned)(p.ldo * 2) * 8u;
-    u32x4 aux[EPI == EPI_DGELU ? 2 * MT : 1];
-    u32x2 pk[EPI == EPI_DGELU ? MT : 1][NT];
-    if constexpr (EPI == EPI_DGELU) {
+    u32x4 aux[DG ? 2 * MT : 1];
+    u32x2 pk[DG ? MT : 1][NT];
+    if constexpr (DG) {
 #pragma unroll
       for (int i = 0; i < MT; ++i)
 #pragma unroll
@@ -126,7 +128,7 @@
     prologue();
     fill = true;
     constexpr int NREQ = S::prologue_requests();
-    if constexpr (EPI == EPI_DGELU) {
+    if constexpr (DG) {
       static_assert(MT == 8, "16 pre-load registers named in one asm statement");
       asm volatile("s_waitcnt vmcnt(%16)" : "+v"(aux[0]), "+v"(aux[1]), "+v"(aux[2]), "+v"(aux[3]), "+v"(aux[4]), "+v"(aux[5]), "+v"(aux[6]), "+v"(aux[7]), "+v"(aux[8]), "+v"(aux[9]), "+v"(aux[10]), "+v"(aux[11]), "+v"(aux[12]), "+v"(aux[13]), "+v"(aux[14]), "+v"(aux[15]) : "n"(NREQ) : "memory");
     } else {
@@ -136,7 +138,7 @@
 #pragma unroll
     for (int j = 0; j < NT; ++j) {
       bias4[j] = (f32x4){0.f, 0.f, 0.f, 0.f};
-      if constexpr (EPI != EPI_DGELU) {
+      if constexpr (!DG) {
 #pragma unroll
         for (int r = 0; r < 4; ++r) bias4[j][r] = round_bf16(((const float*)stg)[16 * j + 4 * g + r]);
       }
@@ -152,7 +154,7 @@
 #pragma unroll
         for (int j = 0; j < NT; ++j) {
           u32x2 o;
-          if constexpr (EPI == EPI_DGELU) o = pk[i][j];
+          if constexpr (DG) o = pk[i][j];
           else {
             const f32x4 v = acc[i][j] + bias4[j];
             o = (u32x2){pack_bf16x2(v[0], v[1]), pack_bf16x2(v[2], v[3])};
@@ -189,7 +191,7 @@
             for (int c = 0; c < 4; ++c) {
               const float lo = round_bf16(bf16lo(v[c]) * bf16lo(pz[c]));
               const float hi = round_bf16(bf16hi(v[c]) * bf16hi(pz[c]));
-              if (voff != OOB) { cs[2 * c] += lo; cs[2 * c + 1] += hi; }
+              if constexpr (CS) { if (voff != OOB) { cs[2 * c] += lo; cs[2 * c + 1] += hi; } }
               o[c] = pack_bf16x2(lo, hi);
             }
             asm_bstore16_nt(o, rsO, voff, soff);
@@ -197,7 +199,7 @@
         }
       }
     }
-    if constexpr (EPI == EPI_DGELU) {
+    if constexpr (CS) {
 #pragma unroll
       for (int bf = 1; bf < 8; bf <<= 1)
 #pragma unroll
@@ -227,7 +229,7 @@
 static bool seam_ok(const GemmNtArgs& p) {
   if (p.K % 64 != 0 || p.K < 128 || p.N % 8 != 0 || p.ldo % 8 != 0) return false;
   if ((size_t)p.M * p.K * 2 >= 0xf0000000ull || (size_t)p.N * p.K * 2 >= 0xf0000000ull || (size_t)p.M * p.ldo * 2 >= 0x80000000ull) return false;
-  if (p.epi == EPI_DGELU) return p.gelu_dg && p.colsum != nullptr && p.N % 256 == 0 && p.aux != nullptr;
+  if (p.epi == EPI_DGELU) return p.gelu_dg && p.N % 256 == 0 && p.aux != nullptr;
   if (p.epi == EPI_GELU) return p.out2 != nullptr;
   return p.epi == EPI_BIAS_BF16;
 }
diff --git a/vit-is-all-you-need_amd/csrc/gemm_tn.hip b/vit-is-all-you-need_amd/csrc/gemm_tn.hip
--- a/vit-is-all-you-need_amd/csrc/gemm_tn.hip
+++ b/vit-is-all-you-need_amd/csrc/gemm_tn.hip
@@ -20,11 +20,18 @@
   return __builtin_shufflevector(lo, hi, 0, 1, 2, 3, 4, 5, 6, 7);
 }
 
+typedef __attribute__((ext_vector_type(2))) __bf16 bf16x2;
+__device__ __forceinline__ float frag_pairsum(bf16x8 f, int c, float s) {
+  const bf16x2 ones = {(__bf16)1.0f, (__bf16)1.0f};
+  return __builtin_amdgcn_fdot2_f32_bf16((bf16x2){f[2 * c], f[2 * c + 1]}, ones, s, false);
+}
+
 constexpr int QSLOT = 16 * 512 * 2;
 
-template <bool WS, int NQ, int D>
+template <bool WS, int NQ, int D, bool CS = false>
 __global__ __launch_bounds__(NW * 64) void gemm_tn_pp_kernel(const GemmTnArgs a, int tiles_p, int tiles_q, int splits) {
   static_assert(D >= 2 && D <= NQ - 2, "prefetch distance: WAR rule");
+  static_assert(!CS || WS, "column sums go through the workspace");
   extern __shared__ __attribute__((aligned(16))) char smem[];
   const int tid = threadIdx.x, lane = tid & 63;
   const int wave = __builtin_amdgcn_readfirstlane(tid >> 6);
@@ -68,7 +75,8 @@
   int offA[MT], offB[NT];
 #pragma unroll
   for (int i = 0; i < MT; ++i) {
-    const int chunk = (wp * (BP / WP) + i * 32) / 8 + 2 * colhalf + (pp >> 1);
+    const int ip = CS ? (i + wq) & (MT - 1) : i;
+    const int chunk = (wp * (BP / WP) + ip * 32) / 8 + 2 * colhalf + (pp >> 1);
     offA[i] = rowpart + ((chunk ^ (qq << 2)) << 4);
   }
 #pragma unroll
@@ -94,6 +102,7 @@
   asm volatile("" ::: "memory");
   if (wp == 1) __builtin_amdgcn_s_barrier();
   int slot_r = 0;
+  float csum = 0.f;
   for (int g = g_lo; g < g_hi; ++g) {
     const char* q = smem + slot_r * QSLOT;
     bf16x8 af[MT], bfr[NT];
@@ -117,7 +126,10 @@
 #pragma unroll
     for (int i = 0; i < MT; ++i)
 #pragma unroll
-      for (int j = 0; j < NT; ++j) acc[i][j] = __builtin_amdgcn_mfma_f32_32x32x16_bf16(af[i], bfr[j], acc[i][j], 0, 0, 0);
+      for (int j = 0; j < NT; ++j) {
+        acc[i][j] = __builtin_amdgcn_mfma_f32_32x32x16_bf16(af[i], bfr[j], acc[i][j], 0, 0, 0);
+        if constexpr (CS) { if (i * NT + j < 4) csum = frag_pairsum(af[0], i * NT + j, csum); }
+      }
     __builtin_amdgcn_s_setprio(0);
     __builtin_amdgcn_sched_barrier(0);
     __builtin_amdgcn_s_barrier();
@@ -127,6 +139,15 @@
   if (wp == 0) __builtin_amdgcn_s_barrier();
   asm volatile("s_waitcnt vmcnt(0)" ::: "memory");
 #undef VITAMD_WAIT_VM
+  int rot = wq;
+  if constexpr (CS) asm volatile("" : "+s"(rot));
+  if constexpr (CS) {
+    if (tile % tiles_q == 0) {
+      csum += __shfl_xor(csum, 32, 64);
+      float* wc = a.ws + (size_t)splits * ntile * (BP * BQ) + ((size_t)split * tiles_p + tile / tiles_q) * BP;
+      if (lane < 32) wc[wp * (BP / WP) + rot * 32 + lane] = csum;
+    }
+  }
 
   if constexpr (WS) {
     float* wt = a.ws + ((size_t)split * ntile + tile) * (BP * BQ);
@@ -135,6 +156,13 @@
       const int ql = wq * (BQ / WQ) + j * 32 + (lane & 31);
 #pragma unroll
       for (int i = 0; i < MT; ++i) {
+        if constexpr (CS) {
+          float* const wti = wt + ((i + rot) & (MT - 1)) * (32 * BQ);
+          const int pl = wp * (BP / WP) + 4 * (lane >> 5);
+#pragma unroll
+          for (int r = 0; r < 16; ++r) wti[(pl + (r & 3) + 8 * (r >> 2)) * BQ + ql] = acc[i][j][r];
+          continue;
+        }
         const int pl = wp * (BP / WP) + i * 32 + 4 * (lane >> 5);
 #pragma unroll
         for (int r = 0; r < 16; ++r) wt[(pl + (r & 3) + 8 * (r >> 2)) * BQ + ql] = acc[i][j][r];
@@ -157,7 +185,7 @@
   }
 }
 
-template <int NQ, int D>
+template <int NQ, int D, bool CS = false>
 __global__ __launch_bounds__(768) void gemm_tn_ld_kernel(const GemmTnArgs a, int tiles_p, int tiles_q, int splits) {
   static_assert(D >= 2 && D <= NQ - 2, "prefetch distance: WAR rule");
   extern __shared__ __attribute__((aligned(16))) char smem[];
@@ -230,7 +258,8 @@
   int offA[MT], offB[NT];
 #pragma unroll
   for (int i = 0; i < MT; ++i) {
-    const int chunk = (wp * (BP / WP) + i * 32) / 8 + 2 * colhalf + (pp >> 1);
+    const int ip = CS ? (i + wq) & (MT - 1) : i;
+    const int chunk = (wp * (BP / WP) + ip * 32) / 8 + 2 * colhalf + (pp >> 1);
     offA[i] = rowpart + ((chunk ^ (qq << 2)) << 4);
   }
 #pragma unroll
@@ -242,6 +271,7 @@
   asm volatile("" ::: "memory");
   if (wp == 1) __builtin_amdgcn_s_barrier();
   int slot_r = 0;
+  float csum = 0.f;
   for (int g = g_lo; g < g_hi; ++g) {
     const char* q = smem + slot_r * QSLOT;
     bf16x8 af[MT], bfr[NT];
@@ -257,7 +287,10 @@
 #pragma unroll
     for (int i = 0; i < MT; ++i)
 #pragma unroll
-      for (int j = 0; j < NT; ++j) acc[i][j] = __builtin_amdgcn_mfma_f32_32x32x16_bf16(af[i], bfr[j], acc[i][j], 0, 0, 0);
+      for (int j = 0; j < NT; ++j) {
+        acc[i][j] = __builtin_amdgcn_mfma_f32_32x32x16_bf16(af[i], bfr[j], acc[i][j], 0, 0, 0);
+        if constexpr (CS) { if (i * NT + j < 4) csum = frag_pairsum(af[0], i * NT + j, csum); }
+      }
     __builtin_amdgcn_s_setprio(0);
     __builtin_amdgcn_sched_barrier(0);
     __builtin_amdgcn_s_barrier();
@@ -266,12 +299,28 @@
   }
   if (wp == 0) __builtin_amdgcn_s_barrier();
 #undef VITAMD_WAIT_VM
+  int rot = wq;
+  if constexpr (CS) asm volatile("" : "+s"(rot));
+  if constexpr (CS) {
+    if (tile % tiles_q == 0) {
+      csum += __shfl_xor(csum, 32, 64);
+      float* wc = a.ws + (size_t)splits * ntile * (BP * BQ) + ((size_t)split * tiles_p + tile / tiles_q) * BP;
+      if (lane < 32) wc[wp * (BP / WP) + rot * 32 + lane] = csum;
+    }
+  }
   float* wt = a.ws + ((size_t)split * ntile + tile) * (BP * BQ);
 #pragma unroll
   for (int j = 0; j < NT; ++j) {
     const int ql = wq * (BQ / WQ) + j * 32 + (lane & 31);
 #pragma unroll
     for (int i = 0; i < MT; ++i) {
+      if constexpr (CS) {
+        float* const wti = wt + ((i + rot) & (MT - 1)) * (32 * BQ);
+        const int pl = wp * (BP / WP) + 4 * (lane >> 5);
+#pragma unroll
+        for (int r = 0; r < 16; ++r) wti[(pl + (r & 3) + 8 * (r >> 2)) * BQ + ql] = acc[i][j][r];
+        continue;
+      }
       const int pl = wp * (BP / WP) + i * 32 + 4 * (lane >> 5);
 #pragma unroll
       for (int r = 0; r < 16; ++r) wt[(pl + (r & 3) + 8 * (r >> 2)) * BQ + ql] = acc[i][j][r];
@@ -281,7 +330,17 @@
 
 constexpr int RPT = 1;
 __global__ __launch_bounds__(256) void splitk_reduce_kernel(const float* __restrict__ ws, float* __restrict__ out, int P, int Q, int ldo,
-                                                            int tiles_q, int ntile, int splits, int accumulate) {
+                                                            int tiles_q, int ntile, int splits, int accumulate, float* __restrict__ colsum) {
+  if ((int)blockIdx.y >= ntile) {
+    static_assert(BP == 256, "one thread per column of a row tile");
+    const int tiles_p = ntile / tiles_q, tp = (int)blockIdx.y - ntile, p = tp * BP + (int)threadIdx.x;
+    if (blockIdx.x != 0 || p >= P) return;
+    const float* part = ws + (size_t)splits * ntile * (BP * BQ) + tp * BP + threadIdx.x;
+    float s = part[0];
+    for (int s2 = 1; s2 < splits; ++s2) s += part[(size_t)s2 * tiles_p * BP];
+    colsum[p] += s;
+    return;
+  }
   const int tile = blockIdx.y;
   const int p0 = (tile / tiles_q) * BP, q0 = (tile % tiles_q) * BQ;
   f32x4 sum[RPT];
@@ -329,7 +388,8 @@
 extern "C" long vitamd_gemm_tn_ws_bytes(int R, int P, int Q, int splits) {
   if (R <= 0 || P <= 0 || Q <= 0) return 0;
   const long ntile = (long)((P + BP - 1) / BP) * ((Q + BQ - 1) / BQ);
-  return (long)auto_splits(R, P, Q, splits) * ntile * BP * BQ * (long)sizeof(float);
+  const long tiles_p = (P + BP - 1) / BP;
+  return (long)auto_splits(R, P, Q, splits) * (ntile * BP * BQ + tiles_p * BP) * (long)sizeof(float);
 }
 
 int vitamd_gemm_tn_impl(const GemmTnArgs& a, hipStream_t stream) {
@@ -340,19 +400,29 @@
   const int ntile = tiles_p * tiles_q;
   const int splits = auto_splits(a.R, a.P, a.Q, a.splits);
   constexpr int lds = 8 * QSLOT;
-  const bool use_ws = a.ws != nullptr && a.ws_bytes >= (size_t)splits * ntile * BP * BQ * sizeof(float);
+  const size_t cs_bytes = a.colsum ? (size_t)splits * tiles_p * BP * sizeof(float) : 0;
+  const bool use_ws = a.ws != nullptr && a.ws_bytes >= (size_t)splits * ntile * BP * BQ * sizeof(float) + cs_bytes;
   if (!use_ws && !a.accumulate) return VITAMD_ERR_ARG;
+  if (!use_ws && a.colsum) return VITAMD_ERR_ARG;
   const dim3 grid(ntile * splits), block(NW * 64);
   if (use_ws) {
     if (a.form == 1) {
-      if (int e = set_lds(gemm_tn_ld_kernel<8, 4>, lds)) return e;
-      hipLaunchKernelGGL((gemm_tn_ld_kernel<8, 4>), grid, dim3(768), lds, stream, a, tiles_p, tiles_q, splits);
+      if (a.colsum) {
+        if (int e = set_lds(gemm_tn_ld_kernel<8, 4, true>, lds)) return e;
+        hipLaunchKernelGGL((gemm_tn_ld_kernel<8, 4, true>), grid, dim3(768), lds, stream, a, tiles_p, tiles_q, splits);
+      } else {
+        if (int e = set_lds(gemm_tn_ld_kernel<8, 4>, lds)) return e;
+        hipLaunchKernelGGL((gemm_tn_ld_kernel<8, 4>), grid, dim3(768), lds, stream, a, tiles_p, tiles_q, splits);
+      }
+    } else if (a.colsum) {
+      if (int e = set_lds(gemm_tn_pp_kernel<true, 8, 4, true>, lds)) return e;
+      hipLaunchKernelGGL((gemm_tn_pp_kernel<true, 8, 4, true>), grid, block, lds, stream, a, tiles_p, tiles_q, splits);
     } else {
       if (int e = set_lds(gemm_tn_pp_kernel<true, 8, 4>, lds)) return e;
       hipLaunchKernelGGL((gemm_tn_pp_kernel<true, 8, 4>), grid, block, lds, stream, a, tiles_p, tiles_q, splits);
     }
-    hipLaunchKernelGGL(splitk_reduce_kernel, dim3(BP * BQ / 4 / 256 / RPT, ntile), dim3(256), 0, stream, a.ws, a.out, a.P, a.Q, a.ldo, tiles_q, ntile, splits,
-                       a.accumulate);
+    hipLaunchKernelGGL(splitk_reduce_kernel, dim3(BP * BQ / 4 / 256 / RPT, ntile + (a.colsum ? tiles_p : 0)), dim3(256), 0, stream, a.ws, a.out, a.P, a.Q, a.ldo,
+                       tiles_q, ntile, splits, a.accumulate, a.colsum);
   } else {
     if (int e = set_lds(gemm_tn_pp_kernel<false, 8, 4>, lds)) return e;
     hipLaunchKernelGGL((gemm_tn_pp_kernel<false, 8, 4>), grid, block, lds, stream, a, tiles_p, tiles_q, splits);
diff --git a/vit-is-all-you-need_amd/csrc/vitamd_internal.h b/vit-is-all-you-need_amd/csrc/vitamd_internal.h
--- a/vit-is-all-you-need_amd/csrc/vitamd_internal.h
+++ b/vit-is-all-you-need_amd/csrc/vitamd_internal.h
@@ -8,6 +8,7 @@
   EPI_DGELU = 3,
   EPI_PATCH_F32 = 4,
   EPI_F32 = 5,
+  EPI_DGELU_NOCS = 6,
 };
 
 enum NtTileCode {
@@ -18,6 +19,7 @@
   NT_TILE_AUTO_NO_PERSISTENT = 512,
   NT_TILE_AUTO_NO_SEAM = 1024,
   NT_TILE_LOADER = 2048,
+  NT_TILE_SEAM = 4096,
 };
 inline bool is_auto(int tile) { return tile == NT_TILE_AUTO || tile == NT_TILE_AUTO_NO_PERSISTENT || tile == NT_TILE_AUTO_NO_SEAM; }
 
@@ -51,6 +53,7 @@
   size_t ws_bytes;
   int accumulate;
   int form;
+  float* colsum;
 };
 
 int vitamd_gemm_nt_impl(const GemmNtArgs& p, hipStream_t stream);
diff --git a/vit-is-all-you-need_amd/vitamd/functions.py b/vit-is-all-you-need_amd/vitamd/functions.py
--- a/vit-is-all-you-need_amd/vitamd/functions.py
+++ b/vit-is-all-you-need_amd/vitamd/functions.py
@@ -303,6 +303,10 @@
     return out, None
 
 
+BIAS_FROM_WGRAD = True
+
+BIAS_QKV_FROM_WGRAD = True
+
 KEEP_WGRAD_SIDE = True
 
 
@@ -331,24 +335,32 @@
     _, w2_t = WEIGHTS.get(w2, True)
     if dy2 is None:
         dy2 = ops.cast_bf16_dropout(g2, drop[2:]) if drop[2] > 0 else ops.cast_bf16(g2)
+    from_wgrad = BIAS_FROM_WGRAD
+    if from_wgrad:
+        emit_colsum = None
+
     def wgrad_fc2():
-        ops.gemm_tn(dy2, h, dW2, accumulate=False, splits=_tn_splits(dW2, R_mlp), form=_tn_form("fc2"))
-        if not have_db2:
+        ops.gemm_tn(dy2, h, dW2, accumulate=False, splits=_tn_splits(dW2, R_mlp), form=_tn_form("fc2"), colsum=db2 if from_wgrad else None)
+        if not from_wgrad and not have_db2:
             ops.colsum(dy2, db2)
     on_side_mlp(wgrad_fc2, dy2, h, dW2, db2)
-    dpre = ops.gemm_nt(dy2, w2_t, ops.EPI_DMUL, aux=pre, colsum=db1)
-    on_side_mlp(lambda: ops.gemm_tn(dpre, bln, dW1, accumulate=False, splits=_tn_splits(dW1, R_mlp), form=_tn_form("fc1")), dpre, bln, dW1)
+    dpre = ops.gemm_nt(dy2, w2_t, ops.EPI_DMUL, aux=pre, colsum=None if from_wgrad else db1)
+    on_side_mlp(lambda: ops.gemm_tn(dpre, bln, dW1, accumulate=False, splits=_tn_splits(dW1, R_mlp), form=_tn_form("fc1"),
+                                    colsum=db1 if from_wgrad else None), dpre, bln, dW1, db1)
     dbln = ops.gemm_nt(dpre, w1_t, ops.EPI_BIAS_BF16)
     g1, d_o = ops.layernorm_bwd(dbln, x1, mean2, rstd2, g_res=g2, want_bf16=True, xhat=bln)
+    qkv_from_wgrad = BIAS_QKV_FROM_WGRAD
+    dbias = None if qkv_from_wgrad else dbqkv
     if keep is None:
-        dqkv = ops.attention_bwd(qkv, o, lse, d_o, B, N, H, causal, dbias=dbqkv, dropout=drop[:2])
+        dqkv = ops.attention_bwd(qkv, o, lse, d_o, B, N, H, causal, dbias=dbias, dropout=drop[:2])
     elif _keep_native(N, keep):
-        dqkv = ops.attention_bwd_keep(qkv, o, lse, d_o, B, N, H, keep, dbias=dbqkv)
+        dqkv = ops.attention_bwd_keep(qkv, o, lse, d_o, B, N, H, keep, dbias=dbias)
     else:
         d_o_full = torch.zeros((B, N, d_o.shape[1]), dtype=BF16, device=d_o.device)
         d_o_full[:, :keep] = d_o.view(B, keep, -1)
-        dqkv = ops.attention_bwd(qkv, o, lse, d_o_full.view(B * N, -1), B, N, H, causal, dbias=dbqkv)
-    on_side(lambda: ops.gemm_tn(dqkv, a, dWqkv, accumulate=False, splits=_tn_splits(dWqkv), form=_tn_form("qkv")), dqkv, a, dWqkv)
+        dqkv = ops.attention_bwd(qkv, o, lse, d_o_full.view(B * N, -1), B, N, H, causal, dbias=dbias)
+    on_side(lambda: ops.gemm_tn(dqkv, a, dWqkv, accumulate=False, splits=_tn_splits(dWqkv), form=_tn_form("qkv"),
+                                colsum=dbqkv if qkv_from_wgrad else None), dqkv, a, dWqkv, dbqkv)
     da = ops.gemm_nt(dqkv, wqkv_t, ops.EPI_BIAS_BF16)
     g0, g0b = ops.layernorm_bwd(da, x0, mean1, rstd1, g_res=g1, want_bf16=emit_bf16, colsum=emit_colsum, dropout=emit_dropout,
                                 xhat=a, keep=None if keep is None else (N, keep))
diff --git a/vit-is-all-you-need_amd/vitamd/lib.py b/vit-is-all-you-need_amd/vitamd/lib.py
--- a/vit-is-all-you-need_amd/vitamd/lib.py
+++ b/vit-is-all-you-need_amd/vitamd/lib.py
@@ -19,6 +19,7 @@
     "vitamd_gemm_nt_bf16": [_P, _P, _P, _P, _P, _P, _P, _I, _I, _I, _I, _I, _I, _I, _I, _I, _P],
     "vitamd_gemm_tn_bf16": [_P, _P, _P, _I, _I, _I, _I, _I, _I, _I, _P],
     "vitamd_gemm_tn_bf16_ws": [_P, _P, _P, _I, _I, _I, _I, _I, _I, _I, _P, _L, _I, _I, _P],
+    "vitamd_gemm_tn_bf16_ws_colsum": [_P, _P, _P, _P, _I, _I, _I, _I, _I, _I, _I, _P, _L, _I, _I, _P],
     "vitamd_gemm_tn_ws_bytes": [_I, _I, _I, _I],
     "vitamd_layernorm_fwd": [_P, _P, _P, _P, _P, _P, _I, _I, _F, _P],
     "vitamd_layernorm_bwd": [_P, _P, _P, _P, _P, _P, _P, _P, _I, _I, _P],
diff --git a/vit-is-all-you-need_amd/vitamd/ops.py b/vit-is-all-you-need_amd/vitamd/ops.py
--- a/vit-is-all-you-need_amd/vitamd/ops.py
+++ b/vit-is-all-you-need_amd/vitamd/ops.py
@@ -141,21 +141,31 @@
 TN_FORM_SHARED, TN_FORM_EXCLUSIVE = 0, 1
 
 
-def gemm_tn(l, r, out, splits=0, accumulate=True, atomic=False, form=TN_FORM_SHARED):
+def gemm_tn(l, r, out, splits=0, accumulate=True, atomic=False, form=TN_FORM_SHARED, colsum=None):
     _need(l, BF16, "l", 2); _need(r, BF16, "r", 2); _need(out, F32, "out", 2)
     R, P = l.shape
     R2, Q = r.shape
     if R != R2 or tuple(out.shape) != (P, Q):
         raise _lib.VitamdError("gemm_tn: shape mismatch")
+    if colsum is not None:
+        _need(colsum, F32, "colsum", 1)
+        if colsum.numel() != P:
+            raise _lib.VitamdError("gemm_tn: colsum must be fp32 [P]")
     if atomic:
         if not accumulate:
             raise _lib.VitamdError("gemm_tn: the atomic form can only accumulate")
+        if colsum is not None:
+            raise _lib.VitamdError("gemm_tn: the atomic form has no reduce pass to sum colsum in")
         code = _L().vitamd_gemm_tn_bf16(_p(l), _p(r), _p(out), R, P, Q, P, Q, Q, splits, _stream())
     else:
         nbytes = _L().vitamd_gemm_tn_ws_bytes(R, P, Q, splits)
         ws = _workspace(l.device, nbytes)
-        code = _L().vitamd_gemm_tn_bf16_ws(_p(l), _p(r), _p(out), R, P, Q, P, Q, Q, splits, _p(ws), ws.numel() * 4, int(accumulate),
-                                           int(form), _stream())
+        if colsum is not None:
+            code = _L().vitamd_gemm_tn_bf16_ws_colsum(_p(l), _p(r), _p(out), _p(colsum), R, P, Q, P, Q, Q, splits, _p(ws), ws.numel() * 4,
+                                                      int(accumulate), int(form), _stream())
+        else:
+            code = _L().vitamd_gemm_tn_bf16_ws(_p(l), _p(r), _p(out), R, P, Q, P, Q, Q, splits, _p(ws), ws.numel() * 4, int(accumulate),
+                                               int(form), _stream())
     _lib.check(code, f"gemm_tn[R={R},P={P},Q={Q}]")
     return out
 
```
